# YannisLamp/crypto-recommendation

Measured on AMD Instinct MI355X. Metric: point hash+assign ops/sec at d=128, N=10M, K=256; 1/2/4/8 MI355X, higher is better.
Workload: dtype fp32 points; split-f16 MFMA scores (f32 accumulate); tuples, bucket IDs and cluster IDs bit-exact (x87-exact hashing, certified argmin); distances: certified f32, <= 2^-20 relative to the reference's fp64 (north star: 1e-5; the context's default LSHKM_DIST_CERTIFIED mode), LSHKM_DIST_EXACT for the r; 1 GPU; C3 Lloyd K=256 + C2 LSH L=5 k=4 hashing, N=10000000 per GPU, d=128; N_per_gpu=10000000, N_total=10000000, d=128, K=256, L=5, k=4, nb=100000, parallelism=dp1 (row shards)

## Files before the change

crypto-recommendation_amd/csrc/api.cpp:

```cpp
#include <hip/hip_runtime.h>

#include <algorithm>
#include <cmath>
#include <cstring>
#include <map>
#include <mutex>
#include <random>
#include <sstream>
#include <string>
#include <vector>

#include "../../include/lshkm.h"
#include "common.h"
#include "kernels.h"
#include "index.h"
#include "kpp_layout.h"

namespace lshkm {
static thread_local std::string g_err;
void set_error(const std::string& msg) { g_err = msg; }

int device_cu_count(int* ncu) {
    static std::mutex mu;
    static std::map<int, int> cus;
    int dev = 0;
    if (hipGetDevice(&dev) != hipSuccess) return kstatus("hipGetDevice");
    std::lock_guard<std::mutex> lock(mu);
    if (!cus.count(dev) &&
        hipDeviceGetAttribute(&cus[dev], hipDeviceAttributeMultiprocessorCount, dev) != hipSuccess) {
        cus.erase(dev);
        return kstatus("hipDeviceGetAttribute");
    }
    *ncu = cus[dev];
    return 0;
}
}

using namespace lshkm;

namespace lshkm {

Buf::~Buf() { if (p) (void)hipFree(p); }
int Buf::reserve(size_t bytes) {
    if (bytes <= cap) return 0;
    if (p) { (void)hipFree(p); p = nullptr; cap = 0; }
    if (hipMalloc(&p, bytes) != hipSuccess) { set_error("hipMalloc failed (" + std::to_string(bytes) + " B)"); p = nullptr; return LSHKM_ERR_NOMEM; }
    cap = bytes;
    return 0;
}

}

extern "C" {

const char* lshkm_last_error(void) { return g_err.c_str(); }
const char* lshkm_version(void) { return "lshkm-gfx950 0.1"; }

int lshkm_ctx_create(int device, lshkm_ctx* out) {
    LSHKM_CHECK(out, LSHKM_ERR_ARG, "out is NULL");
    *out = nullptr;
    if (const int rc = pow_contract_check()) return rc;
    int n = 0;
    LSHKM_HIP(hipGetDeviceCount(&n));
    LSHKM_CHECK(device >= 0 && device < n, LSHKM_ERR_ARG, "device out of range");
    LSHKM_HIP(hipSetDevice(device));
    hipDeviceProp_t prop;
    LSHKM_HIP(hipGetDeviceProperties(&prop, device));
    LSHKM_CHECK(std::string(prop.gcnArchName).find("gfx950") != std::string::npos, LSHKM_ERR_UNSUPPORTED,
                std::string("liblshkm is built for gfx950 only; device is ") + prop.gcnArchName);
    lshkm_ctx c = new lshkm_ctx_s();
    c->device = device;
    if (hipStreamCreateWithFlags(&c->own_stream, hipStreamNonBlocking) != hipSuccess) { delete c; set_error("stream create failed"); return LSHKM_ERR_HIP; }
    c->stream = c->own_stream;
    if (c->stats.reserve(sizeof(unsigned long long) * STAT_COUNT)) { delete c; return LSHKM_ERR_NOMEM; }
    (void)hipMemsetAsync(c->stats.p, 0, sizeof(unsigned long long) * STAT_COUNT, c->stream);
    *out = c;
    return 0;
}

int lshkm_ctx_set_stream(lshkm_ctx ctx, void* s) {
    LSHKM_CHECK(ctx, LSHKM_ERR_ARG, "ctx is NULL");
    ctx->stream = (hipStream_t)s;
    return 0;
}

int lshkm_ctx_set_dist_mode(lshkm_ctx ctx, int mode) {
    LSHKM_CHECK(ctx, LSHKM_ERR_ARG, "ctx is NULL");
    LSHKM_CHECK(mode == LSHKM_DIST_CERTIFIED || mode == LSHKM_DIST_EXACT, LSHKM_ERR_ARG,
                "unknown distance mode (LSHKM_DIST_CERTIFIED or LSHKM_DIST_EXACT)");
    ctx->dist_mode = mode;
    return 0;
}

int lshkm_ctx_get_dist_mode(lshkm_ctx ctx, int* mode) {
    LSHKM_CHECK(ctx && mode, LSHKM_ERR_ARG, "bad arguments");
    *mode = ctx->dist_mode;
    return 0;
}

int lshkm_ctx_sync(lshkm_ctx ctx) {
    LSHKM_CHECK(ctx, LSHKM_ERR_ARG, "ctx is NULL");
    LSHKM_HIP(hipStreamSynchronize(ctx->stream));
    return 0;
}

int lshkm_dev_alloc(lshkm_ctx ctx, int64_t bytes, void** out) {
    LSHKM_CHECK(ctx && out && bytes >= 0, LSHKM_ERR_ARG, "bad arguments");
    *out = nullptr;
    if (bytes == 0) return 0;
    LSHKM_HIP(hipSetDevice(ctx->device));
    if (hipMalloc(out, (size_t)bytes) != hipSuccess) {
        *out = nullptr;
        set_error("hipMalloc failed (" + std::to_string(bytes) + " B)");
        return LSHKM_ERR_NOMEM;
    }
    return 0;
}

int lshkm_dev_free(lshkm_ctx ctx, void* p) {
    LSHKM_CHECK(ctx, LSHKM_ERR_ARG, "ctx is NULL");
    if (!p) return 0;
    LSHKM_HIP(hipStreamSynchronize(ctx->stream));
    LSHKM_HIP(hipFree(p));
    return 0;
}

int lshkm_memcpy_h2d(lshkm_ctx ctx, void* dst_dev, const void* src_host, int64_t bytes) {
    LSHKM_CHECK(ctx && bytes >= 0 && (bytes == 0 || (dst_dev && src_host)), LSHKM_ERR_ARG, "bad arguments");
    if (bytes == 0) return 0;
    LSHKM_HIP(hipMemcpyAsync(dst_dev, src_host, (size_t)bytes, hipMemcpyHostToDevice, ctx->stream));
    LSHKM_HIP(hipStreamSynchronize(ctx->stream));
    return 0;
}

int lshkm_memcpy_d2h(lshkm_ctx ctx, void* dst_host, const void* src_dev, int64_t bytes) {
    LSHKM_CHECK(ctx && bytes >= 0 && (bytes == 0 || (dst_host && src_dev)), LSHKM_ERR_ARG, "bad arguments");
    if (bytes == 0) return 0;
    LSHKM_HIP(hipMemcpyAsync(dst_host, src_dev, (size_t)bytes, hipMemcpyDeviceToHost, ctx->stream));
    LSHKM_HIP(hipStreamSynchronize(ctx->stream));
    return 0;
}

int lshkm_ctx_destroy(lshkm_ctx ctx) {
    if (!ctx) return 0;
    (void)hipStreamSynchronize(ctx->stream);
    if (ctx->own_stream) (void)hipStreamDestroy(ctx->own_stream);
    delete ctx;
    return 0;
}

int lshkm_get_stat(lshkm_ctx ctx, int which, int64_t* v) {
    LSHKM_CHECK(ctx && v && which >= 0 && which < STAT_COUNT, LSHKM_ERR_ARG, "bad stat query");
    unsigned long long x = 0;
    LSHKM_HIP(hipMemcpyAsync(&x, (unsigned long long*)ctx->stats.p + which, sizeof(x), hipMemcpyDeviceToHost, ctx->stream));
    LSHKM_HIP(hipStreamSynchronize(ctx->stream));
    *v = (int64_t)x;
    return 0;
}

int lshkm_ctx_enable_timing(lshkm_ctx ctx, int on) {
    LSHKM_CHECK(ctx, LSHKM_ERR_ARG, "ctx is NULL");
    for (hipEvent_t& e : ctx->tev)
        if (!e) LSHKM_HIP(hipEventCreate(&e));
    ctx->timing = on != 0;
    return 0;
}

int lshkm_last_kernel_ms(lshkm_ctx ctx, float* ms) {
    LSHKM_CHECK(ctx && ms && ctx->tev[1], LSHKM_ERR_STATE, "timing not enabled");
    LSHKM_HIP(hipEventSynchronize(ctx->tev[1]));
    LSHKM_HIP(hipEventElapsedTime(ms, ctx->tev[0], ctx->tev[1]));
    if (ctx->tev_side) {
        float m2 = 0.f;
        LSHKM_HIP(hipEventSynchronize(ctx->tev[2]));
        LSHKM_HIP(hipEventElapsedTime(&m2, ctx->tev[0], ctx->tev[2]));
        *ms = std::max(*ms, m2);
    }
    return 0;
}

int lshkm_reset_stats(lshkm_ctx ctx) {
    LSHKM_CHECK(ctx, LSHKM_ERR_ARG, "ctx is NULL");
    LSHKM_HIP(hipMemsetAsync(ctx->stats.p, 0, sizeof(unsigned long long) * STAT_COUNT, ctx->stream));
    return 0;
}

static uint32_t engine_state(std::default_random_engine& g) {
    std::ostringstream os;
    os << g;
    return (uint32_t)std::stoul(os.str());
}

static void draw_euclid_h(std::default_random_engine& g, int d, float w, float* v, float* t) {
    std::normal_distribution<float> nd(0, 1);
    for (int j = 0; j < d; j++) v[j] = nd(g);
    std::uniform_real_distribution<float> ud(0, w);
    *t = ud(g);
}

static void draw_cosine_h(std::default_random_engine& g, int d, double* r) {
    std::normal_distribution<double> nd(0, 1);
    for (int j = 0; j < d; j++) r[j] = nd(g);
}

int lshkm_params_lsh_euclidean(uint64_t seed, int L, int k, int d, float w, float* V, float* t, int32_t* r,
                               uint32_t* state) {
    LSHKM_CHECK(L > 0 && k > 0 && d > 0 && V && t && r, LSHKM_ERR_ARG, "bad arguments");
    std::default_random_engine g;
    g.seed((unsigned long)seed);
    for (int l = 0; l < L; l++) {
        std::uniform_int_distribution<int> uid(0, 100);
        for (int i = 0; i < k; i++) {
            const size_t li = (size_t)l * k + i;
            draw_euclid_h(g, d, w, V + li * d, t + li);
            r[li] = uid(g);
        }
    }
    if (state) *state = engine_state(g);
    return 0;
}

int lshkm_params_lsh_cosine(uint64_t seed, int L, int k, int d, double* R, uint32_t* state) {
    LSHKM_CHECK(L > 0 && k > 0 && d > 0 && R, LSHKM_ERR_ARG, "bad arguments");
    std::default_random_engine g;
    g.seed((unsigned long)seed);
    for (int l = 0; l < L; l++)
        for (int i = 0; i < k; i++) draw_cosine_h(g, d, R + ((size_t)l * k + i) * d);
    if (state) *state = engine_state(g);
    return 0;
}

int lshkm_params_cube_euclidean(uint64_t seed, int k, int d, float w, float* V, float* t, uint32_t* state) {
    LSHKM_CHECK(k > 0 && d > 0 && V && t, LSHKM_ERR_ARG, "bad arguments");
    std::default_random_engine g;
    g.seed((unsigned long)seed);
    for (int i = 0; i < k; i++) draw_euclid_h(g, d, w, V + (size_t)i * d, t + i);
    if (state) *state = engine_state(g);
    return 0;
}

int lshkm_coins_draw(uint32_t* rng_state, const int32_t* h, int64_t n, int32_t* bit) {
    LSHKM_CHECK(rng_state && n >= 0 && (n == 0 || (h && bit)), LSHKM_ERR_ARG, "bad arguments");
    std::default_random_engine g;
    g.seed((unsigned long)*rng_state);
    LSHKM_CHECK(engine_state(g) == *rng_state, LSHKM_ERR_ARG, "rng_state is not a minstd_rand0 state");
    for (int64_t i = 0; i < n; i++) {
        std::uniform_int_distribution<int> coin(1, 2);
        const int c = coin(g);
        bit[i] = (h[i] % c + c) % c;
    }
    *rng_state = engine_state(g);
    return 0;
}

int lshkm_rand_selection(uint64_t seed, int64_t N, int K, int32_t* rows) {
    LSHKM_CHECK(rows && N >= 1 && N <= INT32_MAX && K >= 1 && K <= N, LSHKM_ERR_ARG,
                "bad arguments (need 1 <= K <= N < 2^31)");
    std::default_random_engine g;
    g.seed((unsigned long)seed);
    std::uniform_int_distribution<int> uni(0, (int)(N - 1));
    rows[0] = uni(g);
    for (int i = 1; i < K; i++) {
        int r = uni(g), c = 0;
        while (c < i) {
            if (rows[c] == r) { r = uni(g); c = 0; }
            else c++;
        }
        rows[i] = r;
    }
    return 0;
}

int lshkm_kpp_draws(uint64_t seed, int64_t N_total, int K, int64_t* first_row, double* canon) {
    LSHKM_CHECK(first_row && canon && N_total >= 1 && N_total <= INT32_MAX && K >= 1, LSHKM_ERR_ARG,
                "bad arguments (need 1 <= N < 2^31, K >= 1)");
    std::default_random_engine g;
    g.seed((unsigned long)seed);
    std::uniform_int_distribution<int> uni(0, (int)(N_total - 1));
    *first_row = uni(g);
    canon[0] = 0.0;
    for (int i = 1; i < K; i++) {
        std::uniform_real_distribution<double> unit(0.0, 1.0);
        canon[i] = unit(g);
    }
    return 0;
}

}

static int kmeans_pp_impl(lshkm_ctx ctx, Pts X, int64_t N, int d, int K, int metric, uint64_t seed, int32_t* rows) {
    LSHKM_CHECK(ctx && X.p && rows && N >= 1 && N <= INT32_MAX && d >= 1 && d <= 4096 && K >= 1, LSHKM_ERR_ARG,
                "bad arguments (need N < 2^31, 1 <= d <= 4096, K >= 1)");
    LSHKM_CHECK(metric == LSHKM_METRIC_EUCLIDEAN || metric == LSHKM_METRIC_COSINE, LSHKM_ERR_ARG, "unknown metric");
    LSHKM_HIP(hipSetDevice(ctx->device));
    std::vector<int32_t> chosen(K, 0);
    std::vector<double> canon(K, 0.0);
    int64_t first = 0;
    if (const int rc = lshkm_kpp_draws(seed, N, K, &first, canon.data())) return rc;
    chosen[0] = (int32_t)first;
    Buf &ws = ctx->ws_call[0], &dch = ctx->ws_call[1], &dcanon = ctx->ws_call[2];
    int rc;
    if ((rc = ws.reserve(kpp_layout(N).bytes)) || (rc = dch.reserve(sizeof(int32_t) * K)) ||
        (rc = dcanon.reserve(sizeof(double) * K)))
        return rc;
    LSHKM_HIP(hipMemcpyAsync(dch.p, chosen.data(), sizeof(int32_t) * K, hipMemcpyHostToDevice, ctx->stream));
    LSHKM_HIP(hipMemcpyAsync(dcanon.p, canon.data(), sizeof(double) * K, hipMemcpyHostToDevice, ctx->stream));
    if ((rc = launch_kmeans_pp(ctx->stream, X, N, d, K, metric, dcanon.as<double>(), dch.as<int32_t>(), ws.p,
                               (unsigned long long*)ctx->stats.p))) {
        (void)hipStreamSynchronize(ctx->stream);
        return rc;
    }
    LSHKM_HIP(hipMemcpyAsync(rows, dch.p, sizeof(int32_t) * K, hipMemcpyDeviceToHost, ctx->stream));
    LSHKM_HIP(hipStreamSynchronize(ctx->stream));
    return 0;
}

extern "C" {

int lshkm_kmeans_pp(lshkm_ctx ctx, const float* X, int64_t N, int d, int K, int metric, uint64_t seed,
                    int32_t* rows) {
    return kmeans_pp_impl(ctx, X, N, d, K, metric, seed, rows);
}

int lshkm_kmeans_pp_f64(lshkm_ctx ctx, const double* X, int64_t N, int d, int K, int metric, uint64_t seed,
                        int32_t* rows) {
    return kmeans_pp_impl(ctx, X, N, d, K, metric, seed, rows);
}

}

static int kpp_shard_ws_check(lshkm_ctx ctx, int64_t n, const void* ws, int64_t ws_bytes) {
    LSHKM_CHECK(ctx && n >= 0 && n <= INT32_MAX, LSHKM_ERR_ARG, "bad arguments (need 0 <= n < 2^31)");
    LSHKM_CHECK(n == 0 || (ws && ws_bytes >= 0 && (size_t)ws_bytes >= kpp_layout(n).bytes), LSHKM_ERR_ARG,
                "workspace smaller than lshkm_kpp_shard_ws_bytes");
    LSHKM_HIP(hipSetDevice(ctx->device));
    return 0;
}

static int kpp_shard_read(lshkm_ctx ctx, int64_t n, const void* ws, int launch_rc, KppShardOut* out) {
    if (launch_rc) {
        (void)hipStreamSynchronize(ctx->stream);
        return launch_rc;
    }
    LSHKM_HIP(hipMemcpyAsync(out, (const char*)ws + kpp_layout(n).out, sizeof(*out), hipMemcpyDeviceToHost,
                             ctx->stream));
    LSHKM_HIP(hipStreamSynchronize(ctx->stream));
    return 0;
}

static int kpp_shard_dist_impl(lshkm_ctx ctx, Pts X, int64_t n, int d, int metric, const void* c, int it, void* ws,
                               int64_t ws_bytes, uint64_t* max_bits, double* sum) {
    if (const int rc = kpp_shard_ws_check(ctx, n, ws, ws_bytes)) return rc;
    LSHKM_CHECK(max_bits && sum && d >= 1 && d <= 4096 && it >= 1, LSHKM_ERR_ARG,
                "bad arguments (need 1 <= d <= 4096, it >= 1)");
    LSHKM_CHECK(metric == LSHKM_METRIC_EUCLIDEAN || metric == LSHKM_METRIC_COSINE, LSHKM_ERR_ARG, "unknown metric");
    *max_bits = 0;
    *sum = 0.0;
    if (n == 0) return 0;
    LSHKM_CHECK(X.p && c, LSHKM_ERR_ARG, "rows or centroid row is NULL");
    KppShardOut o;
    const int lrc = launch_kpp_shard_dist(ctx->stream, X, n, d, metric, c, it, ws);
    if (const int rc = kpp_shard_read(ctx, n, ws, lrc, &o)) return rc;
    *max_bits = o.max_bits;
    *sum = o.sum;
    return 0;
}

extern "C" {

int lshkm_kpp_shard_ws_bytes(int64_t n, int64_t* bytes) {
    LSHKM_CHECK(bytes && n >= 0 && n <= INT32_MAX, LSHKM_ERR_ARG, "bad arguments (need 0 <= n < 2^31)");
    *bytes = (int64_t)kpp_layout(n).bytes;
    return 0;
}

int lshkm_kpp_shard_dist(lshkm_ctx ctx, const float* X, int64_t n, int d, int metric, const float* c, int it, void* ws,
                         int64_t ws_bytes, uint64_t* max_bits, double* sum) {
    return kpp_shard_dist_impl(ctx, X, n, d, metric, c, it, ws, ws_bytes, max_bits, sum);
}

int lshkm_kpp_shard_dist_f64(lshkm_ctx ctx, const double* X, int64_t n, int d, int metric, const double* c, int it,
                             void* ws, int64_t ws_bytes, uint64_t* max_bits, double* sum) {
    return kpp_shard_dist_impl(ctx, X, n, d, metric, c, it, ws, ws_bytes, max_bits, sum);
}

int lshkm_kpp_shard_units(lshkm_ctx ctx, int64_t n, uint64_t gmax_bits, double start, void* ws, int64_t ws_bytes) {
    if (const int rc = kpp_shard_ws_check(ctx, n, ws, ws_bytes)) return rc;
    if (n == 0) return 0;
    return launch_kpp_shard_units(ctx->stream, n, gmax_bits, start, ws);
}

int lshkm_kpp_shard_chain(lshkm_ctx ctx, int64_t n, double s_in, void* ws, int64_t ws_bytes, double* s_out) {
    if (const int rc = kpp_shard_ws_check(ctx, n, ws, ws_bytes)) return rc;
    LSHKM_CHECK(s_out, LSHKM_ERR_ARG, "s_out is NULL");
    *s_out = s_in;
    if (n == 0) return 0;
    KppShardOut o;
    const int lrc = launch_kpp_shard_chain(ctx->stream, n, s_in, ws, (unsigned long long*)ctx->stats.p);
    if (const int rc = kpp_shard_read(ctx, n, ws, lrc, &o)) return rc;
    *s_out = o.s_out;
    return 0;
}

int lshkm_kpp_shard_pick(lshkm_ctx ctx, int64_t n, double rd, int owns_row0, void* ws, int64_t ws_bytes,
                         int64_t* row) {
    if (const int rc = kpp_shard_ws_check(ctx, n, ws, ws_bytes)) return rc;
    LSHKM_CHECK(row, LSHKM_ERR_ARG, "row is NULL");
    *row = -1;
    if (n == 0) return 0;
    KppShardOut o;
    const int lrc = launch_kpp_shard_pick(ctx->stream, n, rd, owns_row0, ws);
    if (const int rc = kpp_shard_read(ctx, n, ws, lrc, &o)) return rc;
    LSHKM_CHECK(o.pick >= -1 && o.pick < n, LSHKM_ERR_STATE, "pick outside the shard (rd above the running sum?)");
    *row = o.pick;
    return 0;
}

int lshkm_params_cube_cosine(uint64_t seed, int k, int d, double* R, uint32_t* state) {
    LSHKM_CHECK(k > 0 && d > 0 && R, LSHKM_ERR_ARG, "bad arguments");
    std::default_random_engine g;
    g.seed((unsigned long)seed);
    for (int i = 0; i < k; i++) draw_cosine_h(g, d, R + (size_t)i * d);
    if (state) *state = engine_state(g);
    return 0;
}

}

namespace lshkm {

int ProjTable::upload(hipStream_t s, int metric_, int d_, int L_, int k_, float w_, const float* V, const float* t,
                      const int32_t* r, const double* R) {
    metric = metric_; d = d_; L = L_; k = k_; w = w_;
    LK = L * k;
    LKpad = hash_lkpad(LK);
    const int drows = (d + 3) / 4 * 4;
    std::vector<double> PT((size_t)drows * LKpad, 0.0), pn(LK, 0.0);
    std::vector<float> tt(LK, 0.f);
    std::vector<int32_t> rr(LK, 0);
    for (int f = 0; f < LK; f++) {
        long double n2 = 0.0L;
        for (int j = 0; j < d; j++) {
            const double v = metric == LSHKM_METRIC_EUCLIDEAN ? (double)V[(size_t)f * d + j] : R[(size_t)f * d + j];
            PT[(size_t)j * LKpad + f] = v;
            n2 += (long double)v * (long double)v;
        }
        pn[f] = (double)sqrtl(n2) * (1.0 + 0x1p-40);
        if (metric == LSHKM_METRIC_EUCLIDEAN) { tt[f] = t ? t[f] : 0.f; rr[f] = r ? r[f] : 0; }
    }
    int rc;
    if ((rc = PT_d.reserve(PT.size() * 8)) || (rc = t_d.reserve(LK * 4)) || (rc = pn_d.reserve(LK * 8)) ||
        (rc = r_d.reserve(LK * 4)))
        return rc;
    LSHKM_HIP(hipMemcpyAsync(PT_d.p, PT.data(), PT.size() * 8, hipMemcpyHostToDevice, s));
    LSHKM_HIP(hipMemcpyAsync(t_d.p, tt.data(), LK * 4, hipMemcpyHostToDevice, s));
    LSHKM_HIP(hipMemcpyAsync(pn_d.p, pn.data(), LK * 8, hipMemcpyHostToDevice, s));
    LSHKM_HIP(hipMemcpyAsync(r_d.p, rr.data(), LK * 4, hipMemcpyHostToDevice, s));
    bool r_small = true;
    for (int f = 0; f < LK; f++) r_small = r_small && rr[f] >= 0 && rr[f] <= 100;
    fused_ok = metric == LSHKM_METRIC_EUCLIDEAN && d == 128 && LK <= 32 && r_small;
    mfma_ok = d == 128 && LK <= 32;
    std::vector<_Float16> vh, vl;
    std::vector<double> v1;
    if (mfma_ok) {
        vh.assign(64 * 128, (_Float16)0.f);
        vl.assign(64 * 128, (_Float16)0.f);
        v1.assign(LK, 0.0);
        for (int f = 0; f < LK; f++) {
            long double s1 = 0.0L;
            for (int j = 0; j < 128; j++) {
                const double v = metric == LSHKM_METRIC_EUCLIDEAN ? (double)V[(size_t)f * d + j] : R[(size_t)f * d + j];
                const _Float16 hv = (_Float16)v;
                vh[f * 128 + j] = hv;
                vl[f * 128 + j] = (_Float16)(float)(v - (double)hv);
                s1 += fabsl((long double)v);
            }
            v1[f] = (double)s1 * (1.0 + 0x1p-40);
        }
        if ((rc = vh_d.reserve(vh.size() * 2)) || (rc = vl_d.reserve(vl.size() * 2)) || (rc = v1_d.reserve(LK * 8)))
            return rc;
        LSHKM_HIP(hipMemcpyAsync(vh_d.p, vh.data(), vh.size() * 2, hipMemcpyHostToDevice, s));
        LSHKM_HIP(hipMemcpyAsync(vl_d.p, vl.data(), vl.size() * 2, hipMemcpyHostToDevice, s));
        LSHKM_HIP(hipMemcpyAsync(v1_d.p, v1.data(), LK * 8, hipMemcpyHostToDevice, s));
    }
    LSHKM_HIP(hipStreamSynchronize(s));
    hV.assign(V ? V : (const float*)nullptr, V ? V + (size_t)LK * d : nullptr);
    return 0;
}

HashParams ProjTable::params(int64_t nb) const {
    HashParams p;
    p.PT = (const double*)PT_d.p;
    p.t = (const float*)t_d.p;
    p.pnorm = (const double*)pn_d.p;
    p.r = (const int32_t*)r_d.p;
    p.w = w;
    p.d = d; p.L = L; p.k = k; p.LK = LK; p.LKpad = LKpad;
    p.nb = nb;
    return p;
}

HashMfmaParams ProjTable::mfma_params(int64_t nb) const {
    HashMfmaParams p;
    p.Vh = vh_d.as<_Float16>(); p.Vl = vl_d.as<_Float16>();
    p.t = (const float*)t_d.p; p.pnorm = (const double*)pn_d.p; p.v1 = (const double*)v1_d.p;
    p.r = (const int32_t*)r_d.p; p.PT = (const double*)PT_d.p;
    p.w = w;
    p.d = d; p.L = L; p.k = k; p.LK = LK; p.LKpad = LKpad;
    p.nb = nb;
    return p;
}

}

extern "C" {

int lshkm_lsh_create(lshkm_ctx ctx, int metric, int d, int k, int L, int64_t nb, float w, const float* V,
                     const float* t, const int32_t* r, const double* R, lshkm_lsh* out) {
    LSHKM_CHECK(ctx && out, LSHKM_ERR_ARG, "ctx/out is NULL");
    LSHKM_CHECK(d > 0 && d <= 1024 && k > 0 && L > 0 && L * k <= 256, LSHKM_ERR_ARG, "unsupported d/k/L");
    LSHKM_CHECK(k <= 30, LSHKM_ERR_ARG, "k > 30");
    if (metric == LSHKM_METRIC_EUCLIDEAN) {
        LSHKM_CHECK(V && t && r, LSHKM_ERR_ARG, "euclidean LSH needs V, t, r");
        LSHKM_CHECK(nb > 0 && nb < (1ll << 31), LSHKM_ERR_ARG, "nb must be in [1, 2^31)");
        LSHKM_CHECK(w > 0.f, LSHKM_ERR_ARG, "w must be > 0");
    } else if (metric == LSHKM_METRIC_COSINE) {
        LSHKM_CHECK(R, LSHKM_ERR_ARG, "cosine LSH needs R");
        nb = (int64_t)1 << k;
    } else {
        set_error("unknown metric");
        return LSHKM_ERR_ARG;
    }
    LSHKM_HIP(hipSetDevice(ctx->device));
    lshkm_lsh h = new lshkm_lsh_s();
    h->ctx = ctx; h->metric = metric; h->nb = nb;
    int rc = h->proj.upload(ctx->stream, metric, d, L, k, w, V, t, r, R);
    if (rc) { delete h; return rc; }
    *out = h;
    return 0;
}

int lshkm_lsh_destroy(lshkm_lsh lsh) {
    if (!lsh) return 0;
    (void)hipDeviceSynchronize();
    delete lsh;
    return 0;
}

}

static int lsh_hash_impl(lshkm_lsh lsh, Pts X, int64_t N, int32_t* tuples, int32_t* phi, int32_t* bucket) {
    LSHKM_CHECK(lsh && (X.p || N == 0) && N >= 0, LSHKM_ERR_ARG, "bad arguments");
    lshkm_ctx ctx = lsh->ctx;
    LSHKM_HIP(hipSetDevice(ctx->device));
    const int mode = lsh->metric == LSHKM_METRIC_EUCLIDEAN ? HM_LSH_EUCLID : HM_LSH_COSINE;
    const int rc = hash_rows(ctx, mode, X, N, lsh->proj, lsh->nb, mode == HM_LSH_EUCLID ? tuples : nullptr, phi, bucket,
                             nullptr);
    if (rc) { LSHKM_LAUNCH_CHECK(); return rc; }
    return 0;
}

extern "C" {

int lshkm_lsh_hash(lshkm_lsh lsh, const float* X, int64_t N, int32_t* tuples, int32_t* phi, int32_t* bucket) {
    return lsh_hash_impl(lsh, X, N, tuples, phi, bucket);
}

int lshkm_lsh_hash_f64(lshkm_lsh lsh, const double* X, int64_t N, int32_t* tuples, int32_t* phi, int32_t* bucket) {
    return lsh_hash_impl(lsh, X, N, tuples, phi, bucket);
}

}

static int assign_path(int metric, int d, int K, bool f64) {
    if (test_switch("LSHKM_ASSIGN_PATH", "exact")) return 2;
    if (!test_switch("LSHKM_ASSIGN_PATH", "f32")) {
        const FusedRoute r = fused_route(metric != LSHKM_METRIC_EUCLIDEAN, f64, d, K, false, 0, 0,
                                         test_switch("LSHKM_FUSED_FORM", "chunked"));
        if (r.form != FusedForm::none) return r.rows == 0 ? 0 : 3;
    }
    return assign_dp(d) > 0 ? 1 : 2;
}

static bool fuse_hash(const lshkm_lsh_s* lsh, int metric, int K, bool f64) {
    const lshkm::ProjTable& pj = lsh->proj;
    if (lsh->metric != metric || !(metric == LSHKM_METRIC_EUCLIDEAN ? pj.fused_ok : pj.mfma_ok)) return false;
    return fused_route(metric != LSHKM_METRIC_EUCLIDEAN, f64, pj.d, K, true, pj.k, pj.LK,
                       test_switch("LSHKM_FUSED_FORM", "chunked")).form != FusedForm::none;
}

ExactForm lshkm::exact_form(const AssignJob& q) {
    return exact_route(q.metric != LSHKM_METRIC_EUCLIDEAN, q.X.f64, q.d, q.K, test_switch("LSHKM_EXACT_PASS", "full"));
}

int lshkm::exact_listed_prep(lshkm_ctx ctx, const AssignJob& q) {
    const ExactForm form = exact_form(q);
    int rc;
    if ((rc = ctx->ws_ct.reserve(exact_ws_bytes(form, q.d, q.K)))) return rc;
    return launch_exact_prep(ctx->stream, q, form, ctx->ws_ct.p);
}

int lshkm::exact_listed(lshkm_ctx ctx, const AssignJob& q, const RowList& l, bool exact_dist, bool prepped,
                        const double* xn2, const double* nbv) {
    int rc;
    if (!prepped && l.bound > 0 && (rc = exact_listed_prep(ctx, q))) return rc;
    return launch_exact_pass(ctx->stream, q, l, exact_form(q), ctx->ws_ct.p, exact_dist, xn2, nbv);
}

static int assign_f32_mfma(lshkm_ctx ctx, const AssignJob& q) {
    hipStream_t s = ctx->stream;
    const int DP = assign_dp(q.d), Kpad = (q.K + 63) / 64 * 64;
    const int64_t N = q.N;
    int rc;
    if ((rc = ctx->ws_c32.reserve((size_t)Kpad * DP * 4)) || (rc = ctx->ws_cconst.reserve((size_t)3 * Kpad * 4)) ||
        (rc = ctx->ws_ambig.reserve((size_t)std::max<int64_t>(N, 1) * 2 * 4)) ||
        (rc = ctx->ws_counter.reserve(64)))
        return rc;
    unsigned long long* cnt = (unsigned long long*)ctx->ws_counter.p;
    LSHKM_HIP(hipMemsetAsync(cnt, 0, 16, s));
    if ((rc = launch_centroid_prep(s, q.C, q.K, Kpad, q.d, DP, q.metric, q.X.f64, (float*)ctx->ws_c32.p, (float*)ctx->ws_cconst.p))) return rc;
    if ((rc = launch_assign_mfma(s, q.X, N, q.d, DP, q.C, q.K, Kpad, q.metric, (const float*)ctx->ws_c32.p, (const float*)ctx->ws_cconst.p,
                                 q.assign, q.dist, (int32_t*)ctx->ws_ambig.p, cnt))) return rc;
    RowList l;
    l.p = (int32_t*)ctx->ws_ambig.p; l.count = cnt; l.bound = N;
    if ((rc = exact_listed(ctx, q, l, true, false, nullptr, nullptr))) return rc;
    if (q.metric != LSHKM_METRIC_EUCLIDEAN &&
        ((rc = launch_cos_fix(s, q.X, N, q.d, q.C, (const int32_t*)ctx->ws_ambig.p + N, cnt + 1, q.assign, q.dist)) ||
         (rc = launch_add_counter(s, (unsigned long long*)ctx->stats.p + STAT_COS_FIX, cnt + 1)))) return rc;
    return launch_add_counter(s, (unsigned long long*)ctx->stats.p + STAT_ASSIGN_AMBIG, cnt);
}

static int assign_impl(lshkm_ctx ctx, Pts X, int64_t N, int d, const double* C, int K, int metric,
                       const int32_t* src_rows_host, int32_t* assign, double* dist, lshkm_lsh lsh, int32_t* tuples,
                       int32_t* phi, int32_t* bucket, bool force_exact = false) {
    hipStream_t s = ctx->stream;
    const int path = assign_path(metric, d, K, X.f64);
    AssignRequest q;
    q.X = X; q.N = N; q.d = d; q.C = C; q.K = K; q.metric = metric; q.assign = assign; q.dist = dist;
    q.tuples = tuples; q.phi = phi; q.bucket = bucket; q.force_exact = force_exact;
    if (lsh && path == 0 && fuse_hash(lsh, metric, K, X.f64)) q.lsh = lsh;
    int rc;
    if (lsh && !q.lsh && (rc = hash_rows(ctx, lsh->metric == LSHKM_METRIC_EUCLIDEAN ? HM_LSH_EUCLID : HM_LSH_COSINE,
                                         X, N, lsh->proj, lsh->nb,
                                         lsh->metric == LSHKM_METRIC_EUCLIDEAN ? tuples : nullptr, phi, bucket,
                                         nullptr))) { LSHKM_LAUNCH_CHECK(); return rc; }
    if (path == 0 || path == 3) rc = fused_assign(ctx, q);
    else if (path == 1) rc = assign_f32_mfma(ctx, q);
    else {
        RowList all;
        all.bound = N;
        rc = launch_exact_pass(s, q, all, ExactForm::every, nullptr, true, nullptr, nullptr);
    }
    if (rc) { LSHKM_LAUNCH_CHECK(); return rc; }
    if (src_rows_host) {
        if ((rc = ctx->ws_src.reserve((size_t)K * 4))) return rc;
        const bool same = ctx->src_cache_dev == ctx->ws_src.p && ctx->src_cache_cap == ctx->ws_src.cap &&
                          ctx->src_cache.size() == (size_t)K &&
                          std::memcmp(ctx->src_cache.data(), src_rows_host, (size_t)K * 4) == 0;
        if (!same) {
            if ((rc = ctx->pin_stage((size_t)K * 4))) return rc;
            std::memcpy(ctx->pinned, src_rows_host, (size_t)K * 4);
            LSHKM_HIP(hipMemcpyAsync(ctx->ws_src.p, ctx->pinned, (size_t)K * 4, hipMemcpyHostToDevice, s));
            LSHKM_HIP(hipEventRecord(ctx->pinned_ev, s));
            ctx->src_cache.assign(src_rows_host, src_rows_host + K);
            ctx->src_cache_dev = ctx->ws_src.p;
            ctx->src_cache_cap = ctx->ws_src.cap;
        }
        if ((rc = launch_assign_override(s, (const int32_t*)ctx->ws_src.p, K, N, assign, dist))) { LSHKM_LAUNCH_CHECK(); return rc; }
    }
    return 0;
}

static int lloyd_impl(lshkm_ctx ctx, Pts X, int64_t N, int d, const double* C, int K, int metric,
                      const int32_t* src_rows_host, int32_t* assign, double* dist) {
    LSHKM_CHECK(ctx && (X.p || N == 0) && C && (assign || N == 0) && (dist || N == 0) && N >= 0 && d > 0 && K > 0,
                LSHKM_ERR_ARG, "bad arguments");
    LSHKM_CHECK(metric == LSHKM_METRIC_EUCLIDEAN || metric == LSHKM_METRIC_COSINE, LSHKM_ERR_ARG, "unknown metric");
    LSHKM_HIP(hipSetDevice(ctx->device));
    return assign_impl(ctx, X, N, d, C, K, metric, src_rows_host, assign, dist, nullptr, nullptr, nullptr, nullptr);
}

static int hash_assign_impl(lshkm_lsh lsh, Pts X, int64_t N, const double* C, int K, const int32_t* src_rows_host,
                            int32_t* tuples, int32_t* phi, int32_t* bucket, int32_t* assign, double* dist,
                            int metric = LSHKM_METRIC_EUCLIDEAN) {
    LSHKM_CHECK(lsh && (X.p || N == 0) && C && (assign || N == 0) && (dist || N == 0) && N >= 0 && K > 0, LSHKM_ERR_ARG,
                "bad arguments");
    lshkm_ctx ctx = lsh->ctx;
    LSHKM_HIP(hipSetDevice(ctx->device));
    LSHKM_CHECK(metric == LSHKM_METRIC_EUCLIDEAN || metric == LSHKM_METRIC_COSINE, LSHKM_ERR_ARG, "unknown metric");
    return assign_impl(ctx, X, N, lsh->proj.d, C, K, metric, src_rows_host, assign, dist, lsh, tuples, phi, bucket);
}

static int range_impl(lshkm_ctx ctx, Pts X, int64_t N, int d, const double* C, int K, int metric,
                      const int64_t* comb_ptr, const int32_t* comb_idx, const int32_t* key_host,
                      const int32_t* src_rows_host, int32_t* assign, double* dist, int* passes_host) {
    LSHKM_CHECK(ctx && (X.p || N == 0) && C && comb_ptr && (assign || N == 0) && (dist || N == 0) && N >= 0 &&
                    N < (1ll << 31) && d > 0 && K > 0,
                LSHKM_ERR_ARG, "bad arguments");
    LSHKM_CHECK(metric == LSHKM_METRIC_EUCLIDEAN || metric == LSHKM_METRIC_COSINE, LSHKM_ERR_ARG, "unknown metric");
    LSHKM_HIP(hipSetDevice(ctx->device));
    hipStream_t s = ctx->stream;
    lshkm::Buf* w = ctx->ws_range;
    int rc;
    int64_t M = 0;
    LSHKM_HIP(hipMemcpyAsync(&M, comb_ptr + K, 8, hipMemcpyDeviceToHost, s));
    LSHKM_HIP(hipStreamSynchronize(s));
    LSHKM_CHECK(M >= 0 && (M == 0 || comb_idx), LSHKM_ERR_ARG, "bad combined-bucket CSR");
    const size_t scratch = sort_scratch_bytes(std::max<int64_t>(M, 1), std::max<int64_t>(N, 1));
    if ((rc = w[0].reserve(64)) || (rc = w[1].reserve((size_t)std::max<int64_t>(M, 1) * 4 * 4)) ||
        (rc = w[2].reserve(scratch)) || (rc = w[3].reserve((size_t)(N + 1) * 8)) ||
        (rc = w[4].reserve((size_t)std::max<int64_t>(M, 1) * 9)) || (rc = w[5].reserve((size_t)K * 4)))
        return rc;
    double* r0 = (double*)w[0].p;
    unsigned long long* cnt = (unsigned long long*)w[0].p + 1;
    int32_t* rows = (int32_t*)w[1].p;
    int32_t* cents = rows + std::max<int64_t>(M, 1);
    int32_t* rows_s = cents + std::max<int64_t>(M, 1);
    int32_t* cents_s = rows_s + std::max<int64_t>(M, 1);
    int64_t* vptr = (int64_t*)w[3].p;
    double* cache = (double*)w[4].p;
    int8_t* cached = (int8_t*)(cache + std::max<int64_t>(M, 1));
    const int32_t* key = nullptr;
    if (key_host) {
        LSHKM_HIP(hipMemcpyAsync(w[5].p, key_host, (size_t)K * 4, hipMemcpyHostToDevice, s));
        key = (const int32_t*)w[5].p;
    }
    if ((rc = launch_range_radius(s, C, K, d, metric, r0, (unsigned long long*)w[0].p + 4))) return rc;
    if ((rc = launch_range_init(s, N, assign, dist))) return rc;
    int passes = 0;
    if (M > 0 && N > 0) {
        if ((rc = launch_range_pairs(s, comb_ptr, comb_idx, K, rows, cents))) return rc;
        if ((rc = stable_sort_by_key(s, rows, 1, cents, M, N, rows_s, cents_s, w[2].p))) return rc;
        if ((rc = launch_csr_bounds(s, rows_s, M, N, vptr))) return rc;
        LSHKM_HIP(hipMemsetAsync(cached, 0, (size_t)M, s));
        for (;;) {
            unsigned long long assigned = 0;
            LSHKM_HIP(hipMemsetAsync(cnt, 0, 8, s));
            if ((rc = launch_range_pass(s, X, d, C, K, metric, key, vptr, cents_s, cache, cached, N, r0, passes,
                                        assign, dist, cnt)))
                return rc;
            passes++;
            LSHKM_HIP(hipMemcpyAsync(&assigned, cnt, 8, hipMemcpyDeviceToHost, s));
            LSHKM_HIP(hipStreamSynchronize(s));
            if (!assigned) break;
        }
    } else {
        passes = 1;
    }
    if (N > 0) {
        if ((rc = w[6].reserve((size_t)N * 4))) return rc;
        int32_t* list = (int32_t*)w[6].p;
        unsigned long long* ucnt = cnt + 1;
        unsigned long long U = 0;
        LSHKM_HIP(hipMemsetAsync(ucnt, 0, 8, s));
        if ((rc = launch_range_unassigned(s, assign, N, list, ucnt))) return rc;
        LSHKM_HIP(hipMemcpyAsync(&U, ucnt, 8, hipMemcpyDeviceToHost, s));
        LSHKM_HIP(hipStreamSynchronize(s));
        if (U > 0) {
            if ((rc = w[7].reserve((size_t)U * d * X.esize())) || (rc = w[8].reserve((size_t)U * 12))) return rc;
            double* dr = (double*)w[8].p;
            int32_t* ar = (int32_t*)(dr + U);
            if ((rc = launch_range_gather(s, X, d, list, (int64_t)U, w[7].p))) return rc;
            const Pts Xr = X.f64 ? Pts(w[7].as<double>()) : Pts(w[7].as<float>());
            rc = assign_impl(ctx, Xr, (int64_t)U, d, C, K, metric, nullptr, ar, dr, nullptr, nullptr, nullptr, nullptr,
                             true);
            if (rc) return rc;
            if ((rc = launch_range_scatter(s, list, (int64_t)U, ar, dr, assign, dist))) return rc;
        }
    }
    if (src_rows_host) {
        if ((rc = ctx->ws_src.reserve((size_t)K * 4))) return rc;
        ctx->src_cache_dev = nullptr;
        LSHKM_HIP(hipMemcpyAsync(ctx->ws_src.p, src_rows_host, (size_t)K * 4, hipMemcpyHostToDevice, s));
        if ((rc = launch_assign_override(s, (const int32_t*)ctx->ws_src.p, K, N, assign, dist))) return rc;
        LSHKM_HIP(hipStreamSynchronize(s));
    }
    if (key_host) LSHKM_HIP(hipStreamSynchronize(s));
    if (passes_host) *passes_host = passes;
    return 0;
}

extern "C" {

int lshkm_lloyd_assign(lshkm_ctx ctx, const float* X, int64_t N, int d, const double* C, int K, int metric,
                       const int32_t* src_rows_host, int32_t* assign, double* dist) {
    return lloyd_impl(ctx, X, N, d, C, K, metric, src_rows_host, assign, dist);
}

int lshkm_lloyd_assign_f64(lshkm_ctx ctx, const double* X, int64_t N, int d, const double* C, int K, int metric,
                           const int32_t* src_rows_host, int32_t* assign, double* dist) {
    return lloyd_impl(ctx, X, N, d, C, K, metric, src_rows_host, assign, dist);
}

int lshkm_hash_assign(lshkm_lsh lsh, const float* X, int64_t N, const double* C, int K, const int32_t* src_rows_host,
                      int32_t* tuples, int32_t* phi, int32_t* bucket, int32_t* assign, double* dist) {
    return hash_assign_impl(lsh, X, N, C, K, src_rows_host, tuples, phi, bucket, assign, dist);
}

int lshkm_hash_assign_f64(lshkm_lsh lsh, const double* X, int64_t N, const double* C, int K,
                          const int32_t* src_rows_host, int32_t* tuples, int32_t* phi, int32_t* bucket,
                          int32_t* assign, double* dist) {
    return hash_assign_impl(lsh, X, N, C, K, src_rows_host, tuples, phi, bucket, assign, dist);
}

int lshkm_hash_assign_metric(lshkm_lsh lsh, const float* X, int64_t N, const double* C, int K, int metric,
                             const int32_t* src_rows_host, int32_t* tuples, int32_t* phi, int32_t* bucket,
                             int32_t* assign, double* dist) {
    return hash_assign_impl(lsh, X, N, C, K, src_rows_host, tuples, phi, bucket, assign, dist, metric);
}

int lshkm_hash_assign_metric_f64(lshkm_lsh lsh, const double* X, int64_t N, const double* C, int K, int metric,
                                 const int32_t* src_rows_host, int32_t* tuples, int32_t* phi, int32_t* bucket,
                                 int32_t* assign, double* dist) {
    return hash_assign_impl(lsh, X, N, C, K, src_rows_host, tuples, phi, bucket, assign, dist, metric);
}

int lshkm_range_assign(lshkm_ctx ctx, const float* X, int64_t N, int d, const double* C, int K, int metric,
                       const int64_t* comb_ptr, const int32_t* comb_idx, const int32_t* key_host,
                       const int32_t* src_rows_host, int32_t* assign, double* dist, int* passes_host) {
    return range_impl(ctx, X, N, d, C, K, metric, comb_ptr, comb_idx, key_host, src_rows_host, assign, dist,
                      passes_host);
}

int lshkm_range_assign_f64(lshkm_ctx ctx, const double* X, int64_t N, int d, const double* C, int K, int metric,
                           const int64_t* comb_ptr, const int32_t* comb_idx, const int32_t* key_host,
                           const int32_t* src_rows_host, int32_t* assign, double* dist, int* passes_host) {
    return range_impl(ctx, X, N, d, C, K, metric, comb_ptr, comb_idx, key_host, src_rows_host, assign, dist,
                      passes_host);
}

int lshkm_synth(lshkm_ctx ctx, uint64_t seed, int64_t row0, int64_t rows, int d, float* X) {
    LSHKM_CHECK(ctx && (X || rows == 0) && rows >= 0 && d > 0, LSHKM_ERR_ARG, "bad arguments");
    LSHKM_HIP(hipSetDevice(ctx->device));
    int rc = launch_synth(ctx->stream, seed, row0, rows, d, X);
    if (rc) { LSHKM_LAUNCH_CHECK(); }
    return rc;
}

int lshkm_synth_normal(lshkm_ctx ctx, uint64_t seed, int64_t row0, int64_t rows, int d, float* X) {
    LSHKM_CHECK(ctx && (X || rows == 0) && rows >= 0 && d > 0, LSHKM_ERR_ARG, "bad arguments");
    LSHKM_HIP(hipSetDevice(ctx->device));
    int rc = launch_synth(ctx->stream, seed, row0, rows, d, X, 1);
    if (rc) { LSHKM_LAUNCH_CHECK(); }
    return rc;
}

}
```

crypto-recommendation_amd/csrc/assign.hip:

```cpp
#include "common.h"
#include "kernels.h"
#include "exact.h"

namespace lshkm {

constexpr int AS_THREADS = 256;
constexpr int AS_PB = 128;
constexpr int AS_CC = 64;

typedef float floatx16 __attribute__((ext_vector_type(16)));

int assign_dp(int d) {
    const int dps[] = {16, 32, 64, 128, 256};
    for (int dp : dps)
        if (d <= dp) return dp;
    return 0;
}

__global__ void centroid_prep_kernel(const double* __restrict__ C, int K, int Kpad, int d, int DP, int metric,
                                     int xf64, float* __restrict__ C32, float* __restrict__ cconst) {
    const int c = blockIdx.x * 64 + threadIdx.x;
    const double xw = xf64 ? 2.0 : 0.0;
    float* cn2 = cconst;
    float* chunk = cconst + Kpad + 2 * blockIdx.x;
    double ec = 0.0, eb = 0.0;
    if (c >= K) {
        for (int j = 0; j < DP; j++) C32[(size_t)c * DP + j] = 0.f;
        cn2[c] = metric ? __builtin_nanf("") : __builtin_inff();
    } else {
        double s = 0.0;
        for (int j = 0; j < d; j++) {
            const double v = C[(size_t)c * d + j];
            s = fma(v, v, s);
            C32[(size_t)c * DP + j] = (float)v;
        }
        for (int j = d; j < DP; j++) C32[(size_t)c * DP + j] = 0.f;
        const double up = 1.0 + 0x1p-18;
        const double nc = sqrt(s) * (1.0 + 0x1p-30);
        if (metric == 0) {
            cn2[c] = s < 0x1p100 ? (float)s : __builtin_inff();
            if (!(s < 0x1p100)) atomicOr(reinterpret_cast<unsigned int*>(cconst + Kpad + Kpad / 32), 1u);
            ec = 0x1p-24 * (2.0 * DP + 12.0 + xw) * nc * up;
            eb = (0x1p-24 * 5.0 * s + 0x1p-40 * s + (xf64 ? 0x1p-140 * nc : 0.0)) * up + 1e-30;
        } else {
            const bool ok = s >= 1e-20 && s < 1e30;
            const double rc = ok ? 1.0 / sqrt(s) : 0.0;
            cn2[c] = ok ? (float)rc : __builtin_nanf("");
            ec = (0x1p-24 * (DP + 20.0 + xw) + 0x1p-40) * up;
            eb = ok ? ((DP + 4.0) * 0x1p-124 * rc + 0x1p-116) * up
                    : (s == 0.0 && c > 0 ? 0.0 : __builtin_inf());
        }
    }
    for (int off = 32; off >= 1; off >>= 1) {
        ec = fmax(ec, __shfl_xor(ec, off));
        eb = fmax(eb, __shfl_xor(eb, off));
    }
    if (threadIdx.x == 0) {
        chunk[0] = (float)(ec * (1.0 + 0x1p-20));
        chunk[1] = (float)(eb * (1.0 + 0x1p-20));
    }
}

int launch_centroid_prep(hipStream_t s, const double* C, int K, int Kpad, int d, int DP, int metric, bool xf64,
                         float* C32, float* cconst) {
    (void)hipMemsetAsync(cconst + Kpad + Kpad / 32, 0, 4, s);
    hipLaunchKernelGGL(centroid_prep_kernel, dim3((Kpad + 63) / 64), dim3(64), 0, s, C, K, Kpad, d, DP, metric,
                       xf64 ? 1 : 0, C32, cconst);
    return kstatus("assign.hip");
}

template <int DP, int MET, typename TX>
__global__ __launch_bounds__(AS_THREADS, 2) void assign_mfma_kernel(
    const TX* __restrict__ X, int64_t N, int d, const double* __restrict__ C, int Kpad,
    const float* __restrict__ C32, const float* __restrict__ cconst, int32_t* __restrict__ assign,
    double* __restrict__ dist, int32_t* __restrict__ ambig, unsigned long long* __restrict__ ambig_count) {
    constexpr int H = DP / 2;
    constexpr int DS = DP + 4;
    extern __shared__ __attribute__((aligned(16))) char smem[];
    float* lds = reinterpret_cast<float*>(smem);
    const int lane = threadIdx.x & 63, wave = threadIdx.x >> 6;
    const int col = lane & 31, h = lane >> 5;
    const int64_t pbase = (int64_t)blockIdx.x * AS_PB + wave * 32;

    float* xs = lds + wave * 32 * DS;
    if (d == DP) {
        for (int e4 = lane; e4 < 32 * DP / 4; e4 += 64) {
            const int r = e4 / (DP / 4), j = (e4 % (DP / 4)) * 4;
            const int64_t row = pbase + r;
            float4 v = make_float4(0.f, 0.f, 0.f, 0.f);
            if constexpr (sizeof(TX) == 4) {
                if (row < N) v = *reinterpret_cast<const float4*>(X + row * DP + j);
            } else if (row < N) {
                const double2 a = *reinterpret_cast<const double2*>(X + row * DP + j);
                const double2 b = *reinterpret_cast<const double2*>(X + row * DP + j + 2);
                v = make_float4((float)a.x, (float)a.y, (float)b.x, (float)b.y);
            }
            *reinterpret_cast<float4*>(xs + r * DS + j) = v;
        }
    } else if (sizeof(TX) == 8 && (d & 1) == 0) {
        for (int e2 = lane; e2 < 32 * DP / 2; e2 += 64) {
            const int r = e2 / (DP / 2), j = (e2 % (DP / 2)) * 2;
            const int64_t row = pbase + r;
            float2 v = make_float2(0.f, 0.f);
            if (row < N && j < d) {
                const double2 a = *reinterpret_cast<const double2*>(X + row * d + j);
                v = make_float2((float)a.x, (float)a.y);
            }
            *reinterpret_cast<float2*>(xs + r * DS + j) = v;
        }
    } else if (sizeof(TX) == 4 && (d & 3) == 0) {
        for (int e4 = lane; e4 < 32 * DP / 4; e4 += 64) {
            const int r = e4 / (DP / 4), j = (e4 % (DP / 4)) * 4;
            const int64_t row = pbase + r;
            float4 v = make_float4(0.f, 0.f, 0.f, 0.f);
            if (row < N && j < d) v = *reinterpret_cast<const float4*>(reinterpret_cast<const float*>(X) + row * d + j);
            *reinterpret_cast<float4*>(xs + r * DS + j) = v;
        }
    } else {
        for (int e = lane; e < 32 * DP; e += 64) {
            const int r = e / DP, j = e % DP;
            const int64_t row = pbase + r;
            xs[r * DS + j] = (row < N && j < d) ? (float)X[row * d + j] : 0.f;
        }
    }
    __syncthreads();
    float b[H];
#pragma unroll
    for (int s = 0; s < H; s += 4) {
        const float4 v = *reinterpret_cast<const float4*>(xs + col * DS + h * H + s);
        b[s] = v.x; b[s + 1] = v.y; b[s + 2] = v.z; b[s + 3] = v.w;
    }
    double xn2 = 0.0;
#pragma unroll
    for (int s = 0; s < H; s++) xn2 = fma((double)b[s], (double)b[s], xn2);
    xn2 += __shfl_xor(xn2, 32);
    if (sizeof(TX) == 8) xn2 = xn2 * (1.0 + 0x1p-21) + 0x1p-280;
    const float nx = (float)(sqrt(xn2) * (1.0 + 0x1p-30));
    const float ex = MET == 0 ? (xn2 < 0x1p100 ? (float)(0x1p-40 * xn2 * (1.0 + 0x1p-18) + 1e-30) : __builtin_inff())
                              : (xn2 < 1e36 ? 0.f : __builtin_inff());
    __syncthreads();

    float L1 = __builtin_inff(), L2 = __builtin_inff(), U = __builtin_inff();
    int i1 = 0;
    float* cs = lds;
    float* cc = lds + AS_CC * DS;
    const float* chunkc = cconst + Kpad;
    for (int c0 = 0; c0 < Kpad; c0 += AS_CC) {
        for (int e4 = threadIdx.x; e4 < AS_CC * DP / 4; e4 += AS_THREADS) {
            const int r = e4 / (DP / 4), j = (e4 % (DP / 4)) * 4;
            *reinterpret_cast<float4*>(cs + r * DS + j) =
                *reinterpret_cast<const float4*>(C32 + (size_t)(c0 + r) * DP + j);
        }
        if (threadIdx.x < AS_CC) cc[threadIdx.x] = cconst[c0 + threadIdx.x];
        const float E = fmaf(nx, chunkc[2 * (c0 / AS_CC)], chunkc[2 * (c0 / AS_CC) + 1] + ex);
        __syncthreads();
#pragma unroll 1
        for (int t = 0; t < AS_CC / 32; t++) {
            floatx16 acc;
#pragma unroll
            for (int r = 0; r < 16; r++) acc[r] = 0.f;
            const float* arow = cs + (t * 32 + col) * DS + h * H;
#pragma unroll
            for (int s = 0; s < H; s += 4) {
                const float4 a = *reinterpret_cast<const float4*>(arow + s);
                acc = __builtin_amdgcn_mfma_f32_32x32x2f32(a.x, b[s], acc, 0, 0, 0);
                acc = __builtin_amdgcn_mfma_f32_32x32x2f32(a.y, b[s + 1], acc, 0, 0, 0);
                acc = __builtin_amdgcn_mfma_f32_32x32x2f32(a.z, b[s + 2], acc, 0, 0, 0);
                acc = __builtin_amdgcn_mfma_f32_32x32x2f32(a.w, b[s + 3], acc, 0, 0, 0);
            }
#pragma unroll
            for (int g = 0; g < 4; g++) {
                const int cb = t * 32 + 8 * g + 4 * h;
                const float4 cn = *reinterpret_cast<const float4*>(cc + cb);
                const float cnv[4] = {cn.x, cn.y, cn.z, cn.w};
#pragma unroll
                for (int q = 0; q < 4; q++) {
                    const float sc = MET == 0 ? fmaf(-2.f, acc[4 * g + q], cnv[q]) : -acc[4 * g + q] * cnv[q];
                    const float lo = sc - E, hi = sc + E;
                    if (lo < L1) { L2 = L1; L1 = lo; i1 = c0 + cb + q; }
                    else if (lo < L2) L2 = lo;
                    U = fminf(U, hi);
                }
            }
        }
        __syncthreads();
    }

    const float oL1 = __shfl_xor(L1, 32), oL2 = __shfl_xor(L2, 32), oU = __shfl_xor(U, 32);
    const int oi1 = __shfl_xor(i1, 32);
    float nL2; int ni1;
    if (oL1 < L1 || (oL1 == L1 && oi1 < i1)) { ni1 = oi1; nL2 = fminf(L1, oL2); }
    else { ni1 = i1; nL2 = fminf(oL1, L2); }
    U = fminf(U, oU);
    const bool cbad = __float_as_uint(cconst[Kpad + Kpad / 32]) != 0u;
    const bool cert = !cbad && nL2 > U;
    const int64_t row = pbase + col;
    const bool valid = row < N;

    if (MET == 1) {
        bool fix = false;
        if (h == 1 && valid) {
            if (cert) {
                assign[row] = ni1;
                double v;
                if (cosine_fast(X + row * d, C + (size_t)ni1 * d, d, v)) dist[row] = v;
                else fix = true;
            } else {
                const unsigned long long slot = atomicAdd(ambig_count, 1ull);
                ambig[slot] = (int32_t)row;
            }
        }
        seg_append(fix, (int32_t)row, ambig_count + 1, ambig + N, lane);
        return;
    }
    double accd = 0.0;
    const TX* xrow = X + (valid ? row : 0) * d;
    if (h == 0 && cert && valid) {
        const double* crow = C + (size_t)ni1 * d;
#pragma unroll
        for (int s = 0; s < H; s++)
            if (s < d) {
                const double xv = sizeof(TX) == 4 ? (double)b[s] : (double)xrow[s];
                const double df = __dsub_rn(xv, crow[s]);
                accd = __dadd_rn(accd, gp_sq(df));
            }
    }
    const double part = __shfl_xor(accd, 32);
    if (h == 1 && valid) {
        if (cert) {
            double a2 = part;
            const double* crow = C + (size_t)ni1 * d;
#pragma unroll
            for (int s = 0; s < H; s++)
                if (H + s < d) {
                    const double xv = sizeof(TX) == 4 ? (double)b[s] : (double)xrow[H + s];
                    const double df = __dsub_rn(xv, crow[H + s]);
                    a2 = __dadd_rn(a2, gp_sq(df));
                }
            assign[row] = ni1;
            dist[row] = sqrt(a2);
        } else {
            const unsigned long long slot = atomicAdd(ambig_count, 1ull);
            ambig[slot] = (int32_t)row;
        }
    }
}

template <typename TX>
static int assign_mfma_tx(hipStream_t s, const TX* X, int64_t N, int d, int DP, const double* C, int Kpad, int metric,
                          const float* C32, const float* cconst, int32_t* assign, double* dist, int32_t* ambig,
                          unsigned long long* ambig_count) {
    const dim3 grid((unsigned)((N + AS_PB - 1) / AS_PB)), block(AS_THREADS);
    const size_t lds = (size_t)4 * 32 * (DP + 4) * 4;
    switch (DP * 2 + (metric ? 1 : 0)) {
#define AS_CASE(V) \
        case 2 * V: hipLaunchKernelGGL((assign_mfma_kernel<V, 0, TX>), grid, block, lds, s, X, N, d, C, Kpad, C32, cconst, assign, dist, ambig, ambig_count); break; \
        case 2 * V + 1: hipLaunchKernelGGL((assign_mfma_kernel<V, 1, TX>), grid, block, lds, s, X, N, d, C, Kpad, C32, cconst, assign, dist, ambig, ambig_count); break;
        AS_CASE(16) AS_CASE(32) AS_CASE(64) AS_CASE(128) AS_CASE(256)
#undef AS_CASE
        default: return -4;
    }
    return kstatus("assign.hip");
}

int launch_assign_mfma(hipStream_t s, Pts X, int64_t N, int d, int DP, const double* C, int K, int Kpad, int metric,
                       const float* C32, const float* cconst, int32_t* assign, double* dist, int32_t* ambig,
                       unsigned long long* ambig_count) {
    (void)K;
    if (N <= 0) return 0;
    return X.f64 ? assign_mfma_tx(s, X.d(), N, d, DP, C, Kpad, metric, C32, cconst, assign, dist, ambig, ambig_count)
                 : assign_mfma_tx(s, X.f(), N, d, DP, C, Kpad, metric, C32, cconst, assign, dist, ambig, ambig_count);
}

template <typename TX>
__global__ __launch_bounds__(256) void cos_fix_kernel(const TX* __restrict__ X, int d, const double* __restrict__ C,
                                                      const int32_t* __restrict__ rows,
                                                      const unsigned long long* __restrict__ count,
                                                      const int32_t* __restrict__ assign, double* __restrict__ dist) {
    const int64_t n = (int64_t)*count;
    for (int64_t i = (int64_t)blockIdx.x * 256 + threadIdx.x; i < n; i += (int64_t)gridDim.x * 256) {
        const int64_t row = rows[i];
        dist[row] = exact_cosine_x87(X + row * d, C + (size_t)assign[row] * d, d);
    }
}

int launch_cos_fix(hipStream_t s, Pts X, int64_t N, int d, const double* C, const int32_t* rows,
                   const unsigned long long* count, const int32_t* assign, double* dist) {
    if (N <= 0) return 0;
    const dim3 grid((unsigned)std::min<int64_t>((N + 255) / 256, 2048));
    if (X.f64) hipLaunchKernelGGL(cos_fix_kernel<double>, grid, dim3(256), 0, s, X.d(), d, C, rows, count, assign, dist);
    else hipLaunchKernelGGL(cos_fix_kernel<float>, grid, dim3(256), 0, s, X.f(), d, C, rows, count, assign, dist);
    return kstatus("assign.hip");
}

__global__ void assign_override_kernel(const int32_t* __restrict__ src, int K, int64_t N,
                                       int32_t* __restrict__ assign, double* __restrict__ dist) {
    const int c = blockIdx.x * blockDim.x + threadIdx.x;
    if (c >= K) return;
    const int32_t r = src[c];
    if (r < 0 || r >= N) return;
    for (int c2 = c + 1; c2 < K; c2++)
        if (src[c2] == r) return;
    assign[r] = c;
    dist[r] = 0.0;
}

constexpr int OV_LDS_MAX = 8192;
__global__ __launch_bounds__(1024) void assign_override_lds_kernel(const int32_t* __restrict__ src, int K, int64_t N,
                                                                  int32_t* __restrict__ assign,
                                                                  double* __restrict__ dist) {
    __shared__ __attribute__((aligned(16))) int32_t ls[OV_LDS_MAX + 16];
    const int Kp = (K + 15) & ~15;
    for (int c = threadIdx.x; c < Kp + 16; c += blockDim.x) ls[c] = c < K ? src[c] : -1;
    __syncthreads();
    for (int c = threadIdx.x; c < K; c += blockDim.x) {
        const int32_t r = ls[c];
        if (r < 0 || r >= N) continue;
        bool later = false;
        for (int b = (c + 1) & ~15; b < Kp && !later; b += 16) {
            const int4 v0 = *reinterpret_cast<const int4*>(ls + b);
            const int4 v1 = *reinterpret_cast<const int4*>(ls + b + 4);
            const int4 v2 = *reinterpret_cast<const int4*>(ls + b + 8);
            const int4 v3 = *reinterpret_cast<const int4*>(ls + b + 12);
            const int w[16] = {v0.x, v0.y, v0.z, v0.w, v1.x, v1.y, v1.z, v1.w,
                               v2.x, v2.y, v2.z, v2.w, v3.x, v3.y, v3.z, v3.w};
#pragma unroll
            for (int t = 0; t < 16; t++) later |= b + t > c && w[t] == r;
        }
        if (!later) {
            assign[r] = c;
            dist[r] = 0.0;
        }
    }
}

int launch_assign_override(hipStream_t s, const int32_t* src_rows, int K, int64_t N, int32_t* assign,
                           double* dist) {
    if (K <= OV_LDS_MAX)
        hipLaunchKernelGGL(assign_override_lds_kernel, dim3(1), dim3(1024), 0, s, src_rows, K, N, assign, dist);
    else
        hipLaunchKernelGGL(assign_override_kernel, dim3((K + 255) / 256), dim3(256), 0, s, src_rows, K, N, assign,
                           dist);
    return kstatus("assign.hip");
}

__global__ void add_counter_kernel(unsigned long long* dst, const unsigned long long* src) {
    if (threadIdx.x == 0) *dst += *src;
}

int launch_add_counter(hipStream_t s, unsigned long long* dst, const unsigned long long* src) {
    hipLaunchKernelGGL(add_counter_kernel, dim3(1), dim3(1), 0, s, dst, src);
    return kstatus("assign.hip");
}

struct CounterAdds {
    int n;
    int dst[8];
    const unsigned long long* src[8];
};
__global__ void add_counters_kernel(unsigned long long* stats, CounterAdds c) {
    if ((int)threadIdx.x < c.n) atomicAdd(stats + c.dst[threadIdx.x], *c.src[threadIdx.x]);
}

int launch_add_counters(hipStream_t s, unsigned long long* stats, int n, const int* dst_idx,
                        const unsigned long long* const* src) {
    if (n <= 0) return 0;
    if (n > 8) {
        set_error("launch_add_counters: at most 8 counters");
        return -1;
    }
    CounterAdds c;
    c.n = n;
    for (int i = 0; i < n; i++) { c.dst[i] = dst_idx[i]; c.src[i] = src[i]; }
    hipLaunchKernelGGL(add_counters_kernel, dim3(1), dim3(64), 0, s, stats, c);
    return kstatus("assign.hip");
}

}
```

crypto-recommendation_amd/csrc/exact_pass.hip:

```cpp
#include <type_traits>

#include "common.h"
#include "kernels.h"
#include "exact.h"
#include "pick.h"

namespace lshkm {

struct ListWalk {
    const int32_t* rows;
    int64_t total, g0, gstride;
};
template <int SPLIT, int WAVES>
__device__ inline ListWalk list_walk(const int32_t* rows, const unsigned long long* row_count, int64_t max_rows,
                                     const int32_t* seg_counts, int64_t seg_rows) {
    const int wave = threadIdx.x >> 6;
    ListWalk w;
    if (seg_counts) {
        const int nseg = gridDim.x / SPLIT;
        const int seg = blockIdx.x % nseg, part = blockIdx.x / nseg;
        w.rows = rows + (int64_t)seg * seg_rows;
        w.total = seg_counts[SEG_SLOTS * seg + SEG_ROWS];
        w.g0 = (int64_t)part * WAVES + wave;
        w.gstride = (int64_t)SPLIT * WAVES;
    } else {
        w.rows = rows;
        w.total = rows ? (int64_t)*row_count : max_rows;
        w.g0 = (int64_t)blockIdx.x * WAVES + wave;
        w.gstride = (int64_t)gridDim.x * WAVES;
    }
    if (w.total > max_rows) w.total = max_rows;
    return w;
}

template <int R>
__device__ inline int group_rows(const int32_t* __restrict__ rows, int64_t base, int64_t cnt, int32_t (&myrow)[R]) {
    const int nr = (int)min((int64_t)R, cnt - base);
#pragma unroll
    for (int r = 0; r < R; r++) myrow[r] = rows[base + min(r, nr - 1)];
    return nr;
}

template <int R, typename TX>
__device__ inline void stage_rows(const TX* __restrict__ X, int d, const int32_t (&myrow)[R], TX (*xs)[XB_DMAX],
                                  float (&xn2p)[R]) {
    const int lane = threadIdx.x & 63;
    TX xv[R][XB_DMAX / 64];
#pragma unroll
    for (int r = 0; r < R; r++)
#pragma unroll
        for (int u = 0; u < XB_DMAX / 64; u++) {
            const int j = lane + 64 * u;
            xv[r][u] = j < d ? X[(int64_t)myrow[r] * d + j] : TX(0);
        }
#pragma unroll
    for (int r = 0; r < R; r++) {
        float q = 0.f;
#pragma unroll
        for (int u = 0; u < XB_DMAX / 64; u++) {
            const int j = lane + 64 * u;
            if (j < d) {
                xs[r][j] = xv[r][u];
                q = fmaf((float)xv[r][u], (float)xv[r][u], q);
            }
        }
        xn2p[r] = q;
    }
    wave_sync();
}

template <typename F>
__device__ inline void every_centroid(int K, F&& dd, double& best, int& bi) {
    for (int c = threadIdx.x & 63; c < K; c += 64) {
        const double v = dd(c);
        if (bi < 0 ? (v == v || c == 0) : v < best) { best = v; bi = c; }
    }
}

template <typename TX>
__device__ inline bool cosine_nonfinite_row(const TX* x, int d, double& best, int& bi) {
    bool bad = false;
    for (int j = threadIdx.x & 63; j < d; j += 64) bad |= !(fabs((double)x[j]) <= 1.7976931348623157e308);
    if (!__any(bad)) return false;
    best = __longlong_as_double((long long)0xFFF8000000000000ull);
    bi = 0;
    return true;
}

__device__ inline void wave_store(double best, int bi, int64_t row, int32_t* __restrict__ assign,
                                  double* __restrict__ dist) {
    group_argmin<64>(best, bi);
    if ((threadIdx.x & 63) == 0) {
        assign[row] = bi < 0 ? 0 : bi;
        dist[row] = bi < 0 ? -1.0 : best;
    }
}

constexpr int XC_MAXV = 4;
template <typename TX>
__global__ __launch_bounds__(64 * XE_WAVES) void assign_exact_kernel(
    const TX* __restrict__ X, int d, const double* __restrict__ C, int K, int metric,
    const int32_t* __restrict__ rows, const unsigned long long* __restrict__ row_count, int64_t max_rows,
    int32_t* __restrict__ assign, double* __restrict__ dist, const int32_t* __restrict__ seg_counts,
    int64_t seg_rows, const double* __restrict__ xn2, const double* __restrict__ nbv) {
    const int lane = threadIdx.x & 63;
    const ListWalk w = list_walk<XE_SPLIT, XE_WAVES>(rows, row_count, max_rows, seg_counts, seg_rows);
    for (int64_t it = w.g0; it < w.total; it += w.gstride) {
        const int64_t row = w.rows ? w.rows[it] : it;
        const TX* x = X + row * d;
        double best = 0.0; int bi = -1;
        const double xa = metric == 1 && xn2 ? xn2[row] : -1.0;
        if (metric == 1 && cosine_nonfinite_row(x, d, best, bi)) {
            wave_store(best, bi, row, assign, dist);
            continue;
        }
        if (metric == 1 && K <= 64 * XC_MAXV) {
            double v[XC_MAXV], rad[XC_MAXV];
            int st[XC_MAXV];
            double U = __builtin_inf();
            bool unknown = false;
#pragma unroll
            for (int k = 0; k < XC_MAXV; k++) {
                const int c = lane + 64 * k;
                st[k] = 0; v[k] = 0.0; rad[k] = 0.0;
                if (c < K) {
                    st[k] = cosine_interval(x, C + (size_t)c * d, d, v[k], rad[k], xa, nbv ? nbv[c] : -1.0);
                    unknown |= st[k] == 2;
                    if (st[k] != 2) U = fmin(U, v[k] + rad[k]);
                }
            }
            if (!__ballot(unknown)) {
                U = group_min<64>(U);
#pragma unroll
                for (int k = 0; k < XC_MAXV; k++) {
                    const int c = lane + 64 * k;
                    if (c < K && v[k] - rad[k] <= U) {
                        const double dd = st[k] == 0 ? v[k] : exact_cosine_x87(x, C + (size_t)c * d, d, xa, nbv ? nbv[c] : -1.0);
                        if (bi < 0 || dd < best) { best = dd; bi = c; }
                    }
                }
                group_argmin<64>(best, bi);
                if (lane == 0) {
                    assign[row] = bi;
                    dist[row] = best;
                }
                continue;
            }
        }
        every_centroid(K, [&](int c) {
            return metric == 0 ? exact_euclid(x, C + (size_t)c * d, d)
                               : exact_cosine_x87(x, C + (size_t)c * d, d, xa, nbv ? nbv[c] : -1.0);
        }, best, bi);
        wave_store(best, bi, row, assign, dist);
    }
}

__global__ void transpose_centroids_kernel(const double* __restrict__ C, int K, int Kpad, int d,
                                           double* __restrict__ CT) {
    const int64_t e = (int64_t)blockIdx.x * blockDim.x + threadIdx.x;
    if (e >= (int64_t)d * Kpad) return;
    const int j = (int)(e / Kpad), c = (int)(e % Kpad);
    CT[e] = c < K ? C[(size_t)c * d + j] : 0.0;
}

template <typename TX>
__global__ __launch_bounds__(64 * XB_WAVES) void assign_exact_batch_kernel(
    const TX* __restrict__ X, int d, const double* __restrict__ CT, int K, int Kpad,
    const int32_t* __restrict__ rows, const unsigned long long* __restrict__ row_count, int64_t max_rows,
    int32_t* __restrict__ assign, double* __restrict__ dist, const int32_t* __restrict__ seg_counts,
    int64_t seg_rows) {
    __shared__ TX xs[XB_WAVES][XB_R][XB_DMAX];
    const int lane = threadIdx.x & 63, wave = threadIdx.x >> 6;
    const ListWalk w = list_walk<XB_SPLIT, XB_WAVES>(rows, row_count, max_rows, seg_counts, seg_rows);
    const int64_t ngroups = (w.total + XB_R - 1) / XB_R;
    for (int64_t g = w.g0; g < ngroups; g += w.gstride) {
        int32_t myrow[XB_R];
        const int nr = group_rows(w.rows, g * XB_R, w.total, myrow);
        float xn2p[XB_R];
        stage_rows(X, d, myrow, xs[wave], xn2p);
        double best[XB_R];
        int bi[XB_R];
#pragma unroll
        for (int r = 0; r < XB_R; r++) { best[r] = 0.0; bi[r] = -1; }
        for (int c0 = 0; c0 < K; c0 += 256) {
            double acc[XB_R][4];
#pragma unroll
            for (int r = 0; r < XB_R; r++)
#pragma unroll
                for (int i = 0; i < 4; i++) acc[r][i] = 0.0;
            const double* ct = CT + c0 + lane;
#pragma unroll 4
            for (int j = 0; j < d; j++) {
                double cv[4];
#pragma unroll
                for (int i = 0; i < 4; i++) cv[i] = ct[(size_t)j * Kpad + 64 * i];
#pragma unroll
                for (int r = 0; r < XB_R; r++) {
                    const double xj = (double)xs[wave][r][j];
#pragma unroll
                    for (int i = 0; i < 4; i++) {
                        const double df = __dsub_rn(xj, cv[i]);
                        acc[r][i] = __dadd_rn(acc[r][i], gp_sq(df));
                    }
                }
            }
#pragma unroll
            for (int i = 0; i < 4; i++) {
                const int c = c0 + lane + 64 * i;
                if (c >= K) continue;
#pragma unroll
                for (int r = 0; r < XB_R; r++) {
                    const double dd = sqrt(acc[r][i]);
                    if (bi[r] < 0 || dd < best[r]) { best[r] = dd; bi[r] = c; }
                }
            }
        }
#pragma unroll
        for (int r = 0; r < XB_R; r++) {
            double b = best[r];
            int i1 = bi[r];
            group_argmin<64>(b, i1);
            if (lane == 0 && r < nr) {
                assign[myrow[r]] = i1;
                dist[myrow[r]] = b;
            }
        }
        wave_sync();
    }
}


template <int MET, typename TX>
__device__ inline double pruned_dist(const TX* __restrict__ x, const double* __restrict__ c, int d) {
    if constexpr (MET == 0) {
        return exact_euclid_rolled(x, c, d);
    } else {
        if constexpr (sizeof(TX) == 4) {
            if ((d & 15) == 0) return exact_cosine_x87_b16(x, c, d);
        }
        return exact_cosine_x87(x, c, d);
    }
}

__global__ void exact_prep_kernel(const double* __restrict__ C, int K, int Kpad, int d, int xf64,
                                  float* __restrict__ CT32, float* __restrict__ cconst,
                                  float* __restrict__ chunkc, int metric) {
    const int c = blockIdx.x, lane = threadIdx.x;
    double scale = 1.0;
    if (metric == 1) {
        double q = 0.0;
        for (int j = lane; j < d; j += 64) {
            const double v = c < K ? C[(size_t)c * d + j] : 0.0;
            q = fma(v, v, q);
        }
        for (int off = 32; off >= 1; off >>= 1) q += __shfl_xor(q, off);
        scale = (q >= 1e-200 && q <= 1e200) ? 1.0 / sqrt(q) : 0.0;
        if (c < K && scale == 0.0) {
            for (int j = lane; j < d; j += 64) CT32[(size_t)j * Kpad + c] = 0.f;
            if (lane == 0) cconst[c] = __builtin_inff();
            return;
        }
    }
    double sq = 0.0;
    for (int j = lane; j < d; j += 64) {
        const double v = c < K ? C[(size_t)c * d + j] * scale : 0.0;
        sq = fma(v, v, sq);
        CT32[(size_t)j * Kpad + c] = (float)v;
    }
    for (int off = 32; off >= 1; off >>= 1) sq += __shfl_xor(sq, off);
    if (lane != 0) return;
    if (c >= K) { cconst[c] = __builtin_inff(); return; }
    unsigned int* chunk = reinterpret_cast<unsigned int*>(chunkc + 2 * (c / 64));
    if (metric == 1) {
        cconst[c] = 0.f;
        const double ec = ((d + 2.0) * 0x1p-24 * (1.0 + 0x1p-10) + 0x1p-40 + (xf64 ? 0x1p-23 : 0.0)) * (1.0 + 0x1p-18);
        atomicMax(chunk, __float_as_uint((float)(ec * (1.0 + 0x1p-20))));
        atomicMax(chunk + 1, __float_as_uint(1e-30f));
        return;
    }
    const double up = 1.0 + 0x1p-18;
    const double nc = sqrt(sq) * (1.0 + 0x1p-30);
    cconst[c] = (float)sq;
    const double ec = 0x1p-24 * (2.0 * d + 12.0 + (xf64 ? 2.0 : 0.0)) * nc * up;
    const double eb = (0x1p-24 * 5.0 * sq + 0x1p-40 * sq + (xf64 ? 0x1p-140 * nc : 0.0)) * up + 1e-30;
    atomicMax(chunk, __float_as_uint((float)(ec * (1.0 + 0x1p-20))));
    atomicMax(chunk + 1, __float_as_uint((float)(eb * (1.0 + 0x1p-20))));
}

template <int UNROLL, int R, int NCH, typename TX>
__device__ inline void score_chunks(const float* __restrict__ CT32, int Kpad, int d, const TX (*xs)[XB_DMAX],
                                    float (&acc)[R][NCH]) {
    const int lane = threadIdx.x & 63;
#pragma unroll
    for (int r = 0; r < R; r++)
#pragma unroll
        for (int i = 0; i < NCH; i++) acc[r][i] = 0.f;
    int coff[NCH];
#pragma unroll
    for (int i = 0; i < NCH; i++) coff[i] = (64 * i < Kpad ? 64 * i : 0) + lane;
#pragma unroll UNROLL
    for (int j = 0; j < d; j++) {
        float cv[NCH];
#pragma unroll
        for (int i = 0; i < NCH; i++) cv[i] = CT32[(size_t)j * Kpad + coff[i]];
#pragma unroll
        for (int r = 0; r < R; r++) {
            const float xj = (float)xs[r][j];
#pragma unroll
            for (int i = 0; i < NCH; i++) acc[r][i] = fmaf(xj, cv[i], acc[r][i]);
        }
    }
}

template <int MET, typename TX, int NCH>
__device__ inline bool row_candidates(float xn2p, const float (&acc)[NCH], const float* __restrict__ cconst,
                                      const float* __restrict__ chunkc, int K, unsigned long long (&cm)[NCH],
                                      int& ncand) {
    const int lane = threadIdx.x & 63;
    double xn2 = (double)xn2p;
    for (int off = 32; off >= 1; off >>= 1) xn2 += __shfl_xor(xn2, off);
    xn2 = xn2 * (sizeof(TX) == 4 ? 1.0 + 0x1p-20 : 1.0 + 0x1p-19) + (sizeof(TX) == 4 ? 0.0 : 0x1p-280);
    const float nx = (float)(sqrt(xn2) * (1.0 + 0x1p-30));
    const float ex = (float)(0x1p-40 * xn2 * (1.0 + 0x1p-18) + 1e-30);
    float lo[NCH];
    float U = __builtin_inff();
    bool finite = nx <= 3.0e38f;
#pragma unroll
    for (int i = 0; i < NCH; i++) {
        const int c = lane + 64 * i;
        lo[i] = __builtin_inff();
        if (c < K) {
            const float E = fmaf(nx, chunkc[2 * i], chunkc[2 * i + 1] + ex);
            const float sc = MET == 1 ? cconst[c] - acc[i] : fmaf(-2.f, acc[i], cconst[c]);
            lo[i] = sc - E;
            const float hi = sc + E;
            finite = finite && (hi - lo[i]) <= 3.0e38f;
            U = fminf(U, hi);
        }
    }
    for (int off = 32; off >= 1; off >>= 1) U = fminf(U, __shfl_xor(U, off));
    ncand = 0;
#pragma unroll
    for (int i = 0; i < NCH; i++) {
        cm[i] = __ballot(lo[i] <= U);
        ncand += __popcll(cm[i]);
    }
    return __all(finite) && ncand >= 1;
}

template <int NCH>
__device__ inline int kth_candidate(const unsigned long long (&cm)[NCH], int k) {
    int c = -1, seen = 0;
#pragma unroll
    for (int i = 0; i < NCH; i++) {
        const int n = __popcll(cm[i]);
        if (c < 0 && k >= seen && k < seen + n) {
            unsigned long long m = cm[i];
            for (int t = k - seen; t > 0; t--) m &= m - 1;
            c = 64 * i + __builtin_ctzll(m);
        }
        seen += n;
    }
    return c;
}

template <int MET, typename TX, int NCH>
__device__ inline void wave_decide(const TX* xr, const double* __restrict__ C, int d, int K, bool prune,
                                   const unsigned long long (&cm)[NCH], bool exact_dist, int64_t row,
                                   int32_t* __restrict__ assign, double* __restrict__ dist) {
    double best = 0.0;
    int bi = -1;
    if (prune) {
        const int c = kth_candidate(cm, threadIdx.x & 63);
        if constexpr (MET == 0) {
            pruned_pick_euclid<64>(xr, C, d, c, exact_dist, best, bi);
        } else if (c >= 0) {
            best = pruned_dist<MET>(xr, C + (size_t)c * d, d);
            bi = c;
        }
    } else if (!(MET == 1 && cosine_nonfinite_row(xr, d, best, bi))) {
        every_centroid(K, [&](int c) { return pruned_dist<MET>(xr, C + (size_t)c * d, d); }, best, bi);
    }
    wave_store(best, bi, row, assign, dist);
}

template <int R>
__device__ inline const int* seg_group_prefix(const int32_t* __restrict__ seg_counts, int nseg) {
    __shared__ int gpre[FUSED_MAX_SEGS + 1];
    for (int sg = threadIdx.x; sg < nseg; sg += blockDim.x) gpre[sg + 1] = (seg_counts[SEG_SLOTS * sg + SEG_ROWS] + R - 1) / R;
    __syncthreads();
    if (threadIdx.x == 0) {
        gpre[0] = 0;
        for (int sg = 0; sg < nseg; sg++) gpre[sg + 1] += gpre[sg];
    }
    __syncthreads();
    return gpre;
}

template <typename TX, int MET, bool WIDE>
__global__ __launch_bounds__(64 * XP_WAVES) void assign_pruned_kernel(
    const TX* __restrict__ X, int d, const double* __restrict__ C, const float* __restrict__ CT32,
    const float* __restrict__ cconst, const float* __restrict__ chunkc, int K, int Kpad,
    const int32_t* __restrict__ rows, const unsigned long long* __restrict__ row_count, int64_t max_rows,
    int32_t* __restrict__ assign, double* __restrict__ dist, const int32_t* __restrict__ seg_counts,
    int64_t seg_rows, int nseg, int exact_dist) {
    constexpr int NCH = WIDE ? 16 : 4, R = WIDE ? XPW_R : XP_R, UNROLL = WIDE ? 2 : 8;
    __shared__ TX xs[XP_WAVES][R][XB_DMAX];
    const int lane = threadIdx.x & 63, wave = threadIdx.x >> 6;
    const bool flat_segs = WIDE && seg_counts;
    const ListWalk w = list_walk<XP_SPLIT, XP_WAVES>(rows, row_count, max_rows, flat_segs ? nullptr : seg_counts, seg_rows);
    int64_t ngroups = (w.total + R - 1) / R;
    const int* gpre = nullptr;
    if constexpr (WIDE) {
        if (flat_segs) {
            gpre = seg_group_prefix<R>(seg_counts, nseg);
            ngroups = gpre[nseg];
        }
    }
    for (int64_t g = w.g0; g < ngroups; g += w.gstride) {
        const int32_t* grows = w.rows;
        int64_t gbase = g * R, cnt = w.total;
        if constexpr (WIDE) {
            if (flat_segs) {
                int lo = 0, hi = nseg;
                while (hi - lo > 1) {
                    const int mid = (lo + hi) >> 1;
                    if (gpre[mid] <= g) lo = mid; else hi = mid;
                }
                grows = rows + (int64_t)lo * seg_rows;
                gbase = (g - gpre[lo]) * R;
                cnt = seg_counts[SEG_SLOTS * lo + SEG_ROWS];
            }
        }
        int32_t myrow[R];
        const int nr = group_rows(grows, gbase, cnt, myrow);
        float xn2p[R];
        stage_rows(X, d, myrow, xs[wave], xn2p);
        float acc[R][NCH];
        score_chunks<UNROLL>(CT32, Kpad, d, xs[wave], acc);
        if constexpr (WIDE) {
#pragma unroll
            for (int r = 0; r < R; r++) {
                if (r >= nr) break;
                unsigned long long cm[NCH];
                int ncand;
                const bool ok = row_candidates<MET, TX>(xn2p[r], acc[r], cconst, chunkc, K, cm, ncand);
                wave_decide<MET>(xs[wave][r], C, d, K, ok && ncand <= 64, cm, exact_dist != 0, myrow[r], assign, dist);
            }
        } else {
            constexpr int RL = 64 / R;
            unsigned long long cm[R][NCH];
            int ncand[R];
            bool pr[R];
#pragma unroll
            for (int r = 0; r < R; r++)
                pr[r] = row_candidates<MET, TX>(xn2p[r], acc[r], cconst, chunkc, K, cm[r], ncand[r]) && r < nr;
            {
                const int r = lane / RL, k = lane % RL;
                int c = -1;
#pragma unroll
                for (int rr = 0; rr < R; rr++)
                    if (rr == r && pr[rr] && ncand[rr] <= RL) c = kth_candidate(cm[rr], k);
                double best = 0.0;
                int bi = -1;
                if constexpr (MET == 0) {
                    pruned_pick_euclid<RL>(xs[wave][r], C, d, c, exact_dist != 0, best, bi);
                } else {
                    if (c >= 0) {
                        best = pruned_dist<MET>(xs[wave][r], C + (size_t)c * d, d);
                        bi = c;
                    }
                    group_argmin<RL>(best, bi);
                }
                if (k == 0 && bi >= 0) {
                    assign[myrow[r]] = bi;
                    dist[myrow[r]] = best;
                }
            }
            for (int r = 0; r < nr; r++) {
                if (pr[r] && ncand[r] <= RL) continue;
                wave_decide<MET>(xs[wave][r], C, d, K, pr[r] && ncand[r] <= 64, cm[r], exact_dist != 0, myrow[r], assign, dist);
            }
        }
        wave_sync();
    }
}

int launch_exact_prep(hipStream_t s, const AssignJob& q, ExactForm form, void* ws) {
    const ExactWs w = exact_ws(form, q.d, q.K);
    char* base = static_cast<char*>(ws);
    if (form == ExactForm::batch) {
        const int64_t ne = (int64_t)q.d * w.Kpad;
        hipLaunchKernelGGL(transpose_centroids_kernel, dim3((unsigned)((ne + 255) / 256)), dim3(256), 0, s, q.C, q.K,
                           w.Kpad, q.d, reinterpret_cast<double*>(base + w.ct));
        return kstatus("transpose_centroids_kernel");
    }
    if (!exact_is_pruned(form)) return 0;
    if (q.d > XB_DMAX || q.K > XP_KMAX) {
        set_error("launch_exact_prep: unsupported shape");
        return -1;
    }
    if (hipMemsetAsync(base + w.chunk, 0, w.bytes - w.chunk, s) != hipSuccess) return kstatus("exact prep");
    hipLaunchKernelGGL(exact_prep_kernel, dim3((unsigned)w.Kpad), dim3(64), 0, s, q.C, q.K, w.Kpad, q.d, q.X.f64 ? 1 : 0,
                       reinterpret_cast<float*>(base + w.ct), reinterpret_cast<float*>(base + w.cconst),
                       reinterpret_cast<float*>(base + w.chunk), q.metric == 0 ? 0 : 1);
    return kstatus("exact_prep_kernel");
}

int launch_exact_pass(hipStream_t s, const AssignJob& q, const RowList& l, ExactForm form, const void* ws,
                      bool exact_dist, const double* xn2, const double* nbv) {
    if (l.bound <= 0) return 0;
    const int32_t* seg_counts = l.seg_counts();
    if ((form != ExactForm::every && (q.d > XB_DMAX || !l.p)) || (exact_is_pruned(form) && q.K > XP_KMAX) ||
        l.nseg > FUSED_MAX_SEGS) {
        set_error("launch_exact_pass: unsupported shape");
        return -1;
    }
    const ExactWs w = exact_ws(form, q.d, q.K);
    const char* base = static_cast<const char*>(ws);
    const dim3 grid((unsigned)exact_blocks(form, l.nseg, l.bound, l.p != nullptr));
    const int metric = q.metric == 0 ? 0 : 1;
    with_rows(q.X, [&](auto* X) {
        using TX = std::remove_cv_t<std::remove_pointer_t<decltype(X)>>;
        const auto pruned = [&](auto met, auto wide) {
            hipLaunchKernelGGL((assign_pruned_kernel<TX, decltype(met)::value, decltype(wide)::value>), grid, dim3(64 * XP_WAVES), 0, s, X, q.d,
                               q.C, reinterpret_cast<const float*>(base + w.ct),
                               reinterpret_cast<const float*>(base + w.cconst),
                               reinterpret_cast<const float*>(base + w.chunk), q.K, w.Kpad, l.p, l.count, l.bound,
                               q.assign, q.dist, seg_counts, l.seg_rows, l.nseg, exact_dist ? 1 : 0);
        };
        using Euclid = std::integral_constant<int, 0>;
        using Cosine = std::integral_constant<int, 1>;
        switch (form) {
            case ExactForm::every:
                hipLaunchKernelGGL(assign_exact_kernel<TX>, grid, dim3(64 * XE_WAVES), 0, s, X, q.d, q.C, q.K, metric,
                                   l.p, l.count, l.bound, q.assign, q.dist, seg_counts, l.seg_rows, xn2, nbv);
                break;
            case ExactForm::batch:
                hipLaunchKernelGGL(assign_exact_batch_kernel<TX>, grid, dim3(64 * XB_WAVES), 0, s, X, q.d,
                                   reinterpret_cast<const double*>(base + w.ct), q.K, w.Kpad, l.p, l.count, l.bound,
                                   q.assign, q.dist, seg_counts, l.seg_rows);
                break;
            case ExactForm::pruned:
                if (metric) pruned(Cosine{}, std::false_type{}); else pruned(Euclid{}, std::false_type{});
                break;
            case ExactForm::pruned_wide:
                if (metric) pruned(Cosine{}, std::true_type{}); else pruned(Euclid{}, std::true_type{});
                break;
        }
    });
    return kstatus("exact_pass.hip");
}

}
```

crypto-recommendation_amd/csrc/fused.hip:

```cpp
#include "../../include/lshkm.h"
#include "fused_impl.h"
#include "index.h"

namespace lshkm {

namespace {

struct FusedPlan {
    bool hash = false, cos = false;
    int rows = 0;
    int nblk = 0;
    int64_t seg_rows = 0;
    int np_hi = 0;
    int np_refine = 0;
};

int fused_workspace(lshkm_ctx ctx, const FusedShape& sh, FusedWorkspace& w) {
    const FusedLayout l = fused_layout(sh);
    int rc;
    struct { Buf& b; size_t bytes; } const bufs[] = {
        {ctx->ws_c32, l.c16},      {ctx->ws_cconst, l.cconst}, {ctx->ws_ambig, l.list1}, {ctx->ws_counter, l.counter},
        {ctx->ws_seg, l.seg1},     {ctx->ws_hfix, l.fix},      {ctx->ws_seg3, l.seg3},   {ctx->ws_part, l.part},
        {ctx->ws_ambig2, l.list2}, {ctx->ws_seg2, l.seg2},     {ctx->ws_tuples, l.tuples}, {ctx->ws_cf32, l.cf32},
        {ctx->ws_c64p, l.c64p},    {ctx->ws_xn2, l.xn2}};
    for (const auto& e : bufs)
        if (e.bytes && (rc = e.b.reserve(e.bytes))) return rc;
    const auto at = [](const Buf& b, size_t off) { return off == FusedLayout::NONE ? nullptr : (char*)b.p + off; };
    w.list_cap = l.list_cap;
    w.Ch = (_Float16*)at(ctx->ws_c32, 0); w.Cl = (_Float16*)at(ctx->ws_c32, l.cl_off);
    w.cbound = (float*)at(ctx->ws_cconst, 0); w.cnh = (float*)at(ctx->ws_cconst, l.cnh_off);
    w.nbv = (double*)at(ctx->ws_cconst, l.nbv_off);
    if (l.cf32) { w.C32 = (float*)at(ctx->ws_cf32, 0); w.rn32 = (float*)at(ctx->ws_cf32, l.rn32_off); }
    if (l.c64p) w.C64p = ctx->ws_c64p.as<double>();
    w.list1 = ctx->ws_ambig.as<int32_t>(); w.seg1 = ctx->ws_seg.as<int32_t>();
    w.list2 = ctx->ws_ambig2.as<int32_t>(); w.seg2 = ctx->ws_seg2.as<int32_t>();
    if (l.seg3) w.seg3 = ctx->ws_seg3.as<int32_t>();
    w.hfix = (unsigned long long*)at(ctx->ws_hfix, l.hfix_off);
    w.cfix = (unsigned long long*)at(ctx->ws_hfix, l.cfix_off);
    w.hfix2 = (unsigned long long*)at(ctx->ws_hfix, l.hfix2_off);
    w.pairs = (unsigned long long*)at(ctx->ws_hfix, l.pair_off);
    if (l.part) w.part = ctx->ws_part.as<float4>();
    w.cnt = ctx->ws_counter.as<unsigned long long>();
    if (l.xn2) w.xn2 = ctx->ws_xn2.as<double>();
    if (l.tuples) w.tuples = ctx->ws_tuples.as<int32_t>();
    return 0;
}

FusedArgs fused_common_args(lshkm_ctx ctx, const AssignRequest& q, const FusedShape& sh, const FusedWorkspace& w) {
    FusedArgs a{};
    a.X = q.X.f64 ? nullptr : q.X.f(); a.X64 = q.X.f64 ? q.X.d() : nullptr;
    a.N = q.N; a.d = q.d; a.K = q.K;
    a.xvec = sh.rows == 1 ? (a.d % 4 == 0 && ((uintptr_t)a.X & 15) == 0) : (a.d % 2 == 0 && ((uintptr_t)a.X64 & 15) == 0);
    a.Ch = w.Ch; a.Cl = w.Cl; a.cnh = w.cnh; a.cbound = w.cbound; a.Kpad = sh.Kpad();
    a.C64 = w.C64p ? w.C64p : q.C; a.Cd = q.C;
    a.C32 = w.C32; a.rn32 = w.rn32; a.fast_dist = sh.fast ? 1 : 0;
    a.assign = q.assign; a.dist = q.dist;
    a.stats = ctx->stats.as<unsigned long long>();
    a.nb = 1;
    if (q.lsh) {
        const ProjTable& pj = q.lsh->proj;
        a.Vh = pj.vh_d.as<_Float16>(); a.Vl = pj.vl_d.as<_Float16>(); a.PT = pj.PT_d.as<double>();
        a.tv = pj.t_d.as<float>(); a.pnorm = pj.pn_d.as<double>(); a.v1 = pj.v1_d.as<double>();
        a.rv = pj.r_d.as<int32_t>(); a.w = pj.w; a.L = pj.L; a.k = pj.k; a.LK = pj.LK; a.LKpad = pj.LKpad;
        a.nb = q.lsh->nb;
    }
    a.bdiv = make_bucket_div(a.nb);
    if (sh.cosine) { a.nbv = w.nbv; a.xn2 = w.xn2; }
    a.cfix = w.cfix; a.cfix_counts = w.seg3; a.cfix_count = w.cfix ? w.cnt + CNT_CFIX : nullptr;
    a.pass_first = 1; a.pass_last = 1;
    return a;
}

void hash_outputs(FusedArgs& a, const AssignRequest& q, const FusedShape& sh, const FusedWorkspace& w) {
    a.hfix = w.hfix; a.hfix_count = w.hfix ? w.cnt + CNT_HFIX : nullptr;
    if (!q.lsh) return;
    a.phi = q.phi; a.bucket = q.bucket;
    a.tuples = sh.cosine ? nullptr : q.tuples ? q.tuples : w.tuples;
}

template <typename T>
DevList<T> segmented(T* p, unsigned long long* count, int32_t* counts, const AssignRequest& q, const FusedPlan& plan) {
    DevList<T> l;
    l.p = p; l.count = count; l.bound = q.N; l.counts = counts;
    l.seg_rows = plan.seg_rows; l.nseg = plan.nblk;
    return l;
}

int fused_hi_passes(hipStream_t s, const FusedArgs& hi, const FusedPlan& p) {
    const bool gather_on = !test_switch("LSHKM_GATHER", "0");
    int rc;
    if (p.rows != 0) {
        HiForm h;
        h.metric = p.cos; h.rows = p.rows;
        h.fast = !p.cos && hi.fast_dist;
        h.gath = !p.cos && !h.fast && p.rows == 1 && hi.Kpad <= FH_GATH_KMAX && gather_on;
        return launch_fused_hi_pass(s, p.nblk, h, hi);
    }
    if (!p.cos && p.np_hi == 2 && test_switch("LSHKM_HI_TWO_IMAGE", "1")) {
        HiForm h;
        h.hash = p.hash; h.two_image = true;
        return launch_fused_hi_pass(s, p.nblk, h, hi);
    }
    for (int i = 0; i < p.np_hi; i++) {
        const int c0 = i * FH_KMAX;
        FusedArgs a = hi;
        a.Ch = hi.Ch + (size_t)c0 * FU_D; a.cnh = hi.cnh + c0;
        a.Kpad = std::min(FH_KMAX, hi.Kpad - c0);
        a.t0 = c0 / 32; a.pass_first = i == 0; a.pass_last = i == p.np_hi - 1;
        HiForm h;
        h.hash = p.hash && i == 0; h.mp = p.np_hi > 1; h.metric = p.cos;
        if (!p.cos && !h.mp) {
            const bool small = a.Kpad <= FH_GATH_KMAX && gather_on;
            h.fast = small && a.fast_dist;
            h.gath = small && !a.fast_dist;
            h.rowpf = h.fast && !test_switch("LSHKM_ROW_PREFETCH", "0");
        } else if (!p.cos) {
            h.fast = !h.hash && a.fast_dist && a.pass_last;
        }
        if ((rc = launch_fused_hi_pass(s, p.nblk, h, a))) return rc;
    }
    return 0;
}

int fused_refine_passes(hipStream_t s, const FusedArgs& rf, const FusedPlan& p) {
    for (int i = 0; i < p.np_refine; i++) {
        const int c0 = i * FP_KMAX;
        FusedArgs r = rf;
        r.Ch = rf.Ch + (size_t)c0 * FU_D; r.Cl = rf.Cl + (size_t)c0 * FU_D; r.cnh = rf.cnh + c0;
        r.Kpad = std::min(FP_KMAX, rf.Kpad - c0);
        r.t0 = c0 / 32; r.pass_first = i == 0; r.pass_last = i == p.np_refine - 1;
        const int rc = launch_fused_refine_pass(s, (unsigned)p.nblk, p.cos, p.np_refine > 1, p.rows, r);
        if (rc) return rc;
    }
    return 0;
}

struct SideFork {
    lshkm_ctx c;
    bool open = false;
    int fork() {
        if (hipEventRecord(c->fork_ev, c->stream) != hipSuccess ||
            hipStreamWaitEvent(c->side_stream, c->fork_ev, 0) != hipSuccess)
            return kstatus("fused_assign (fork)");
        open = true;
        return 0;
    }
    int end_side() {
        if (c->timing) {
            if (hipEventRecord(c->tev[2], c->side_stream) != hipSuccess) return kstatus("fused_assign (timing)");
            c->tev_side = true;
        }
        if (hipEventRecord(c->join_ev, c->side_stream) != hipSuccess) return kstatus("fused_assign (join)");
        return 0;
    }
    int join() {
        if (!open) return 0;
        if (hipStreamWaitEvent(c->stream, c->join_ev, 0) != hipSuccess) return kstatus("fused_assign (join)");
        open = false;
        return 0;
    }
    ~SideFork() { if (open) (void)hipStreamSynchronize(c->side_stream); }
};

#ifdef LSHKM_PHASE_TIMING
struct PhaseReport {
    hipStream_t s;
    unsigned long long* d = nullptr;
    explicit PhaseReport(hipStream_t s_) : s(s_) {
        static unsigned long long* prof_d = nullptr;
        if (!prof_d) (void)hipMalloc(&prof_d, 64);
        (void)hipMemsetAsync(prof_d, 0, 64, s);
        d = prof_d;
    }
    ~PhaseReport() {
        unsigned long long v[6];
        (void)hipMemcpyAsync(v, d, 48, hipMemcpyDeviceToHost, s);
        (void)hipStreamSynchronize(s);
        fprintf(stderr, "PHASES %llu %llu %llu %llu %llu\n", v[0], v[1], v[2], v[3], v[4]);
    }
};
#endif

}

int fused_assign(lshkm_ctx ctx, const AssignRequest& q) {
    hipStream_t s = ctx->stream;
    const bool cosine = q.metric != LSHKM_METRIC_EUCLIDEAN;
    const ProjTable* pj = q.lsh ? &q.lsh->proj : nullptr;
    const FusedRoute route = fused_route(cosine, q.X.f64, q.d, q.K, pj != nullptr, pj ? pj->k : 0, pj ? pj->LK : 0,
                                         test_switch("LSHKM_FUSED_FORM", "chunked"));
    if (route.form == FusedForm::none || (pj && (q.lsh->metric != q.metric || !pj->mfma_ok))) {
        set_error("fused_assign: no fused form runs this shape (fused_route, fused_layout.h)");
        return LSHKM_ERR_ARG;
    }
    FusedShape sh;
    sh.N = q.N; sh.d = q.d; sh.K = q.K; sh.cosine = cosine; sh.rows = route.rows;
    sh.hash = pj != nullptr; sh.LK = pj ? pj->LK : 0;
    sh.fast = !cosine && sh.rows != 2 && !q.force_exact && ctx->dist_mode == LSHKM_DIST_CERTIFIED;
    sh.image32 = sh.fast || (!cosine && sh.rows != 2 && sh.Kpad() <= 256 && !test_switch("LSHKM_GATHER32", "0"));
    sh.own_tuples = sh.hash && !cosine && !q.tuples;
    const bool pwfix = sh.pwfix();
    int rc;
    FusedWorkspace w;
    if ((rc = fused_workspace(ctx, sh, w))) return rc;
    LSHKM_HIP(hipMemsetAsync(w.cnt, 0, FUSED_COUNTER_CLEAR, s));
    if (ctx->timing) LSHKM_HIP(hipEventRecord(ctx->tev[0], s));
    ctx->tev_side = false;
    if ((rc = launch_fused_prep(s, q.C, q.K, q.d, cosine ? 1 : 0, w))) return rc;
    const bool xprep = exact_is_pruned(exact_form(q));
    if (xprep && (rc = exact_listed_prep(ctx, q))) return rc;
    if (w.xn2 && (rc = launch_row_sumsq(s, q.X.d(), q.N, q.d, w.xn2))) return rc;

    const FusedArgs common = fused_common_args(ctx, q, sh, w);
    RowList exact_rows;
    exact_rows.p = w.list1; exact_rows.count = w.cnt + CNT_AMBIG; exact_rows.bound = q.N;
    RecList dist_fix[2];
    int ndist_fix = 0;
    RecList pair_rows;
    SideFork side{ctx};
    if (q.N > 0 && route.form == FusedForm::chunked) {
        FusedArgs a = common;
        hash_outputs(a, q, sh, w);
        a.ambig = w.list1; a.ambig_count = w.cnt + CNT_AMBIG;
        if ((rc = launch_fused_chunked(s, sh.hash, a))) return rc;
    } else if (q.N > 0) {
        FusedPlan p;
        p.hash = sh.hash; p.cos = cosine; p.rows = sh.rows;
        int ncu = 0;
        if (device_cu_count(&ncu)) return LSHKM_ERR_HIP;
        p.nblk = fused_grid(q.N, ncu);
        p.seg_rows = fused_seg_rows(q.N, p.nblk);
        if (p.nblk > FUSED_MAX_SEGS) {
            set_error("fused_assign: more blocks than list segments");
            return LSHKM_ERR_ARG;
        }
        p.np_hi = (sh.Kpad() + FH_KMAX - 1) / FH_KMAX;
        p.np_refine = (sh.Kpad() + FP_KMAX - 1) / FP_KMAX;
        const RowList l1 = segmented(w.list1, w.cnt + CNT_REFINED, w.seg1, q, p);
        const RecList lh = segmented(w.hfix, w.cnt + CNT_HFIX, w.seg1, q, p);
        const RowList l2 = segmented(w.list2, w.cnt + CNT_AMBIG, w.seg2, q, p);
        FusedArgs seg = common;
        seg.seg_rows = p.seg_rows; seg.part = w.part;
#ifdef LSHKM_PHASE_TIMING
        PhaseReport report(s);
        seg.prof = report.d;
#endif
        FusedArgs hi = seg;
        hash_outputs(hi, q, sh, w);
        hi.ambig = l1.p; hi.ambig_count = l1.count; hi.seg_counts = l1.counts;
        if ((rc = fused_hi_passes(s, hi, p))) return rc;
        if (sh.hash) {
            const bool forked = ctx->side_init() == 0;
            if (forked && (rc = side.fork())) return rc;
            launch_hash_fixup(forked ? ctx->side_stream : s, lh, cosine, hi);
            if (forked && (rc = side.end_side())) return rc;
        }
        FusedArgs rf = seg;
        rf.list_in = l1.p; rf.list_counts = l1.counts; rf.list_seg_rows = l1.seg_rows;
        rf.ambig = l2.p; rf.ambig_count = l2.count; rf.seg_counts = l2.counts;
        rf.hfix = cosine ? w.hfix2 : hi.hfix; rf.hfix_count = cosine ? w.cnt + CNT_CFIX : hi.hfix_count;
        if (sh.pairs() && !test_switch("LSHKM_PAIR_PASS", "0")) {
            pair_rows = segmented(w.pairs, w.cnt + CNT_PAIR, w.seg2, q, p);
            rf.pairs = pair_rows.p; rf.pair_count = pair_rows.count;
        }
        if ((rc = fused_refine_passes(s, rf, p))) return rc;
        if (cosine && (rc = side.join())) return rc;
        if ((rc = kstatus("fused_hi_kernel"))) return rc;
        exact_rows = l2;        if (cosine || pwfix) dist_fix[ndist_fix++] = segmented(w.cfix, w.cnt + CNT_CFIX, w.seg3, q, p);
        if (cosine) dist_fix[ndist_fix++] = segmented(w.hfix2, w.cnt + CNT_CFIX, w.seg2, q, p);
    }
    if (ctx->timing) LSHKM_HIP(hipEventRecord(ctx->tev[1], s));
    if ((rc = exact_listed(ctx, q, exact_rows, !sh.fast, xprep, cosine ? w.xn2 : nullptr, cosine ? w.nbv : nullptr)))
        return rc;
    if ((rc = side.join())) return rc;
    {
        int di[5], n = 0;
        const unsigned long long* sp[5];
        di[n] = STAT_REFINED; sp[n++] = w.cnt + CNT_REFINED;
        if (sh.hash) { di[n] = STAT_HASH_FIX; sp[n++] = w.cnt + CNT_HFIX; }
        di[n] = STAT_ASSIGN_AMBIG; sp[n++] = w.cnt + CNT_AMBIG;
        if (pair_rows.bound > 0) {
            di[n] = STAT_ASSIGN_AMBIG; sp[n++] = w.cnt + CNT_PAIR;
            di[n] = STAT_PAIR_ROWS; sp[n++] = w.cnt + CNT_PAIR;
        }
        if ((rc = launch_add_counters(s, ctx->stats.as<unsigned long long>(), n, di, sp))) return rc;
    }
    if (cosine || pwfix) {
        if ((rc = launch_cos_fix_seg(s, q, ndist_fix, dist_fix, cosine ? w.xn2 : nullptr, cosine ? w.nbv : nullptr)))
            return rc;
        if ((rc = launch_add_counter(s, ctx->stats.as<unsigned long long>() + (cosine ? STAT_COS_FIX : STAT_POW_FIX),
                                     w.cnt + CNT_CFIX)))
            return rc;
    }
    return 0;
}

}
```

crypto-recommendation_amd/csrc/fused_args.h:

```cpp
#pragma once
#include <hip/hip_runtime.h>
#include <stdint.h>

#include "fused_layout.h"
#include "tile.h"

namespace lshkm {

struct FusedArgs {
    const float* X;
    int64_t N;
    const _Float16* Ch;
    const _Float16* Cl;
    const float* cnh;
    const float* cbound;
    const double* C64;
    int Kpad;
    const _Float16* Vh;
    const _Float16* Vl;
    const double* PT;
    const float* tv;
    const double* pnorm;
    const double* v1;
    const int32_t* rv;
    float w;
    int L, k, LK, LKpad;
    int64_t nb;
    int32_t* tuples;
    int32_t* phi;
    int32_t* bucket;
    int32_t* assign;
    double* dist;
    int32_t* ambig;
    unsigned long long* ambig_count;
    unsigned long long* hfix;
    unsigned long long* hfix_count;
    unsigned long long* cfix;
    int32_t* cfix_counts;
    unsigned long long* cfix_count;
    unsigned long long* stats;
    int64_t seg_rows;
    int32_t* seg_counts;
    BucketDiv bdiv;
    const double* nbv;
    const double* xn2;
    float4* part;
    int t0, pass_first, pass_last;
    const int32_t* list_in;
    const int32_t* list_counts;
    int64_t list_seg_rows;
    unsigned long long* prof;
    const float* C32;
    const float* rn32;
    int fast_dist;
    const double* X64;
    int d, xvec;
    const double* Cd;
    int pw_lds;
    unsigned long long* pairs;
    unsigned long long* pair_count;
    int K;
};

}
```

crypto-recommendation_amd/csrc/fused_layout.h:

```cpp
#pragma once
#include <algorithm>
#include <cstddef>
#include <cstdint>

namespace lshkm {

constexpr int FP_WAVES = 8;
constexpr int FH_WAVES_MIN = 8, FH_WAVES_MAX = 12;
constexpr int HMF_W = 4;
constexpr int HMF_BPC = 2;
constexpr int FP_KMAX = 256;
constexpr int FH_KMAX = 512;
constexpr int FUSED_DIMS = 128;

enum class FusedForm { none, hi, chunked };
struct FusedRoute {
    FusedForm form;
    int rows;
};
inline FusedRoute fused_route(bool cosine, bool f64, int d, int K, bool hash, int k, int LK, bool chunked_switch) {
    const bool hash_ok = !hash || (LK >= 1 && LK <= 32 && (!cosine || k == 4));
    if (!f64 && d == FUSED_DIMS && hash_ok) {
        if (!cosine) return {chunked_switch || (hash && k != 4) ? FusedForm::chunked : FusedForm::hi, 0};
        if (!chunked_switch) return {FusedForm::hi, 0};
    }
    if (!hash && d >= 1 && d <= FUSED_DIMS && K <= FH_KMAX) return {FusedForm::hi, f64 ? 2 : 1};
    return {FusedForm::none, 0};
}

constexpr int FUSED_MAX_SEGS = 1024;
constexpr int SEG_ROWS = 0, SEG_FIX = 1, SEG_SLOTS = 2;
constexpr size_t SEG_COUNTER_BYTES = (size_t)FUSED_MAX_SEGS * SEG_SLOTS * 4;
constexpr int64_t FUSED_LIST_SLACK = 32 + (int64_t)FUSED_MAX_SEGS * FH_WAVES_MAX * 32;
inline int64_t fused_list_cap(int64_t N) { return N + FUSED_LIST_SLACK; }
inline int64_t seg_rows_for(int64_t N, int nblk, int W) {
    const int64_t ntiles = (N + 31) / 32;
    return (int64_t)W * 32 * ((ntiles + (int64_t)nblk * W - 1) / ((int64_t)nblk * W));
}
inline int fused_grid(int64_t N, int ncu) {
    const int64_t want = ((N + 31) / 32 + FP_WAVES - 1) / FP_WAVES;
    return (int)std::max<int64_t>(1, std::min<int64_t>(ncu, want));
}
inline int64_t fused_seg_rows(int64_t N, int nblk) {
    int64_t r = 0;
    for (const int W : {FP_WAVES, FH_WAVES_MIN, FH_WAVES_MAX}) r = std::max(r, seg_rows_for(N, nblk, W));
    return r;
}
inline int hash_mfma_grid(int64_t N, int ncu) {
    const int64_t want = ((N + 31) / 32 + HMF_W - 1) / HMF_W;
    return (int)std::max<int64_t>(1, std::min<int64_t>((int64_t)ncu * HMF_BPC, want));
}
inline int64_t hash_mfma_seg_rows(int64_t N, int nblk) { return seg_rows_for(N, nblk, HMF_W); }

constexpr int64_t FUSED_PART_BYTES_PER_ROW = 32;
inline int64_t fused_part_bytes(int64_t N) {
    const int64_t tiles = std::max<int64_t>((N + 31) / 32, (fused_list_cap(N) + 31) / 32 + FUSED_MAX_SEGS);
    return tiles * 32 * FUSED_PART_BYTES_PER_ROW;
}

constexpr int CNT_AMBIG = 0;
constexpr int CNT_HFIX = 1;
constexpr int CNT_REFINED = 2;
constexpr int CNT_CFIX = 3;
constexpr int CNT_PAIR = 4;
constexpr size_t FUSED_COUNTER_BYTES = 64, FUSED_COUNTER_CLEAR = 40;

struct FusedShape {
    int64_t N = 0;
    int d = FUSED_DIMS, K = 0;
    bool cosine = false;
    int rows = 0;
    bool hash = false;
    int LK = 0;
    bool fast = false;
    bool image32 = false;
    bool own_tuples = false;
    int Kpad() const { return (K + 63) / 64 * 64; }
    bool pwfix() const { return !cosine && !fast; }
    bool pairs() const { return !cosine && Kpad() <= FP_KMAX; }
};
struct FusedLayout {
    static constexpr size_t NONE = ~(size_t)0;
    int64_t list_cap = 0;
    int64_t part_bytes = 0;
    size_t c16 = 0;
    size_t cconst = 0;
    size_t list1 = 0, list2 = 0;
    size_t seg1 = 0, seg2 = 0, seg3 = 0;
    size_t counter = 0;
    size_t fix = 0;
    size_t part = 0;
    size_t tuples = 0;
    size_t cf32 = 0;
    size_t c64p = 0;
    size_t xn2 = 0;
    size_t cl_off = 0, cnh_off = 0, nbv_off = 0, rn32_off = 0;
    size_t hfix_off = NONE, cfix_off = NONE, hfix2_off = NONE, pair_off = NONE;
};
inline FusedLayout fused_layout(const FusedShape& q) {
    FusedLayout l;
    const size_t Kpad = (size_t)q.Kpad(), D = FUSED_DIMS;
    const bool pwfix = q.pwfix();
    l.list_cap = fused_list_cap(q.N);
    const size_t cap = (size_t)l.list_cap, rows1 = (size_t)std::max<int64_t>(q.N, 1);
    l.c16 = Kpad * D * 2 * 2;
    l.cl_off = Kpad * D * 2;
    l.cconst = (Kpad + 8) * 4 + Kpad * 8;
    l.cnh_off = 8 * 4;
    l.nbv_off = (Kpad + 8) * 4;
    l.list1 = l.list2 = cap * 4;
    l.seg1 = l.seg2 = SEG_COUNTER_BYTES;
    l.counter = FUSED_COUNTER_BYTES;
    size_t regions = 0;
    if (q.hash || q.cosine || pwfix) regions++;
    if (q.hash || q.cosine) l.hfix_off = 0;
    if (q.cosine || pwfix) l.cfix_off = regions++ * cap * 8;
    if (q.cosine) l.hfix2_off = regions++ * cap * 8;
    if (q.pairs()) l.pair_off = regions++ * cap * 8;
    l.fix = regions * cap * 8;
    if (q.cosine || pwfix) l.seg3 = SEG_COUNTER_BYTES;
    if (Kpad > (size_t)FP_KMAX) l.part = (size_t)(l.part_bytes = fused_part_bytes(q.N));
    if (q.hash && !q.cosine && q.own_tuples) l.tuples = rows1 * (size_t)q.LK * 4;
    if (q.image32) {
        l.cf32 = Kpad * D * 4 + Kpad * 4;
        l.rn32_off = Kpad * D * 4;
    }
    if (q.rows != 0 && q.d != FUSED_DIMS) l.c64p = Kpad * D * 8;
    if (q.cosine && q.rows == 2) l.xn2 = rows1 * 8;
    return l;
}

struct HashLayout {
    int64_t list_cap = 0;
    size_t fix = 0, seg1 = 0, tuples = 0;
};
inline HashLayout hash_layout(int64_t N, int LK, bool own_tuples) {
    HashLayout l;
    l.list_cap = fused_list_cap(N);
    l.fix = (size_t)l.list_cap * 8;
    l.seg1 = SEG_COUNTER_BYTES;
    if (own_tuples) l.tuples = (size_t)N * (size_t)LK * 4;
    return l;
}

}
```

crypto-recommendation_amd/csrc/fused_refine.hip:

```cpp
#include "fused_impl.h"

namespace lshkm {

__device__ inline void split8p(const float* x, half8& hi, half8& lo) {
#pragma unroll
    for (int j = 0; j < 8; j += 2) {
        const half2v hp = {(_Float16)x[j], (_Float16)x[j + 1]};
        hi[j] = hp.x;
        hi[j + 1] = hp.y;
        const half2v lp = {(_Float16)resid_lo(x[j], hp), (_Float16)resid_hi(x[j + 1], hp)};
        lo[j] = lp.x;
        lo[j + 1] = lp.y;
    }
}

__device__ inline void tile_scores(const floatx16& acc_hi, const floatx16& acc_lo, const float* cn_tile_h,
                                   float (&sv)[16]) {
#pragma unroll
    for (int g = 0; g < 4; g++) {
        const float4 cn = *reinterpret_cast<const float4*>(cn_tile_h + 8 * g);
        const float2v h01 = {acc_hi[4 * g], acc_hi[4 * g + 1]}, l01 = {acc_lo[4 * g], acc_lo[4 * g + 1]};
        const float2v h23 = {acc_hi[4 * g + 2], acc_hi[4 * g + 3]}, l23 = {acc_lo[4 * g + 2], acc_lo[4 * g + 3]};
        const float2v c01 = {cn.x, cn.y}, c23 = {cn.z, cn.w};
        const float2v s01 = (h01 + l01) + c01, s23 = (h23 + l23) + c23;
        sv[4 * g] = s01.x; sv[4 * g + 1] = s01.y; sv[4 * g + 2] = s23.x; sv[4 * g + 3] = s23.y;
    }
}

__host__ __device__ constexpr int fp_lds_bytes(int Kpad) { return 16 + 2 * Kpad * FU_RS * 2 + Kpad * 4; }
static_assert(fp_lds_bytes(FP_KMAX) <= 160 * 1024, "refinement LDS image exceeds 160 KiB");

constexpr int FP_PAIR_REC = 16;
constexpr int FP_PAIR_RS = FU_D | 1;
__host__ __device__ constexpr int fp_pair_lds_bytes(int rows) {
    return 16 + FP_WAVES * FP_PAIR_REC * FP_PAIR_RS * (rows == 2 ? 8 : 4);
}
static_assert(fp_pair_lds_bytes(2) <= 160 * 1024, "pair staging exceeds 160 KiB");
__host__ __device__ inline unsigned long long pair_record(int64_t row, int i1, int i2) {
    return (unsigned long long)(uint32_t)row | ((unsigned long long)(uint32_t)i1 << 32) |
           ((unsigned long long)(uint32_t)i2 << 48);
}
template <int ROWS>
__device__ inline void pair_finish(const FusedArgs& a, const unsigned long long* recs, int total, char* lds,
                                   int wave, int lane) {
    using TX = std::conditional_t<ROWS == 2, double, float>;
    const TX* X;
    if constexpr (ROWS == 2) X = a.X64; else X = a.X;
    const int d = ROWS == 0 ? FU_D : a.d;
    TX* xs = reinterpret_cast<TX*>(lds) + wave * FP_PAIR_REC * FP_PAIR_RS;
    for (int base = wave * FP_PAIR_REC; base < total; base += FP_WAVES * FP_PAIR_REC) {
        const int i = base + (lane >> 1);
        const unsigned long long rec = recs[min(i, total - 1)];
        int64_t row = (int64_t)(uint32_t)rec;
        int c = (lane & 1) ? (int)(rec >> 48) : (int)((rec >> 32) & 0xFFFFu);
        if (lane >= 2 * FP_PAIR_REC || i >= total || row >= a.N) row = -1;
        if (row < 0 || c >= a.K) c = -1;
#pragma unroll 1
        for (int r0 = 0; r0 < FP_PAIR_REC && base + r0 < total; r0 += 8) {
            TX xv[8][FU_D / 64];
#pragma unroll
            for (int r = 0; r < 8; r++) {
                const int64_t rr = __shfl(row, 2 * (r0 + r));
#pragma unroll
                for (int u = 0; u < FU_D / 64; u++) {
                    const int j = lane + 64 * u;
                    xv[r][u] = j < d && rr >= 0 ? X[rr * d + j] : TX(0);
                }
            }
#pragma unroll
            for (int r = 0; r < 8; r++)
#pragma unroll
                for (int u = 0; u < FU_D / 64; u++) xs[(r0 + r) * FP_PAIR_RS + lane + 64 * u] = xv[r][u];
        }
        wave_sync();
        double best = 0.0;
        int bi = -1;
        pruned_pick_euclid<2>(xs + ((lane >> 1) & (FP_PAIR_REC - 1)) * FP_PAIR_RS, a.Cd, d, c, !a.fast_dist, best, bi);
        if (!(lane & 1) && bi >= 0) {
            a.assign[row] = bi;
            a.dist[row] = best;
        }
        wave_sync();
    }
}

template <int MET, bool MP, int ROWS>
__global__ __launch_bounds__(FP_THREADS, 1) void fused_persistent_kernel(FusedArgs a) {
    extern __shared__ __attribute__((aligned(16))) char smem[];
    const int Kpad = a.Kpad;
    constexpr bool PAIR = MET == 0 && !MP;
    int* lcount = reinterpret_cast<int*>(smem);
    _Float16* lch = reinterpret_cast<_Float16*>(smem + 16);
    _Float16* lcl = lch + Kpad * FU_RS;
    float* lcn = reinterpret_cast<float*>(lcl + Kpad * FU_RS);

    constexpr int FP_CU = 4;
    for (int e0 = 0; e0 < Kpad * 16; e0 += FP_THREADS * FP_CU) {
        float4 vh[FP_CU], vl[FP_CU];
#pragma unroll
        for (int u = 0; u < FP_CU; u++) {
            const int e = e0 + u * FP_THREADS + (int)threadIdx.x < Kpad * 16 ? e0 + u * FP_THREADS + (int)threadIdx.x : 0;
            const int r = e >> 4, g = e & 15;
            vh[u] = *reinterpret_cast<const float4*>(a.Ch + (size_t)r * FU_D + g * 8);
            vl[u] = *reinterpret_cast<const float4*>(a.Cl + (size_t)r * FU_D + g * 8);
        }
#pragma unroll
        for (int u = 0; u < FP_CU; u++) {
            const int e = e0 + u * FP_THREADS + (int)threadIdx.x < Kpad * 16 ? e0 + u * FP_THREADS + (int)threadIdx.x : 0;
            const int r = e >> 4, g = e & 15;
            *reinterpret_cast<float4*>(lch + r * FU_RS + g * 8) = vh[u];
            *reinterpret_cast<float4*>(lcl + r * FU_RS + g * 8) = vl[u];
        }
    }
    for (int e = threadIdx.x; e < Kpad; e += FP_THREADS) lcn[e] = a.cnh[e];
    if (threadIdx.x < 2) lcount[threadIdx.x] = 0;
    int32_t* ambig_seg = a.ambig + (int64_t)blockIdx.x * a.seg_rows;
    unsigned long long* hfix_seg = a.hfix + (int64_t)blockIdx.x * a.seg_rows;
    unsigned long long* pair_seg = PAIR && a.pairs ? a.pairs + (int64_t)blockIdx.x * a.seg_rows : nullptr;
    __syncthreads();

    const int lane = threadIdx.x & 63, wave = threadIdx.x >> 6;
    const int col = lane & 31, h = lane >> 5;
    const float ecf = a.cbound[0], ebf = a.cbound[1], cmaxf = a.cbound[3];
    const bool c_ok = __float_as_uint(a.cbound[2]) == 0u;
    const _Float16* my_h = lch + col * FU_RS + 8 * h;
    const _Float16* my_l = lcl + col * FU_RS + 8 * h;
    const int ntile32 = Kpad >> 5;
    const int32_t* lrows = a.list_in + (int64_t)blockIdx.x * a.list_seg_rows;
    const int64_t lcnt = (int64_t)a.list_counts[SEG_SLOTS * blockIdx.x + SEG_ROWS];
    const int64_t ptile0 = (int64_t)blockIdx.x * ((a.list_seg_rows + 31) >> 5);

    PT_DECL
    for (int64_t tile = wave; tile < (lcnt + 31) >> 5; tile += FP_WAVES) {
        const bool valid = tile * 32 + col < lcnt;
        const int64_t row = lrows[valid ? tile * 32 + col : lcnt - 1];
        const int64_t ptile = ptile0 + tile;

        float xf[64];
        if constexpr (ROWS != 0) {
            load_row_gen<ROWS>(a, valid ? row : a.N - 1, h, xf);
        } else {
            load_row_b(a.X + (valid ? row : a.N - 1) * FU_D + 8 * h, xf);
        }
        half8 bh[8], bl[8];
        float2v n2a = {0.f, 0.f}, n2b = {0.f, 0.f};
#pragma unroll
        for (int s = 0; s < 8; s++) {
            split8p(xf + 8 * s, bh[s], bl[s]);
#pragma unroll
            for (int j = 0; j < 8; j += 4) {
                const float2v u = {xf[8 * s + j], xf[8 * s + j + 1]}, v = {xf[8 * s + j + 2], xf[8 * s + j + 3]};
                n2a = __builtin_elementwise_fma(u, u, n2a);
                n2b = __builtin_elementwise_fma(v, v, n2b);
            }
        }
        float xn2f = (n2a.x + n2a.y) + (n2b.x + n2b.y);
        xn2f += __shfl_xor(xn2f, 32);
        const double xn2 = (double)xn2f * (1.0 + 0x1p-16);
        const double nx = sqrt(xn2);
        const double x1 = FU_SQRT_D * nx;
        const bool x_ok = xn2f <= FU_RANGE * FU_RANGE;

        PT_MARK(0)
        PT_MARK(1)
        const float E = MET == 0
            ? (float)(nx * (double)ecf + (double)ebf + FU_A2 * x1 + 0x1p-41 * xn2 +
                      0x1p-18 * (nx * (double)cmaxf + 0.5 * (double)cmaxf * (double)cmaxf) +
                      (ROWS == 2 ? 0x1p-24 * nx * (double)cmaxf : 0.0)) * (1.f + 0x1p-20f) + 1e-30f
            : (float)(nx * (double)ecf + (double)ebf + FU_A2 * x1 + 0x1p-41 * xn2 +
                      0x1p-18 * nx * (double)cmaxf + 0x1p-43 * nx) * (1.f + 0x1p-20f) + 1e-30f;
        float m1 = -__builtin_inff(), m2 = -__builtin_inff();
        int t1 = 0;
        Top3 top = {m1, m1, m1, 0, 0};
        if (MP && !a.pass_first) {
            const float4 st = a.part[ptile * 64 + lane];
            m1 = st.x; m2 = st.y; t1 = __float_as_int(st.z);
        }
        const int tg0 = MP ? a.t0 : 0;
        __builtin_amdgcn_s_setprio(MFMA_PRIO);
#pragma unroll 1
        for (int t = 0; t < ntile32; t++) {
            float sv[16];
            floatx16 acc_hi, acc_lo;
            tile_mfma(my_h + t * 32 * FU_RS, my_l + t * 32 * FU_RS, bh, bl, acc_hi, acc_lo);
            tile_scores(acc_hi, acc_lo, lcn + t * 32 + 4 * h, sv);
            if constexpr (PAIR) {
                tile_epilogue3(sv, t, top);
            } else {
                const float m1_prev = m1;
                tile_epilogue(sv, m1, m2);
                t1 = m1 != m1_prev ? t + tg0 : t1;
            }
        }
        __builtin_amdgcn_s_setprio(0);
        if constexpr (PAIR) { m1 = top.m1; m2 = top.m2; t1 = top.t1; }
        if (MP && !a.pass_last) {
            a.part[ptile * 64 + lane] = make_float4(m1, m2, __int_as_float(t1), 0.f);
            continue;
        }
        const uint32_t l1 = __float_as_uint(m1) & 0xFu;
        const int i1 = t1 * 32 + 8 * (int)(l1 >> 2) + 4 * h + (int)(l1 & 3u);
        const float om1 = __shfl_xor(m1, 32), om2 = __shfl_xor(m2, 32);
        const int oi1 = __shfl_xor(i1, 32);
        const float M2 = fmaxf(fmaxf(m2, om2), fminf(m1, om1));
        const int I1 = (om1 > m1 || (om1 == m1 && oi1 < i1)) ? oi1 : i1;
        const float M1 = fmaxf(m1, om1);
        const bool cert = x_ok && c_ok && ((double)M2 < (double)M1 - 2.0 * (double)E);
        bool pair = false;
        int I2 = 0;
        if constexpr (PAIR) {
            const uint32_t l2 = __float_as_uint(m2) & 0xFu;
            const int i2 = top.t2 * 32 + 8 * (int)(l2 >> 2) + 4 * h + (int)(l2 & 3u);
            const HalfTop me = {m1, m2, top.m3, i1, i2};
            const HalfTop ot = {om1, om2, __shfl_xor(top.m3, 32), oi1, __shfl_xor(i2, 32)};
            const PairMerge pm = I1 == i1 ? merge_halves(me, ot) : merge_halves(ot, me);
            I2 = pm.I2;
            pair = pair_seg && !cert && x_ok && c_ok && I1 != I2 && I1 < a.K && I2 < a.K &&
                   (double)pm.M3 < (double)M1 - 2.0 * (double)E;
        }

        PT_MARK(2)
        if constexpr (MET == 1) {
            bool fix = false;
            if (h == 1 && valid && cert) {
                a.assign[row] = I1;
                double v;
                bool okc;
                if constexpr (ROWS == 1) okc = cosine_fast_nb(a.X + row * a.d, a.Cd + (size_t)I1 * a.d, a.d, a.nbv[I1], v);
                else if constexpr (ROWS == 2) okc = cosine_fast_nb(a.X64 + row * a.d, a.Cd + (size_t)I1 * a.d, a.d, a.nbv[I1], v);
                else okc = cosine_fast_nb(a.X + row * FU_D, a.C64 + (size_t)I1 * FU_D, FU_D, a.nbv[I1], v);
                if (okc) a.dist[row] = v;
                else fix = true;
            }
            const unsigned long long fb = __ballot(fix);
            if (fb) {
                const int leader = __builtin_ctzll(fb);
                int base = 0;
                if (lane == leader) base = atomicAdd(lcount + 1, __popcll(fb));
                base = __shfl(base, leader);
                if (fix) hfix_seg[base + __popcll(fb & ((1ull << lane) - 1ull))] = (unsigned long long)row;
            }
        } else {
            const double* crow = a.C64 + (size_t)I1 * FU_D + 8 * h;
            double acc = 0.0;
            double2 cbuf[4];
            double2 xnext[4];
            const int64_t rowc = valid ? row : a.N - 1;
            if constexpr (ROWS == 2) load_x64_step(a, rowc, 0, h, xnext);
#pragma unroll
            for (int j = 0; j < 4; j++) cbuf[j] = *reinterpret_cast<const double2*>(crow + 2 * j);
#pragma unroll
            for (int s = 0; s < 8; s++) {
                double sq[8];
                double2 cur[4];
#pragma unroll
                for (int j = 0; j < 4; j++) cur[j] = cbuf[j];
                if (s + 1 < 8) {
#pragma unroll
                    for (int j = 0; j < 4; j++) cbuf[j] = *reinterpret_cast<const double2*>(crow + 16 * (s + 1) + 2 * j);
                }
                double2 xcur[4];
                if constexpr (ROWS == 2) {
#pragma unroll
                    for (int j = 0; j < 4; j++) xcur[j] = xnext[j];
                    if (s + 1 < 8) load_x64_step(a, rowc, s + 1, h, xnext);
                } else {
#pragma unroll
                    for (int j = 0; j < 4; j++) xcur[j] = make_double2((double)xf[8 * s + 2 * j], (double)xf[8 * s + 2 * j + 1]);
                }
#pragma unroll
                for (int j = 0; j < 4; j++) {
                    const double2 cc = cur[j];
                    const double d0 = __dsub_rn(xcur[j].x, cc.x);
                    const double d1 = __dsub_rn(xcur[j].y, cc.y);
                    sq[2 * j] = a.fast_dist ? __dmul_rn(d0, d0) : gp_sq(d0);
                    sq[2 * j + 1] = a.fast_dist ? __dmul_rn(d1, d1) : gp_sq(d1);
                }
                if (h == 0) {
#pragma unroll
                    for (int j = 0; j < 8; j++) acc = __dadd_rn(acc, sq[j]);
                }
                acc = take_from_lower(acc);
                if (h == 1) {
#pragma unroll
                    for (int j = 0; j < 8; j++) acc = __dadd_rn(acc, sq[j]);
                }
                acc = take_from_upper(acc);
            }
            if (h == 1 && valid && cert) {
                a.assign[row] = I1;
                a.dist[row] = sqrt(acc);
            }
        }
        PT_MARK(3)
        if constexpr (PAIR)
            seg_append(valid && pair && h == 1, pair_record(row, I1, I2), lcount + 1, pair_seg, lane);
        const bool amb = valid && !cert && !pair;
        const unsigned long long amask = __ballot(amb && h == 1);
        if (h == 1 && valid) {
            if (amb) {
                int base = 0;
                const int leader = __builtin_ctzll(amask);
                if (lane == leader) base = atomicAdd(lcount, __popcll(amask));
                base = __shfl(base, leader);
                const int rank = __popcll(amask & ((1ull << lane) - 1ull));
                ambig_seg[base + rank] = (int32_t)row;
            }
        }
        PT_MARK(4)
    }
    PT_FLUSH
    __syncthreads();
    if constexpr (PAIR) {
        if (pair_seg && lcount[1] > 0) pair_finish<ROWS>(a, pair_seg, lcount[1], smem + 16, wave, lane);
    }
    if (threadIdx.x < 2 && (!MP || (threadIdx.x == 0 ? a.pass_last != 0 : (MET == 1 && a.pass_last)))) {
        const int c = lcount[threadIdx.x];
        a.seg_counts[SEG_SLOTS * blockIdx.x + threadIdx.x] = c;
        if (c) atomicAdd(threadIdx.x == 0 ? a.ambig_count : MET == 1 ? a.hfix_count : a.pair_count, (unsigned long long)c);
    }
}

template <int MET, bool MP, int ROWS>
static void refine_launch(hipStream_t s, unsigned nblk, const FusedArgs& a) {
    const int lds = MET == 0 && !MP && a.pairs ? std::max(fp_lds_bytes(a.Kpad), fp_pair_lds_bytes(ROWS)) : fp_lds_bytes(a.Kpad);
    hipLaunchKernelGGL((fused_persistent_kernel<MET, MP, ROWS>), dim3(nblk), dim3(FP_THREADS), (size_t)lds, s, a);
}
template <int MET, bool MP>
static void refine_rows(hipStream_t s, unsigned nblk, int rows, const FusedArgs& a) {
    if (rows == 0) refine_launch<MET, MP, 0>(s, nblk, a);
    else if (rows == 1) refine_launch<MET, MP, 1>(s, nblk, a);
    else refine_launch<MET, MP, 2>(s, nblk, a);
}

int launch_fused_refine_pass(hipStream_t s, unsigned nblk, int metric, bool mp, int rows, const FusedArgs& a) {
    if (metric < 0 || metric > 1 || rows < 0 || rows > 2 || a.Kpad > FP_KMAX) {
        set_error("launch_fused_refine_pass: no kernel for this metric / row kind / slice");
        return -1;
    }
    if (metric == 1) mp ? refine_rows<1, true>(s, nblk, rows, a) : refine_rows<1, false>(s, nblk, rows, a);
    else mp ? refine_rows<0, true>(s, nblk, rows, a) : refine_rows<0, false>(s, nblk, rows, a);
    return 0;
}

}
```

crypto-recommendation_amd/csrc/fused_small.hip:

```cpp
#include "fused_impl.h"

namespace lshkm {

constexpr int HF_WAVES = 4;
constexpr int HF_SPLIT = 4;
constexpr int HF_G = 8;
constexpr int HF_SLOTS = 64 * HF_WAVES / HF_G;
constexpr int HF_XL = FU_D / HF_G;
constexpr int HF_PS = 33;
constexpr int HF_QS = HF_XL * HF_PS + 4;
constexpr size_t HF_LDS = (size_t)HF_G * HF_QS * 8 + 32 * (8 + 8 + 4);
__device__ inline int hf_pidx(int r) { return ((r >> 2) & 7) * HF_QS + (((r >> 5) << 2) | (r & 3)) * HF_PS; }

template <int CTRL>
__device__ inline uint32_t dpp_move(uint32_t v) {
    return (uint32_t)__builtin_amdgcn_mov_dpp((int)v, CTRL, 0xF, 0xF, false);
}
template <int CTRL>
__device__ inline double dpp_move(double v) {
    const uint64_t b = (uint64_t)__double_as_longlong(v);
    const uint64_t lo = dpp_move<CTRL>((uint32_t)b), hi = dpp_move<CTRL>((uint32_t)(b >> 32));
    return __longlong_as_double((long long)((hi << 32) | lo));
}
template <int CTRL>
__device__ inline float dpp_move(float v) { return __uint_as_float(dpp_move<CTRL>(__float_as_uint(v))); }
constexpr int QP_X1 = 0xB1, QP_X2 = 0x4E, HALF_MIRROR = 0x141;
template <typename T>
__device__ inline T group_sum(T v) {
    v += dpp_move<QP_X1>(v);
    v += dpp_move<QP_X2>(v);
    v += dpp_move<HALF_MIRROR>(v);
    return v;
}

__device__ __noinline__ int32_t fixup_floor_x87(const float* xrow, const double* pts, int f, double tt, float w) {
    return hash_x87_floor([&](int j) { return pts[hf_pidx(j) + f]; }, xrow, FU_D, tt, w);
}
__device__ __noinline__ int fixup_sign_x87(const float* xrow, const double* pts, int f) {
    return hash_x87_sign([&](int j) { return pts[hf_pidx(j) + f]; }, xrow, FU_D);
}

struct FixRow {
    int64_t row;
    uint32_t mask;
    float x[HF_XL];
    int32_t v[4];
};

struct alignas(4) Tup4 { int32_t v[4]; };

template <bool COS>
__device__ inline void fix_load(const FusedArgs& a, unsigned long long ent, int q, FixRow& r) {
    r.row = (int64_t)(ent >> 32);
    r.mask = (uint32_t)ent;
    const float* xq = a.X + r.row * FU_D + 4 * q;
#pragma unroll
    for (int u = 0; u < HF_XL / 4; u++) {
        const float4 v = *reinterpret_cast<const float4*>(xq + 32 * u);
        r.x[4 * u] = v.x; r.x[4 * u + 1] = v.y; r.x[4 * u + 2] = v.z; r.x[4 * u + 3] = v.w;
    }
    const int l = min(q, a.L - 1);
    if (COS) {
        r.v[0] = ((a.bucket ? a.bucket : a.phi) + r.row * a.L)[l];
    } else {
        const Tup4 v = reinterpret_cast<const Tup4*>(a.tuples + r.row * a.LK)[l];
#pragma unroll
        for (int j = 0; j < 4; j++) r.v[j] = v.v[j];
    }
}

template <bool COS>
__device__ inline void fix_row(const FusedArgs& a, const double* pts, const double* cpn, const double* ctt, int q,
                               FixRow& r) {
    float xs[4] = {0.f, 0.f, 0.f, 0.f};
#pragma unroll
    for (int j = 0; j < HF_XL; j++) xs[j & 3] = fmaf(r.x[j], r.x[j], xs[j & 3]);
    const float s = group_sum((xs[0] + xs[1]) + (xs[2] + xs[3]));
    const double nx = (double)__builtin_amdgcn_sqrtf(fmaf(s, 1.f + 0x1p-15f, 0x1p-118f)) * (1.0 + 0x1p-20);
    const float* xrow = a.X + r.row * FU_D;
    const int k = a.k;
    const double iwd = 1.0 / (double)a.w;
    for (uint32_t m = r.mask; m; m &= m - 1) {
        const int f = __builtin_ctz(m);
        const double* pq = pts + q * HF_QS + f;
        double aq[4] = {0.0, 0.0, 0.0, 0.0};
#pragma unroll
        for (int j = 0; j < HF_XL; j++) aq[j & 3] = fma(pq[j * HF_PS], (double)r.x[j], aq[j & 3]);
        const double acc = group_sum((aq[0] + aq[1]) + (aq[2] + aq[3]));
        const double P = cpn[f] * nx * (1.0 + 0x1p-40);
        if (COS) {
            int bit;
            if (!hash_decide_sign(acc, P, FU_D, bit)) {
                bit = fixup_sign_x87(xrow, pts, f);
                if (q == 0) atomicAdd(a.stats + STAT_HASH_EXACT, 1ull);
            }
            const int l = f / k, b = 1 << (k - 1 - (f - l * k));
            if (l == q) r.v[0] = bit ? (r.v[0] | b) : (r.v[0] & ~b);
        } else {
            const double tt = ctt[f], iw = iwd;
            const double y = (acc + tt) * iw;
            const double B = ((double)(FU_D + 2) * 0x1p-52 * (P + fabs(tt))) * (iw * (1.0 + 0x1p-50)) +
                             fabs(y) * 0x1p-50;
            const double lo = floor(y - B), hi = floor(y + B);
            int32_t hv = (int32_t)lo;
            if (!(lo == hi && fabs(lo) < 0x1p31)) {
                hv = fixup_floor_x87(xrow, pts, f, tt, a.w);
                if (q == 0) atomicAdd(a.stats + STAT_HASH_EXACT, 1ull);
            }
#pragma unroll
            for (int i = 0; i < 4; i++) r.v[i] = f == 4 * q + i ? hv : r.v[i];
        }
    }
}

__device__ inline void fix_settle(FixRow& r, unsigned long long& ent) {
    asm volatile("" : "+v"(r.row), "+v"(r.mask), "+v"(ent));
#pragma unroll
    for (int j = 0; j < HF_XL; j++) asm volatile("" : "+v"(r.x[j]));
#pragma unroll
    for (int j = 0; j < 4; j++) asm volatile("" : "+v"(r.v[j]));
}

template <bool COS>
__device__ inline void fix_store(const FusedArgs& a, const int32_t* crv, int q, const FixRow& r) {
    const int k = a.k;
    const uint32_t kmask = k >= 32 ? 0xFFFFFFFFu : ((1u << k) - 1u);
    const bool touched = q < a.L && (r.mask & (kmask << (q * k)));
    if (COS) {
        if (touched) {
            if (a.phi) a.phi[r.row * a.L + q] = r.v[0];
            if (a.bucket) a.bucket[r.row * a.L + q] = r.v[0];
        }
        return;
    }
    uint32_t hn = 0;
#pragma unroll
    for (int j = 0; j < 4; j++) hn += phi_term(r.v[j], crv[4 * q + j]);
    if (touched) {
        Tup4 v;
#pragma unroll
        for (int j = 0; j < 4; j++) v.v[j] = r.v[j];
        *reinterpret_cast<Tup4*>(a.tuples + r.row * a.LK + 4 * q) = v;
        const uint32_t ph = phi_final(hn);
        if (a.phi) a.phi[r.row * a.L + q] = (int32_t)ph;
        if (a.bucket) a.bucket[r.row * a.L + q] = bucket_fast(ph, a.bdiv);
    }
}

template <bool COS>
__global__ __launch_bounds__(64 * HF_WAVES) void hash_fixup_kernel(FusedArgs a) {
    extern __shared__ __attribute__((aligned(16))) char smem[];
    double* pts = reinterpret_cast<double*>(smem);
    double* cpn = pts + HF_G * HF_QS;
    double* ctt = cpn + 32;
    int32_t* crv = reinterpret_cast<int32_t*>(ctt + 32);
    const int nseg = gridDim.x / HF_SPLIT;
    const int seg = blockIdx.x % nseg, part = blockIdx.x / nseg;
    const int n = a.seg_counts[SEG_SLOTS * seg + SEG_FIX];
    if (n == 0) return;
    const unsigned long long* list = a.hfix + (int64_t)seg * a.seg_rows;
    const int LK = a.LK, LKpad = a.LKpad;
    {
        const int f = threadIdx.x & 31, fc = min(f, LKpad - 1);
        double pv[FU_D * 32 / (64 * HF_WAVES)];
#pragma unroll
        for (int i = 0; i < FU_D * 32 / (64 * HF_WAVES); i++)
            pv[i] = a.PT[((threadIdx.x >> 5) + i * (2 * HF_WAVES)) * LKpad + fc];
#pragma unroll
        for (int i = 0; i < FU_D * 32 / (64 * HF_WAVES); i++)
            pts[hf_pidx((threadIdx.x >> 5) + i * (2 * HF_WAVES)) + f] = f < LK ? pv[i] : 0.0;
    }
    if (threadIdx.x < 32) {
        const int f = threadIdx.x;
        cpn[f] = f < LK ? a.pnorm[f] : 0.0;
        ctt[f] = !COS && f < LK ? (double)a.tv[f] : 0.0;
        crv[f] = !COS && f < LK ? a.rv[f] : 0;
    }
    __syncthreads();
    const int q = threadIdx.x & (HF_G - 1), slot = threadIdx.x / HF_G;
    constexpr int STRIDE = HF_SPLIT * HF_SLOTS;
    int e = part * HF_SLOTS + slot;
    if (e >= n) return;
    FixRow cur, nxt;
    fix_load<COS>(a, list[e], q, cur);
    unsigned long long ent2 = list[min(e + STRIDE, n - 1)];
    fix_settle(cur, ent2);
    for (; e < n; e += STRIDE) {
        fix_load<COS>(a, ent2, q, nxt);
        ent2 = list[min(e + 2 * STRIDE, n - 1)];
        fix_row<COS>(a, pts, cpn, ctt, q, cur);
        fix_settle(nxt, ent2);
        fix_store<COS>(a, crv, q, cur);
        cur = nxt;
    }
}

void launch_hash_fixup(hipStream_t s, const RecList& l, bool cosine, FusedArgs a) {
    a.hfix = l.p; a.seg_counts = l.counts; a.seg_rows = l.seg_rows;
    const unsigned nseg = (unsigned)l.nseg;
    const dim3 grid(nseg * HF_SPLIT), block(64 * HF_WAVES);
    if (cosine) hipLaunchKernelGGL(hash_fixup_kernel<true>, grid, block, HF_LDS, s, a);
    else hipLaunchKernelGGL(hash_fixup_kernel<false>, grid, block, HF_LDS, s, a);
}

constexpr int FP_PREP_WAVES = 8;
__global__ void fused_centroid_prep(const double* __restrict__ C, int K, int Kpad, _Float16* __restrict__ Ch,
                                    _Float16* __restrict__ Cl, float* __restrict__ cnh, unsigned int* __restrict__ cb,
                                    int metric, double* __restrict__ nbv, float* __restrict__ C32,
                                    float* __restrict__ rn32, int d, double* __restrict__ C64p) {
    const int c = blockIdx.x * FP_PREP_WAVES + (threadIdx.x >> 6);
    const int lane = threadIdx.x & 63;
    double s2 = 0.0, s1 = 0.0;
    bool bad = false;
    double scale = 1.0;
    if (metric == 1) {
        double q = 0.0;
        for (int j = lane; j < FU_D; j += 64) {
            const double v = c < K && j < d ? C[(size_t)c * d + j] : 0.0;
            q = fma(v, v, q);
        }
        for (int off = 32; off >= 1; off >>= 1) q += __shfl_xor(q, off);
        if (c < K && !(q >= 1e-200 && q <= 1e200)) bad = true;
        scale = (q >= 1e-200 && q <= 1e200) ? 1.0 / sqrt(q) : 0.0;
        if (lane == 0 && c < K) {
            double b = 0.0;
            for (int j = 0; j < d; j++) {
                const double cj = C[(size_t)c * d + j];
                b = __dadd_rn(b, gp_sq(cj));
            }
            nbv[c] = b;
        }
    }
    bool not32 = false;
    bool tiny = false;
    double rr = 0.0, hh = 0.0;
    double r32 = 0.0;
    for (int j = lane; j < FU_D; j += 64) {
        const double raw = c < K && j < d ? C[(size_t)c * d + j] : 0.0;
        const double v = raw * scale;
        if (C64p) C64p[(size_t)c * FU_D + j] = raw;
        const float f = (float)v;
        not32 |= c < K && (double)f != v;
        tiny |= c < K && fabs(raw) < 0x1p-460 && raw != 0.0;
        if (C32) {
            C32[(size_t)c * FU_D + j] = f;
            const double e = v - (double)f;
            r32 = fma(e, e, r32);
        }
        const _Float16 hv = (_Float16)f;
        Ch[(size_t)c * FU_D + j] = hv;
        Cl[(size_t)c * FU_D + j] = (_Float16)(f - (float)hv);
        s2 = fma(v, v, s2);
        s1 += fabs(v);
        const double r = v - (double)hv;
        rr = fma(r, r, rr);
        hh = fma((double)hv, (double)hv, hh);
        bad |= !(fabs(v) <= (double)FU_RANGE);
    }
    for (int off = 32; off >= 1; off >>= 1) {
        s2 += __shfl_xor(s2, off);
        s1 += __shfl_xor(s1, off);
        rr += __shfl_xor(rr, off);
        hh += __shfl_xor(hh, off);
        r32 += __shfl_xor(r32, off);
    }
    if (rn32 && lane == 0) rn32[c] = r32 == 0.0 ? 0.f : (float)(sqrt(r32) * (1.0 + 0x1p-40)) * (1.f + 0x1p-22f);
    const unsigned long long anybad = __ballot(bad);
    const unsigned long long any_not32 = __ballot(not32);
    const unsigned long long any_tiny = __ballot(tiny);
    __shared__ unsigned int wmax[FP_PREP_WAVES][8];
    if (lane == 0) {
        unsigned int m[8] = {0u, 0u, 0u, 0u, 0u, 0u, 0u, 0u};
        m[7] = (any_not32 ? 1u : 0u) | (any_tiny ? 2u : 0u);
        if (c >= K) {
            cnh[c] = -0x1p100f;
        } else {
            cnh[c] = metric == 1 ? 0.f : (float)(-0.5 * s2);
            const double up = 1.0 + 0x1p-18;
            const double nc = sqrt(s2) * (1.0 + 0x1p-30);
            m[0] = __float_as_uint((float)((FU_A1 + 0x1p-22) * nc * up));
            m[1] = __float_as_uint((float)((FU_A2 * s1 * (1.0 + 0x1p-20) + (metric == 1 ? 0.0 : 0x1p-23 * s2) +
                                            0x1p-41 * s2) * up));
            m[2] = anybad ? 1u : 0u;
            m[3] = __float_as_uint((float)(nc * up));
            m[4] = __float_as_uint((float)(sqrt(rr) * (1.0 + 0x1p-30) * up));
            m[5] = __float_as_uint((float)(sqrt(hh) * (1.0 + 0x1p-30) * up));
            m[6] = __float_as_uint((float)(metric == 1 ? 0.0 : 0.5 * s2 * up));
        }
#pragma unroll
        for (int i = 0; i < 8; i++) wmax[threadIdx.x >> 6][i] = m[i];
    }
    __syncthreads();
    if (threadIdx.x < 8) {
        const int i = threadIdx.x;
        unsigned int v = 0u;
        for (int w = 0; w < FP_PREP_WAVES; w++) v = i == 2 || i == 7 ? (v | wmax[w][i]) : max(v, wmax[w][i]);
        if (v) {
            if (i == 2 || i == 7) atomicOr(cb + i, v);
            else atomicMax(cb + i, v);
        }
    }
}

int launch_fused_prep(hipStream_t s, const double* C, int K, int d, int metric, const FusedWorkspace& w) {
    const int Kpad = (K + 63) / 64 * 64;
    static_assert(64 % FP_PREP_WAVES == 0, "Kpad is a multiple of 64");
    (void)hipMemsetAsync(w.cbound, 0, 32, s);
    hipLaunchKernelGGL(fused_centroid_prep, dim3((unsigned)(Kpad / FP_PREP_WAVES)), dim3(64 * FP_PREP_WAVES), 0, s, C, K, Kpad, w.Ch, w.Cl, w.cnh,
                       reinterpret_cast<unsigned int*>(w.cbound), metric, w.nbv, w.C32, w.rn32, d, w.C64p);
    return kstatus("fused_centroid_prep");
}

constexpr int CF_SPLIT = 8;
struct CosLists {
    const unsigned long long* list[2];
    const int32_t* counts[2];
};
template <typename TX, int MET>
__global__ __launch_bounds__(256) void cos_fix_seg_kernel(const TX* __restrict__ X, int d, const double* __restrict__ C,
                                                          CosLists cl, int nseg, int64_t seg_rows,
                                                          const int32_t* __restrict__ assign, double* __restrict__ dist,
                                                          const double* __restrict__ xn2, const double* __restrict__ nbv) {
    const int per_list = nseg * CF_SPLIT;
    const int li = blockIdx.x / per_list, b = blockIdx.x % per_list;
    const int seg = b % nseg, part = b / nseg;
    const int n = cl.counts[li][SEG_SLOTS * seg + SEG_FIX];
    const unsigned long long* l = cl.list[li] + (int64_t)seg * seg_rows;
    const bool vec = sizeof(TX) == 4 && d % 8 == 0 && ((uintptr_t)X & 15) == 0 && ((uintptr_t)C & 15) == 0;
    __shared__ double sqs[4][64 * 16];
    double* sq = sqs[threadIdx.x >> 6];
    const int lane = threadIdx.x & 63;
    for (int i0 = part * 256 + (threadIdx.x & ~63); i0 < n; i0 += CF_SPLIT * 256) {
        const int i = i0 + lane;
        const bool live = i < n;
        const int64_t row = (int64_t)l[live ? i : i0];
        const TX* xr = X + row * d;
        const double* cr = C + (size_t)assign[row] * d;
        double v;
        if constexpr (MET == 1) {
            if (nbv && (sizeof(TX) == 4 || xn2)) {
                const double xa = sizeof(TX) == 4 ? -1.0 : xn2[row], cb = nbv[assign[row]];
                if (vec) v = exact_cosine_x87_pf<sizeof(TX) == 4>(xr, cr, d, xa, cb);
                else v = exact_cosine_x87_pf<false>(xr, cr, d, xa, cb);
            } else if (vec) {
                v = exact_cosine_x87_wave<sizeof(TX) == 4>(xr, cr, d, sq);
            } else {
                v = exact_cosine_x87_wave<false>(xr, cr, d, sq);
            }
        } else {
            if (vec) v = exact_euclid_wave<sizeof(TX) == 4>(xr, cr, d, sq);
            else v = exact_euclid_wave<false>(xr, cr, d, sq);
        }
        if (live) dist[row] = v;
    }
}

constexpr int RSQ_S = 10;
template <bool VEC>
__global__ __launch_bounds__(256) void row_sumsq_kernel(const double* __restrict__ X, int64_t N, int d,
                                                         double* __restrict__ out) {
    __shared__ double sqs[4][64 * 8];
    __shared__ __attribute__((aligned(16))) double tr[4][64 * RSQ_S];
    double* sq = sqs[threadIdx.x >> 6];
    double* t = tr[threadIdx.x >> 6];
    const int lane = threadIdx.x & 63;
    for (int64_t i0 = (int64_t)blockIdx.x * 256 + (threadIdx.x & ~63); i0 < N; i0 += (int64_t)gridDim.x * 256) {
        const int64_t i = i0 + lane;
        double a = 0.0;
        if constexpr (VEC) {
            double2 pc[4], pn[4];
            auto load = [&](int j0, double2 (&dst)[4]) {
#pragma unroll
                for (int k = 0; k < 4; k++) {
                    const int q = 64 * k + lane, r = q >> 2, part = q & 3;
                    const int64_t rr = i0 + r < N ? i0 + r : N - 1;
                    const int j = j0 + 2 * part;
                    dst[k] = j < d ? *reinterpret_cast<const double2*>(X + rr * d + j) : make_double2(0.0, 0.0);
                }
            };
            load(0, pn);
            for (int j0 = 0; j0 < d; j0 += 8) {
#pragma unroll
                for (int k = 0; k < 4; k++) pc[k] = pn[k];
                if (j0 + 8 < d) load(j0 + 8, pn);
#pragma unroll
                for (int k = 0; k < 4; k++) {
                    const int q = 64 * k + lane;
                    *reinterpret_cast<double2*>(t + (q >> 2) * RSQ_S + 2 * (q & 3)) = pc[k];
                }
                __builtin_amdgcn_fence(__ATOMIC_RELEASE, "wavefront");
                __builtin_amdgcn_wave_barrier();
                __builtin_amdgcn_fence(__ATOMIC_ACQUIRE, "wavefront");
                double v[8], p[8];
#pragma unroll
                for (int h = 0; h < 4; h++) {
                    const double2 w = *reinterpret_cast<const double2*>(t + lane * RSQ_S + 2 * h);
                    v[2 * h] = w.x;
                    v[2 * h + 1] = w.y;
                }
                __builtin_amdgcn_fence(__ATOMIC_RELEASE, "wavefront");
                __builtin_amdgcn_wave_barrier();
                __builtin_amdgcn_fence(__ATOMIC_ACQUIRE, "wavefront");
                gp_sq_wave<8>(v, p, sq);
#pragma unroll
                for (int u = 0; u < 8; u++)
                    if (j0 + u < d) a = __dadd_rn(a, p[u]);
            }
        } else {
            const double* x = X + (i < N ? i : N - 1) * d;
            for (int j0 = 0; j0 < d; j0 += 8) {
                double v[8], p[8];
#pragma unroll
                for (int u = 0; u < 8; u++) v[u] = j0 + u < d ? x[j0 + u] : 0.0;
                gp_sq_wave<8>(v, p, sq);
#pragma unroll
                for (int u = 0; u < 8; u++)
                    if (j0 + u < d) a = __dadd_rn(a, p[u]);
            }
        }
        if (i < N) out[i] = a;
    }
}

int launch_row_sumsq(hipStream_t s, const double* X, int64_t N, int d, double* out) {
    if (N <= 0) return 0;
    const unsigned grid = (unsigned)std::min<int64_t>((N + 255) / 256, 4096);
    if (d % 2 == 0 && ((uintptr_t)X & 15) == 0) hipLaunchKernelGGL(row_sumsq_kernel<true>, dim3(grid), dim3(256), 0, s, X, N, d, out);
    else hipLaunchKernelGGL(row_sumsq_kernel<false>, dim3(grid), dim3(256), 0, s, X, N, d, out);
    return kstatus("row_sumsq_kernel");
}

int launch_cos_fix_seg(hipStream_t s, const AssignJob& q, int nlists, const RecList* lists, const double* xn2,
                       const double* nbv) {
    const int nseg = nlists > 0 ? lists[0].nseg : 0;
    if (nseg <= 0) return 0;
    if (nlists > 2) return -1;
    const Pts X = q.X;
    const int d = q.d, metric = q.metric;
    const double* C = q.C;
    const int32_t* assign = q.assign;
    double* dist = q.dist;
    const int64_t seg_rows = lists[0].seg_rows;
    CosLists cl{};
    for (int i = 0; i < nlists; i++) { cl.list[i] = lists[i].p; cl.counts[i] = lists[i].counts; }
    const dim3 grid((unsigned)(nlists * nseg * CF_SPLIT));
#define CF_LAUNCH(TX, M, XP) hipLaunchKernelGGL((cos_fix_seg_kernel<TX, M>), grid, dim3(256), 0, s, XP, d, C, cl, nseg, seg_rows, assign, dist, xn2, nbv)
    if (metric == 1) {
        if (X.f64) CF_LAUNCH(double, 1, X.d()); else CF_LAUNCH(float, 1, X.f());
    } else {
        if (X.f64) CF_LAUNCH(double, 0, X.d()); else CF_LAUNCH(float, 0, X.f());
    }
#undef CF_LAUNCH
    return kstatus("cos_fix_seg_kernel");
}

}
```

crypto-recommendation_amd/csrc/index.h:

```cpp
#pragma once
#include <algorithm>
#include <hip/hip_runtime.h>
#include <stdint.h>

#include <vector>

#include "kernels.h"

namespace lshkm {

struct Buf {
    void* p = nullptr;
    size_t cap = 0;
    Buf() = default;
    Buf(const Buf&) = delete;
    Buf& operator=(const Buf&) = delete;
    ~Buf();
    int reserve(size_t bytes);
    template <typename T> T* as() const { return reinterpret_cast<T*>(p); }
};

struct ProjTable {
    int metric = 0, d = 0, L = 0, k = 0, LK = 0, LKpad = 0;
    float w = 0.f;
    Buf PT_d, t_d, pn_d, r_d;
    bool fused_ok = false;
    bool mfma_ok = false;
    Buf vh_d, vl_d, v1_d;
    std::vector<float> hV;
    int upload(hipStream_t s, int metric, int d, int L, int k, float w, const float* V, const float* t,
               const int32_t* r, const double* R);
    HashParams params(int64_t nb) const;
    HashMfmaParams mfma_params(int64_t nb) const;
};

}

struct lshkm_ctx_s;
struct lshkm_lsh_s;
struct lshkm_cube_s;
namespace lshkm {
int cube_vertices(lshkm_cube_s* cube, Pts X, int64_t N, int32_t* vertex);
int hash_rows(lshkm_ctx_s* ctx, int mode, Pts X, int64_t N, const ProjTable& pj, int64_t nb, int32_t* out_h,
              int32_t* out_phi, int32_t* out_bucket, int32_t* mm, bool* h16 = nullptr);
ExactForm exact_form(const AssignJob& q);
int exact_listed_prep(lshkm_ctx_s* ctx, const AssignJob& q);
int exact_listed(lshkm_ctx_s* ctx, const AssignJob& q, const RowList& l, bool exact_dist, bool prepped,
                 const double* xn2, const double* nbv);
struct AssignRequest : AssignJob {
    const ::lshkm_lsh_s* lsh = nullptr;
    int32_t *tuples = nullptr, *phi = nullptr, *bucket = nullptr;
    bool force_exact = false;
};
int fused_assign(lshkm_ctx_s* ctx, const AssignRequest& q);

}

struct lshkm_ctx_s {
    int device = 0;
    int dist_mode = 0;
    hipStream_t stream = nullptr;
    hipStream_t own_stream = nullptr;
    lshkm::Buf stats;
    lshkm::Buf ws_c32, ws_cconst, ws_ambig, ws_counter, ws_src, ws_hfix, ws_ct, ws_seg, ws_tuples, ws_part;
    lshkm::Buf ws_cf32, ws_c64p;
    lshkm::Buf ws_ambig2, ws_seg2;
    lshkm::Buf ws_seg3;
    lshkm::Buf ws_xn2;
    lshkm::Buf ws[16];
    lshkm::Buf ws_range[9];
    lshkm::Buf ws_sil_near;
    lshkm::Buf ws_sil_s;
    lshkm::Buf ws_long;
    lshkm::Buf ws_km;
    lshkm::Buf ws_km_seg;
    lshkm::Buf ws_scan;
    lshkm::Buf ws_pam[5];
    lshkm::Buf ws_call[10];
    lshkm::Buf ws_lshpc[7];
    lshkm::Buf ws_nearest[3];
    lshkm::Buf ws_knn;
    uint64_t ws_epoch = 0;
    bool timing = false;
    hipEvent_t tev[3] = {nullptr, nullptr, nullptr};
    bool tev_side = false;
    hipStream_t side_stream = nullptr;
    hipEvent_t fork_ev = nullptr, join_ev = nullptr;
    int side_init() {
        if (side_stream) return 0;
        if (hipStreamCreateWithFlags(&side_stream, hipStreamNonBlocking) != hipSuccess) return -2;
        if (hipEventCreateWithFlags(&fork_ev, hipEventDisableTiming) != hipSuccess ||
            hipEventCreateWithFlags(&join_ev, hipEventDisableTiming) != hipSuccess)
            return -2;
        return 0;
    }
    static constexpr int PIN_SLOTS = 4;
    void* pin_buf[PIN_SLOTS] = {};
    size_t pin_cap[PIN_SLOTS] = {};
    hipEvent_t pin_ev[PIN_SLOTS] = {};
    bool pin_used[PIN_SLOTS] = {};
    int pin_cur = -1;
    void* pinned = nullptr;
    hipEvent_t pinned_ev = nullptr;
    std::vector<int32_t> src_cache;
    void* src_cache_dev = nullptr;
    size_t src_cache_cap = 0;
    int pin_stage(size_t bytes) {
        const int i = (pin_cur + 1) % PIN_SLOTS;
        if (!pin_ev[i] && hipEventCreateWithFlags(&pin_ev[i], hipEventDisableTiming) != hipSuccess) return -2;
        if (pin_used[i]) (void)hipEventSynchronize(pin_ev[i]);
        if (bytes > pin_cap[i]) {
            if (pin_buf[i]) (void)hipHostFree(pin_buf[i]);
            pin_buf[i] = nullptr; pin_cap[i] = 0;
            if (hipHostMalloc(&pin_buf[i], bytes, hipHostMallocDefault) != hipSuccess) return -3;
            pin_cap[i] = bytes;
        }
        pin_cur = i;
        pin_used[i] = true;
        pinned = pin_buf[i];
        pinned_ev = pin_ev[i];
        return 0;
    }
    void* rb_buf = nullptr;
    size_t rb_cap = 0;
    void* ub_buf = nullptr;
    size_t ub_cap = 0;
    hipEvent_t ub_ev = nullptr;
    bool ub_pending = false;
    static int pin_grow(void*& b, size_t& cap, size_t bytes) {
        if (bytes <= cap) return 0;
        if (b) (void)hipHostFree(b);
        b = nullptr;
        cap = 0;
        const size_t nb = std::max<size_t>(bytes, 64 << 10);
        if (hipHostMalloc(&b, nb, hipHostMallocDefault) != hipSuccess) return -3;
        cap = nb;
        return 0;
    }
    ~lshkm_ctx_s() {
        if (rb_buf) (void)hipHostFree(rb_buf);
        if (ub_ev) {
            if (ub_pending) (void)hipEventSynchronize(ub_ev);
            (void)hipEventDestroy(ub_ev);
        }
        if (ub_buf) (void)hipHostFree(ub_buf);
        for (hipEvent_t& e : tev)
            if (e) (void)hipEventDestroy(e);
        if (side_stream) (void)hipStreamSynchronize(side_stream), (void)hipStreamDestroy(side_stream);
        if (fork_ev) (void)hipEventDestroy(fork_ev);
        if (join_ev) (void)hipEventDestroy(join_ev);
        for (int i = 0; i < PIN_SLOTS; i++) {
            if (pin_ev[i]) (void)hipEventSynchronize(pin_ev[i]), (void)hipEventDestroy(pin_ev[i]);
            if (pin_buf[i]) (void)hipHostFree(pin_buf[i]);
        }
    }
};

namespace lshkm {
struct D2H { void* dst; const void* src; size_t bytes; };
struct H2D { void* dst; const void* src; size_t bytes; };
int d2h_batch(lshkm_ctx_s* ctx, const D2H* r, int n);
int h2d_batch(lshkm_ctx_s* ctx, const H2D* r, int n);
}

struct lshkm_lsh_s {
    lshkm_ctx_s* ctx = nullptr;
    int metric = 0;
    int64_t nb = 0;
    lshkm::ProjTable proj;
    int built = 0;
    int64_t N = 0;
    lshkm::Buf tuples, bucket, row_ptr, idx;
    lshkm::Buf mt0;
    bool mt0_valid = false;
    bool q_valid = false;
    uint64_t q_epoch = 0;
    const void* q_Q = nullptr;
    bool q_f64 = false;
    const void* q_alias = nullptr;
    const int64_t* q_out_ptr = nullptr;
    int64_t q_nq = 0, q_total = 0;
    int q_filtered = 0;
};

struct lshkm_cube_s {
    lshkm_ctx_s* ctx = nullptr;
    int metric = 0;
    int k = 0;
    lshkm::ProjTable proj;
    int32_t hmin = 0, hspan = 0;
    lshkm::Buf memo, memo2, first_row;
    lshkm::Buf rng_d;
    lshkm::Buf mm, cnt;
    int built = 0;
    int64_t N = 0;
    lshkm::Buf vertex, row_ptr, idx;
};
```

crypto-recommendation_amd/csrc/kernels.h:

```cpp
#pragma once
#include <climits>
#include <hip/hip_runtime.h>
#include <stdint.h>

#include "exact_layout.h"
#include "fused_layout.h"
#include "recom_layout.h"

namespace lshkm {

struct Pts {
    const void* p = nullptr;
    bool f64 = false;
    Pts() = default;
    Pts(const float* x) : p(x), f64(false) {}
    Pts(const double* x) : p(x), f64(true) {}
    const float* f() const { return static_cast<const float*>(p); }
    const double* d() const { return static_cast<const double*>(p); }
    size_t esize() const { return f64 ? 8 : 4; }
    Pts row(int64_t r, int d) const {
        Pts q = *this;
        q.p = static_cast<const char*>(p) + (size_t)r * d * esize();
        return q;
    }
};
template <typename F>
inline void with_rows(Pts X, F&& f) {
    if (X.f64) f(X.d());
    else f(X.f());
}

struct AssignJob {
    Pts X;
    int64_t N = 0;
    int d = 0;
    const double* C = nullptr;
    int K = 0;
    int metric = 0;
    int32_t* assign = nullptr;
    double* dist = nullptr;
};

template <typename T>
struct DevList {
    static constexpr int slot = sizeof(T) == 4 ? SEG_ROWS : SEG_FIX;
    T* p = nullptr;
    unsigned long long* count = nullptr;
    int64_t bound = 0;
    int32_t* counts = nullptr;
    int64_t seg_rows = 0;
    int nseg = 0;
    const int32_t* seg_counts() const { return nseg > 0 ? counts : nullptr; }
};
using RowList = DevList<int32_t>;
using RecList = DevList<unsigned long long>;

enum HashMode {
    HM_LSH_EUCLID = 0,
    HM_LSH_COSINE = 1,
    HM_CUBE_EUCLID_H = 2,
    HM_CUBE_COSINE = 3,
};

struct HashParams {
    const double* PT;
    const float* t;
    const double* pnorm;
    const int32_t* r;
    float w;
    int d, L, k, LK, LKpad;
    int64_t nb;
};
int hash_fb(int LK);
int hash_lkpad(int LK);

int launch_proj_hash(hipStream_t s, int mode, Pts X, int64_t N, const HashParams& p,
                     int32_t* out_h, int32_t* out_phi, int32_t* out_bucket,
                     unsigned long long* stats);

struct HashMfmaParams {
    const _Float16* Vh;
    const _Float16* Vl;
    const float* t;
    const double* pnorm;
    const double* v1;
    const int32_t* r;
    const double* PT;
    float w;
    int d, L, k, LK, LKpad;
    int64_t nb;
};
int launch_hash_mfma(hipStream_t s, int mode, const float* X, int64_t N, const HashMfmaParams& p, int32_t* out_h,
                     int32_t* out_phi, int32_t* out_bucket, int32_t* mm, const RecList& list,
                     unsigned long long* stats, int h16 = 0);

int assign_dp(int d);
int launch_centroid_prep(hipStream_t s, const double* C, int K, int Kpad, int d, int DP, int metric, bool xf64,
                         float* C32, float* cconst);
int launch_assign_mfma(hipStream_t s, Pts X, int64_t N, int d, int DP, const double* C, int K,
                       int Kpad, int metric, const float* C32, const float* cconst, int32_t* assign, double* dist,
                       int32_t* ambig, unsigned long long* ambig_count);
int launch_cos_fix(hipStream_t s, Pts X, int64_t N, int d, const double* C, const int32_t* rows,
                   const unsigned long long* count, const int32_t* assign, double* dist);
int launch_exact_prep(hipStream_t s, const AssignJob& q, ExactForm form, void* ws);
int launch_exact_pass(hipStream_t s, const AssignJob& q, const RowList& l, ExactForm form, const void* ws,
                      bool exact_dist, const double* xn2, const double* nbv);
int launch_assign_override(hipStream_t s, const int32_t* src_rows, int K, int64_t N, int32_t* assign,
                           double* dist);

int launch_add_counter(hipStream_t s, unsigned long long* dst, const unsigned long long* src);
int launch_add_counters(hipStream_t s, unsigned long long* stats, int n, const int* dst_idx,
                        const unsigned long long* const* src);

size_t sort_scratch_bytes(int64_t N, int64_t range, int T = 1);
int pow_contract_check();

int sort_pairs_small(hipStream_t s, const int32_t* keys, const int32_t* vals, int64_t n, int32_t* keys_out,
                     int32_t* vals_out, const unsigned int* n_dev = nullptr);
int stable_sort_by_key(hipStream_t s, const int32_t* keys, int64_t kstride, const int32_t* vals, int64_t N,
                       int64_t range, int32_t* keys_out, int32_t* vals_out, void* scratch);
int launch_csr_bounds(hipStream_t s, const int32_t* sorted_keys, int64_t N, int64_t nb, int64_t* row_ptr, int T = 1);
int stable_sort_by_key_batched(hipStream_t s, const int32_t* keys, int64_t kstride, int64_t key_ts, const int32_t* vals,
                               int64_t val_ts, int T, int64_t N, int64_t range, int32_t* keys_out, int32_t* vals_out,
                               void* scratch);

size_t scan_ws_bytes(int64_t M);
int launch_scan_i64(hipStream_t s, const int64_t* a, int64_t M, int64_t* out, int64_t* scratch = nullptr);
int launch_lsh_query(hipStream_t s, const int32_t* qbucket, const int32_t* qtuple, const int32_t* alias, int64_t nq,
                     int L, int k, int64_t nb, int filtered, int64_t N, const int32_t* tuples, const int32_t* bucket,
                     const int64_t* row_ptr, const int32_t* idx, int64_t* sizes, int64_t* cand_off,
                     int32_t* klist, int64_t* kcount, int64_t* qsz, int64_t* out_ptr, int32_t* out, int phase,
                     int64_t* scan_ws = nullptr, const int32_t* mt0 = nullptr);
int launch_lsh_gather_t0(hipStream_t s, const int32_t* tuples, const int32_t* idx, int64_t N, int L, int k, int32_t* mt0);
int launch_cube_query(hipStream_t s, const int32_t* qvert, int64_t nq, const int32_t* masks, int S,
                      const int64_t* row_ptr, const int32_t* idx, int64_t* sizes, int64_t* slot_off,
                      int64_t* out_ptr, int32_t* out, int64_t* scan_ws = nullptr);

int launch_h_minmax(hipStream_t s, const int32_t* h, int64_t n, int32_t* mm_dev);
int launch_coin_first(hipStream_t s, const void* h, bool h16, int64_t N, int k, int32_t hmin, int32_t hspan,
                      const int32_t* memo, int32_t* first_row);
int launch_coin_collect(hipStream_t s, int32_t* first_row, int64_t total, int k, int32_t hspan, int32_t* keys,
                        int32_t* vals, unsigned int* count);
int launch_coin_draw(hipStream_t s, const int32_t* sorted_vals, const unsigned int* count, int32_t hmin, int32_t hspan,
                     int32_t* memo, uint32_t* state);
int launch_coin_vertex(hipStream_t s, const void* h, bool h16, int64_t N, int k, int32_t hmin, int32_t hspan,
                       const int32_t* memo, int32_t* vertex);
int launch_memo_rehome(hipStream_t s, const int32_t* old_memo, int32_t old_min, int32_t old_span, int32_t* new_memo,
                       int32_t new_min, int32_t new_span, int k);
int launch_memo_scatter(hipStream_t s, const int32_t* off, const int32_t* bit, int64_t n, int32_t* memo);

int launch_km_chain(hipStream_t s, Pts X, int d, const int32_t* rows, const int64_t* crow, int K,
                    double* sums, int64_t* counts, const double* carry = nullptr,
                    const int64_t* carry_counts = nullptr, const int* flag = nullptr);
size_t km_seg_ws_bytes(int64_t M, int K, int d);
constexpr size_t KM_SEG_WS_CAP = (size_t)8 << 30;
int launch_km_sums_seg(hipStream_t s, Pts X, int d, const int32_t* rows, const int64_t* crow, int K, int64_t M,
                       double* sums, int64_t* counts, const double* carry, const int64_t* carry_counts, void* ws,
                       const int* flag = nullptr);
size_t km_fx_ws_bytes(int K, int d);
int launch_km_sums_fx(hipStream_t s, Pts X, int d, const int32_t* rows, const int64_t* crow, int K, int64_t M,
                      double* sums, int64_t* counts, const double* carry, const int64_t* carry_counts, void* ws,
                      unsigned long long* stat = nullptr, void* seg_ws = nullptr);
size_t km_shard_ws_bytes(int64_t M, int K, int d);
int launch_km_shard_begin(hipStream_t s, Pts X, int d, const int32_t* rows, const int64_t* crow, int K, int64_t M,
                          double* sums, double* asum, int32_t* qt, int64_t* counts, void* ws);
int launch_km_shard_certify(hipStream_t s, const double* gathered, int world, int rank, const double* asum,
                            const int32_t* qt, const int64_t* counts, int K, int d, double* sums_out, double* start,
                            int* flag, uint8_t* mask, unsigned long long* nflag);
int launch_km_shard_prepare(hipStream_t s, Pts X, int d, const int32_t* rows, const int64_t* crow, int K, int64_t M,
                            const double* start, const int* flag, const uint8_t* mask, void* ws);
int launch_km_shard_chain(hipStream_t s, Pts X, int d, const int32_t* rows, const int64_t* crow, int K, int64_t M,
                          const int* flag, const uint8_t* mask, const double* carry, void* ws, double* sums);
size_t seg_columns_ws_bytes(int64_t n, int K, int m);
int launch_seg_iota(hipStream_t s, int32_t* iota, int64_t n);
int launch_seg_columns(hipStream_t s, const double* V, int64_t n, int K, int m, const int32_t* iota,
                       const int64_t* crow, const double* carry, double* out, void* ws);
int launch_grid_bits(hipStream_t s, Pts X, int64_t n, int* qt);
bool grid_exact_squares(const int* qt_host);
int launch_km_finalize(hipStream_t s, const double* sums, const int64_t* counts, int K, int d, const double* C_old,
                       int metric, double min_dist, double* C_new, int* moved);

int launch_kmeans_pp(hipStream_t s, Pts X, int64_t N, int d, int K, int metric, const double* canon,
                     int32_t* chosen, void* ws, unsigned long long* stats);
int launch_kpp_shard_dist(hipStream_t s, Pts X, int64_t n, int d, int metric, const void* crow, int it, void* ws);
int launch_kpp_shard_units(hipStream_t s, int64_t n, unsigned long long gmax_bits, double start, void* ws);
int launch_kpp_shard_chain(hipStream_t s, int64_t n, double s_in, void* ws, unsigned long long* stats);
int launch_kpp_shard_pick(hipStream_t s, int64_t n, double rd, int owns_row0, void* ws);

int launch_rc_norms(hipStream_t s, const double* X, int64_t N, int d, double* xa);
struct RecomJob {
    Pts X;
    const double* x_mean;
    int64_t N;
    int d;
    const int64_t* crow;
    const int32_t* crows;
    int K;
    Pts U;
    const double* u_mean;
    int64_t nq;
    const int32_t* ucl;
    const int64_t* unk_ptr;
    const int32_t* unk_idx;
};
struct RecomCarry {
    double *main, *abs;
    int64_t* cnt;
};
struct RecomOut {
    double* pred;
    int32_t* pidx;
    int n_top;
    int32_t* out;
};
int launch_rc_cluster_top_n(hipStream_t s, const RecomJob& j, double* scratch, const RcWaveScratch& ws,
                            const RecomOut& o, unsigned long long* soft_count);
struct RcGroups {
    const int32_t* ioff;
    int ngroups;
    int64_t nitems;
    const int32_t* gcl;
    const int32_t* gptr;
    const int32_t* gusr;
    void* items;
    int64_t nusers;
    void* users;
};
struct RcTermsOut {
    const int64_t *soff, *toff;
    int64_t total;
    double *sims, *terms;
};
int launch_rc_terms(hipStream_t s, const RecomJob& j, const RcTermsOut& t, char* map, const RcGroups& groups,
                    unsigned long long* soft_count);
struct RcLong {
    const RcLongUser* tab;
    int64_t nlong, rows;
    int D;
    const int64_t* crow;
    double *V, *carry, *sums;
    int32_t* iota;
    void* ws;
};
int launch_rc_chain_terms(hipStream_t s, const RecomJob& j, const RcTermsOut& t, const RecomCarry& in,
                          const RecomCarry& out, double* pred, int64_t long_min);
int launch_rc_long(hipStream_t s, const RcTermsOut& t, const RecomCarry& in, const double* u_mean,
                   const RecomCarry& out, double* pred, const RcLong& lng);
int launch_rc_top(hipStream_t s, const RecomJob& j, const int64_t* soff, const int64_t* carry_cnt, const RecomOut& o);
int launch_rc_shard_sims(hipStream_t s, const RecomJob& j, const int64_t* soff, double* sims,
                         unsigned long long* soft_count);
int launch_rc_shard_chain(hipStream_t s, const RecomJob& j, const int64_t* soff, const double* sims,
                          const RecomCarry& in, const RecomCarry& out, const RecomOut& o);
int launch_rc_p_closest(hipStream_t s, const double* X, const double* xa, int d, const double* U, int64_t nq,
                        const int64_t* cand_ptr, const int32_t* cand_idx, int P, double* sim, double* key,
                        int32_t* pos, int32_t* out_idx, double* out_sim, int32_t* out_cnt, int32_t* replay,
                        unsigned int* replay_count, bool replay_pass = true);
int launch_rc_top_n(hipStream_t s, const double* X, const double* x_mean, int d, const double* u_mean, int64_t nq,
                    const int64_t* unk_ptr, const int32_t* unk_idx, const int32_t* nb_idx, const double* nb_sim,
                    const int32_t* nb_cnt, int P, int n_top, double* pred, int32_t* pidx, int32_t* out);

int launch_cv_gather(hipStream_t s, const double* X, const double* x_mean, const int32_t* rows, int64_t M, int d,
                     double* W, double* w_mean);
int launch_cv_hide(hipStream_t s, const double* X, const double* x_mean, const int32_t* rows, int64_t M, int d,
                   const int64_t* unk_ptr, const int32_t* unk_idx, const int32_t* draw, double* H, double* h_mean,
                   int32_t* hide_idx, double* old);
int launch_cv_exclude(hipStream_t s, const int64_t* in_ptr, const int32_t* in_idx, int64_t nq, int32_t lo, int32_t hi,
                      int64_t* cnt, int32_t* run_a, int32_t* run_b, int64_t* out_ptr, int32_t* out_idx);
int launch_cv_predict(hipStream_t s, const double* X, const double* x_mean, int d, const double* u_mean, int64_t nq,
                      int64_t entries, const int64_t* unk_ptr, const int32_t* unk_idx, const int32_t* nb_idx,
                      const double* nb_sim, const int32_t* nb_cnt, int P, double* pred);
int launch_cv_fold_sum(hipStream_t s, int64_t F, const int32_t* hide_idx, const double* old, const double* pred,
                       const int64_t* nb_ptr, double* err, double* k_sum_out, int64_t* cnt_out, bool carry);

int launch_range_radius(hipStream_t s, const double* C, int K, int d, int metric, double* r0,
                        unsigned long long* tmp);
int launch_range_pairs(hipStream_t s, const int64_t* comb_ptr, const int32_t* comb_idx, int K, int32_t* rows,
                       int32_t* cents);
int launch_range_init(hipStream_t s, int64_t N, int32_t* assign, double* dist);
int launch_range_pass(hipStream_t s, Pts X, int d, const double* C, int K, int metric, const int32_t* key,
                      const int64_t* vptr, const int32_t* cents, double* cache, int8_t* cached, int64_t N,
                      const double* r0, int64_t pass, int32_t* assign, double* dist, unsigned long long* count);
int launch_range_unassigned(hipStream_t s, const int32_t* assign, int64_t N, int32_t* list,
                            unsigned long long* count);
int launch_range_gather(hipStream_t s, Pts X, int d, const int32_t* list, int64_t M, void* Xr);
int launch_range_scatter(hipStream_t s, const int32_t* list, int64_t M, const int32_t* ar, const double* dr,
                         int32_t* assign, double* dist);

int launch_sil_near(hipStream_t s, const double* C, int K, int d, int metric, int32_t* near);
int launch_sil_points(hipStream_t s, Pts X, int d, int metric, const int32_t* rows, const int64_t* crow,
                      const int32_t* assign, const int32_t* near, int64_t N, double* s_out, bool exsq = false);
int launch_sil_sum(hipStream_t s, const double* sv, const int32_t* rows, const int64_t* crow, int K, int64_t N,
                   double* raw, double* out);

int launch_pam_check_assign(hipStream_t s, const int32_t* assign, int64_t N, int K, int* bad);
constexpr int PAM_SCREEN_DMAX = 128;
constexpr int PAM_SCREEN_COLS = 128;
int launch_pam_prep(hipStream_t s, Pts X, int d, const int32_t* rows, const int32_t* assign, int64_t N, double* n2,
                    float* rho, int* cbad, unsigned long long* cmax);
int launch_pam_screen(hipStream_t s, Pts X, int d, const int32_t* rows, const int64_t* crow, const int2* items,
                      int64_t nitems, const double* n2, const float* rho, double* St, double* Et,
                      const unsigned long long* cmax, unsigned long long* Sfix, unsigned long long* Efix);
int launch_pam_mark(hipStream_t s, const int64_t* crow, int K, const int32_t* screen, const int* cbad,
                    const double* St, const double* Et, const unsigned long long* cmax,
                    const unsigned long long* Sfix, const unsigned long long* Efix, uint8_t* flag, int64_t* cnt,
                    unsigned long long* stats);
int launch_pam_compact(hipStream_t s, const int64_t* crow, int K, const uint8_t* flag, const int64_t* coff,
                       int32_t* cand);
int launch_pam_exact(hipStream_t s, Pts X, int d, int metric, const int32_t* rows, const int64_t* crow,
                     const int32_t* assign, const int32_t* cand, const int64_t* m_dev, int64_t N, double* sums,
                     bool exsq);
int launch_pam_select(hipStream_t s, const int32_t* rows, const int32_t* cand, const int64_t* coff, int K,
                      const double* sums, int32_t* med, double* csum);
int launch_pam_gather(hipStream_t s, Pts X, int d, const int32_t* med, int K, const double* C_old, double* C_new);

struct LshpcSide {
    const float* xh;
    const uint32_t* code;
    const float* inv;
    const float* rel;
    int64_t n;
};
struct LshpcKept {
    float *klo, *khi;
    int32_t *krow, *state;
    int64_t np, seg_rows;
    int cap, segs;
};
int launch_lshpc_prep(hipStream_t s, const double* X, int64_t n, int d, int dp, const double* xa, const int32_t* bucket,
                      int L, int k, const LshpcSide& out);
int launch_lshpc_screen(hipStream_t s, int dp, const LshpcSide& rows, const LshpcSide& users, int32_t excl_lo,
                        int32_t excl_hi, int P, int L, int k, const LshpcKept& kept);
struct CubeProbe;
int launch_cubepc_screen(hipStream_t s, int dp, const LshpcSide& rows, const LshpcSide& users, int P,
                         const CubeProbe& probe, const LshpcKept& kept);
int launch_cubepc_handed(hipStream_t s, const int32_t* vertex, const int32_t* list, int64_t m, const int32_t* masks,
                         int S, const int64_t* row_ptr, int32_t* vg, int64_t* ncand);
int launch_lshpc_join(hipStream_t s, const LshpcKept& kept, int64_t n, int P, int64_t* nkept, int64_t* ncand,
                      int64_t* cptr, int32_t* cidx, unsigned long long* stats);
int launch_lshpc_collect(hipStream_t s, const LshpcKept& kept, int64_t n, int64_t u0, const int32_t* replay,
                         const unsigned int* replay_count, int32_t* handed, unsigned int* handed_count);
int launch_lshpc_stats(hipStream_t s, unsigned long long* stats, int64_t settled, int64_t lists);
int launch_lshpc_gather(hipStream_t s, const double* U, int d, const int32_t* list, int64_t m, double* Ug);
int launch_lshpc_scatter(hipStream_t s, const int32_t* list, int64_t m, int P, const int32_t* gidx, const double* gsim,
                         const int32_t* gcnt, const int64_t* eptr, int32_t* out_idx, double* out_sim, int32_t* out_cnt,
                         int64_t* ncand);

struct NearestSide {
    const float* xh;
    const float* a;
    const float* rel;
    int64_t n;
};
struct NearestKept {
    uint32_t* minkey;
    int32_t *cnt, *krow;
    int64_t seg_rows;
    int cap;
};
int launch_nearest_prep(hipStream_t s, Pts X, int64_t n, int d, int dp, int metric, const NearestSide& out, int32_t* pois,
                        unsigned int* npois);
int launch_nearest_screen(hipStream_t s, int dp, int metric, const NearestSide& rows, const NearestSide& qs,
                          const NearestKept& kept, int64_t tiles, int segs);
int launch_nearest_settle(hipStream_t s, Pts X, Pts Q, int64_t nq, int d, int metric, const int64_t* ptr,
                          const int32_t* idx, const NearestKept& kept, const float* qa, const int32_t* pois,
                          const unsigned int* npois, const double* xn2, const double* qn2, double* dist, int32_t* row,
                          unsigned long long* stats);
int launch_nearest_collect(hipStream_t s, const NearestKept& kept, const float* qa, int64_t nq, int32_t* list,
                           unsigned int* count, unsigned long long* stats);
int launch_nearest_scan(hipStream_t s, Pts X, int64_t N, Pts Q, int64_t nq, int d, int metric, const int32_t* list,
                        const unsigned int* count, const double* xn2, const double* qn2, double* dist, int32_t* row,
                        unsigned long long* stats);
bool nearest_needs_norms(Pts X, int metric);
int launch_nearest_norms(hipStream_t s, Pts X, int64_t n, int d, int metric, double* xa);
int launch_nearest_empty(hipStream_t s, int64_t nq, double* dist, int32_t* row);
int launch_nearest_check(hipStream_t s, const int64_t* ptr, int64_t nq, const int32_t* idx, int64_t total, int64_t N,
                         unsigned int* bad);

struct KnnKept {
    uint32_t *gkey, *tau;
    int32_t *cnt, *krow;
    int64_t seg_rows;
    int groups, grp_shift, cap, k;
};
int launch_knn_screen(hipStream_t s, int dp, int metric, const NearestSide& rows, const NearestSide& qs,
                      const KnnKept& kept, int64_t tiles, int segs);
int launch_knn_settle(hipStream_t s, Pts X, Pts Q, int64_t nq, int d, int metric, int k, const int64_t* ptr,
                      const int32_t* idx, const KnnKept& kept, const float* qa, const int32_t* pois,
                      const unsigned int* npois, const double* xn2, const double* qn2, int32_t* row, double* dist,
                      int32_t* cnt, unsigned long long* stats);
int launch_knn_collect(hipStream_t s, const KnnKept& kept, const float* qa, int64_t nq, int32_t* list,
                       unsigned int* count, unsigned long long* stats);
int launch_knn_scan(hipStream_t s, Pts X, int64_t N, Pts Q, int64_t nq, int d, int metric, int k, const int32_t* list,
                    const unsigned int* count, const double* xn2, const double* qn2, int32_t* row, double* dist,
                    int32_t* cnt, unsigned long long* stats);
int launch_knn_empty(hipStream_t s, int64_t nq, int k, int32_t* row, double* dist, int32_t* cnt);

struct UvVisits {
    const int32_t *tw, *grp;
    int64_t V;
    const double* score;
    const int64_t* ci_ptr;
    const int32_t* ci_idx;
    int64_t T, G;
    int C;
};
int launch_uv_check(hipStream_t s, const UvVisits& q, bool coins, uint32_t* flag);
int launch_uv_count(hipStream_t s, const UvVisits& q, int64_t* cnt);
size_t uv_sort_bytes(int64_t E, int64_t nkeys);
int launch_uv_sums(hipStream_t s, const UvVisits& q, const int64_t* off, int64_t E, const double* carry_sum,
                   const uint8_t* carry_known, int32_t* keys, int32_t* vals, int32_t* keys_s, int32_t* vals_s,
                   void* sort_ws, int64_t* row_ptr, int32_t* long_list, uint32_t* long_count, double* sum,
                   uint8_t* known);
int launch_uv_finish(hipStream_t s, const double* sum, const uint8_t* known, int64_t G, int C, int64_t* kept,
                     int64_t* nunk, int64_t* row_off, int64_t* unk_off, double* mean, int64_t* scan_ws, double* U,
                     double* mean_out, int64_t* unk_ptr, int32_t* unk_idx, int32_t* src);

int launch_synth(hipStream_t s, uint64_t seed, int64_t row0, int64_t rows, int d, float* X, int kind = 0);

}
```

crypto-recommendation_amd/csrc/pick.h:

```cpp
#pragma once
#include "exact.h"

namespace lshkm {

template <typename TX>
__device__ __attribute__((always_inline)) inline double exact_euclid_rolled(const TX* __restrict__ x,
                                                                            const double* __restrict__ c, int d) {
    double acc = 0.0;
#pragma unroll 1
    for (int j = 0; j < d; j++) acc = __dadd_rn(acc, gp_sq(__dsub_rn((double)x[j], c[j])));
    return sqrt(acc);
}

template <typename TX>
__device__ inline double euclid_sumsq_mul(const TX* __restrict__ x, const double* __restrict__ c, int d, PwAcc& pw) {
    double acc = 0.0;
    for (int j0 = 0; j0 < d; j0 += 16) {
        double cv[16];
#pragma unroll
        for (int t = 0; t < 16; t++) cv[t] = j0 + t < d ? c[j0 + t] : 0.0;
#pragma unroll
        for (int t = 0; t < 16; t++)
            if (j0 + t < d) {
                const double df = __dsub_rn((double)x[j0 + t], cv[t]);
                const double p = __dmul_rn(df, df);
                pw.add<true>(df);
                acc = __dadd_rn(acc, p);
            }
    }
    return acc;
}

template <int G>
__device__ inline void group_argmin(double& best, int& bi) {
#pragma unroll
    for (int off = G / 2; off >= 1; off >>= 1) {
        const double ob = __shfl_xor(best, off);
        const int oi = __shfl_xor(bi, off);
        const bool take = oi >= 0 && (bi < 0 || ob < best || (ob == best && oi < bi));
        if (take) { best = ob; bi = oi; }
    }
}
template <int G>
__device__ inline double group_min(double v) {
#pragma unroll
    for (int off = G / 2; off >= 1; off >>= 1) v = fmin(v, __shfl_xor(v, off));
    return v;
}

template <int G, typename TX>
__device__ inline void pruned_pick_euclid(const TX* __restrict__ xr, const double* __restrict__ C, int d, int c,
                                          bool exact_dist, double& best, int& bi) {
    PwAcc pw;
    const double S = c >= 0 ? euclid_sumsq_mul(xr, C + (size_t)c * d, d, pw) : 0.0;
    const bool hard = c >= 0 && pw.hard();
    best = c >= 0 ? sqrt(S) : 0.0;
    bi = c;
    group_argmin<G>(best, bi);
    int anyh = hard ? 1 : 0;
#pragma unroll
    for (int off = G / 2; off >= 1; off >>= 1) anyh |= __shfl_xor(anyh, off);
    if (!anyh) return;
    const double S1 = group_min<G>(c >= 0 && c == bi ? S : __builtin_inf());
    const double S2 = group_min<G>(c >= 0 && c != bi ? S : __builtin_inf());
    if (S2 != __builtin_inf() && !(S2 - S1 > 0x1p-41 * S2)) {
        best = c >= 0 ? exact_euclid_rolled(xr, C + (size_t)c * d, d) : 0.0;
        bi = c;
        group_argmin<G>(best, bi);
        return;
    }
    if (!exact_dist) return;
    const int w = bi;
    double v = __builtin_inf();
    if (c == w) v = hard ? exact_euclid_rolled(xr, C + (size_t)c * d, d) : best;
    best = group_min<G>(v);
}

}
```

Measured before the change: 5.494 billion point hash+assign ops/s.

## Settle ambiguous rows inside refinement pass and fuse epilogue counters/override

Ambiguous rows are resolved in place inside the pair-refinement kernel: the kernel recomputes MFMA tiles to build a candidate mask and picks the exact argmin right away. This removes the separate ambiguous-row list and the exact pass over it. The counter adds, the counter and bound clears and the source-row override are merged into one epilogue kernel, and memsets are skipped when the workspace is known clean from the previous call. In exchange the refine kernel does extra MFMA and exact fp64 work per wave that has ambiguous rows, which can add divergence and register pressure.

```diff
diff --git a/crypto-recommendation_amd/csrc/api.cpp b/crypto-recommendation_amd/csrc/api.cpp
--- a/crypto-recommendation_amd/csrc/api.cpp
+++ b/crypto-recommendation_amd/csrc/api.cpp
@@ -617,6 +617,7 @@
         (rc = ctx->ws_counter.reserve(64)))
         return rc;
     unsigned long long* cnt = (unsigned long long*)ctx->ws_counter.p;
+    ctx->ws_dirty();
     LSHKM_HIP(hipMemsetAsync(cnt, 0, 16, s));
     if ((rc = launch_centroid_prep(s, q.C, q.K, Kpad, q.d, DP, q.metric, q.X.f64, (float*)ctx->ws_c32.p, (float*)ctx->ws_cconst.p))) return rc;
     if ((rc = launch_assign_mfma(s, q.X, N, q.d, DP, q.C, q.K, Kpad, q.metric, (const float*)ctx->ws_c32.p, (const float*)ctx->ws_cconst.p,
@@ -628,6 +629,24 @@
         ((rc = launch_cos_fix(s, q.X, N, q.d, q.C, (const int32_t*)ctx->ws_ambig.p + N, cnt + 1, q.assign, q.dist)) ||
          (rc = launch_add_counter(s, (unsigned long long*)ctx->stats.p + STAT_COS_FIX, cnt + 1)))) return rc;
     return launch_add_counter(s, (unsigned long long*)ctx->stats.p + STAT_ASSIGN_AMBIG, cnt);
+}
+
+static int stage_override(lshkm_ctx ctx, const int32_t* src_rows_host, int K) {
+    hipStream_t s = ctx->stream;
+    int rc;
+    if ((rc = ctx->ws_src.reserve((size_t)K * 4))) return rc;
+    const bool same = ctx->src_cache_dev == ctx->ws_src.p && ctx->src_cache_cap == ctx->ws_src.cap &&
+                      ctx->src_cache.size() == (size_t)K &&
+                      std::memcmp(ctx->src_cache.data(), src_rows_host, (size_t)K * 4) == 0;
+    if (same) return 0;
+    if ((rc = ctx->pin_stage((size_t)K * 4))) return rc;
+    std::memcpy(ctx->pinned, src_rows_host, (size_t)K * 4);
+    LSHKM_HIP(hipMemcpyAsync(ctx->ws_src.p, ctx->pinned, (size_t)K * 4, hipMemcpyHostToDevice, s));
+    LSHKM_HIP(hipEventRecord(ctx->pinned_ev, s));
+    ctx->src_cache.assign(src_rows_host, src_rows_host + K);
+    ctx->src_cache_dev = ctx->ws_src.p;
+    ctx->src_cache_cap = ctx->ws_src.cap;
+    return 0;
 }
 
 static int assign_impl(lshkm_ctx ctx, Pts X, int64_t N, int d, const double* C, int K, int metric,
@@ -644,30 +663,20 @@
                                          X, N, lsh->proj, lsh->nb,
                                          lsh->metric == LSHKM_METRIC_EUCLIDEAN ? tuples : nullptr, phi, bucket,
                                          nullptr))) { LSHKM_LAUNCH_CHECK(); return rc; }
-    if (path == 0 || path == 3) rc = fused_assign(ctx, q);
-    else if (path == 1) rc = assign_f32_mfma(ctx, q);
+    const bool fused = path == 0 || path == 3;
+    if (src_rows_host && (rc = stage_override(ctx, src_rows_host, K))) return rc;
+    if (fused) {
+        if (src_rows_host) q.src_dev = (const int32_t*)ctx->ws_src.p;
+        rc = fused_assign(ctx, q);
+    } else if (path == 1) rc = assign_f32_mfma(ctx, q);
     else {
         RowList all;
         all.bound = N;
         rc = launch_exact_pass(s, q, all, ExactForm::every, nullptr, true, nullptr, nullptr);
     }
     if (rc) { LSHKM_LAUNCH_CHECK(); return rc; }
-    if (src_rows_host) {
-        if ((rc = ctx->ws_src.reserve((size_t)K * 4))) return rc;
-        const bool same = ctx->src_cache_dev == ctx->ws_src.p && ctx->src_cache_cap == ctx->ws_src.cap &&
-                          ctx->src_cache.size() == (size_t)K &&
-                          std::memcmp(ctx->src_cache.data(), src_rows_host, (size_t)K * 4) == 0;
-        if (!same) {
-            if ((rc = ctx->pin_stage((size_t)K * 4))) return rc;
-            std::memcpy(ctx->pinned, src_rows_host, (size_t)K * 4);
-            LSHKM_HIP(hipMemcpyAsync(ctx->ws_src.p, ctx->pinned, (size_t)K * 4, hipMemcpyHostToDevice, s));
-            LSHKM_HIP(hipEventRecord(ctx->pinned_ev, s));
-            ctx->src_cache.assign(src_rows_host, src_rows_host + K);
-            ctx->src_cache_dev = ctx->ws_src.p;
-            ctx->src_cache_cap = ctx->ws_src.cap;
-        }
-        if ((rc = launch_assign_override(s, (const int32_t*)ctx->ws_src.p, K, N, assign, dist))) { LSHKM_LAUNCH_CHECK(); return rc; }
-    }
+    if (src_rows_host && !fused &&
+        (rc = launch_assign_override(s, (const int32_t*)ctx->ws_src.p, K, N, assign, dist))) { LSHKM_LAUNCH_CHECK(); return rc; }
     return 0;
 }
 
diff --git a/crypto-recommendation_amd/csrc/assign.hip b/crypto-recommendation_amd/csrc/assign.hip
--- a/crypto-recommendation_amd/csrc/assign.hip
+++ b/crypto-recommendation_amd/csrc/assign.hip
@@ -306,10 +306,8 @@
 }
 
 constexpr int OV_LDS_MAX = 8192;
-__global__ __launch_bounds__(1024) void assign_override_lds_kernel(const int32_t* __restrict__ src, int K, int64_t N,
-                                                                  int32_t* __restrict__ assign,
-                                                                  double* __restrict__ dist) {
-    __shared__ __attribute__((aligned(16))) int32_t ls[OV_LDS_MAX + 16];
+__device__ inline void override_lds(const int32_t* __restrict__ src, int K, int64_t N, int32_t* __restrict__ assign,
+                                    double* __restrict__ dist, int32_t* ls) {
     const int Kp = (K + 15) & ~15;
     for (int c = threadIdx.x; c < Kp + 16; c += blockDim.x) ls[c] = c < K ? src[c] : -1;
     __syncthreads();
@@ -333,6 +331,12 @@
         }
     }
 }
+__global__ __launch_bounds__(1024) void assign_override_lds_kernel(const int32_t* __restrict__ src, int K, int64_t N,
+                                                                  int32_t* __restrict__ assign,
+                                                                  double* __restrict__ dist) {
+    __shared__ __attribute__((aligned(16))) int32_t ls[OV_LDS_MAX + 16];
+    override_lds(src, K, N, assign, dist, ls);
+}
 
 int launch_assign_override(hipStream_t s, const int32_t* src_rows, int K, int64_t N, int32_t* assign,
                            double* dist) {
@@ -376,4 +380,42 @@
     return kstatus("assign.hip");
 }
 
-}
+constexpr int EPI_THREADS = 256, EPI_THREADS_MAX = 1024;
+__global__ __launch_bounds__(EPI_THREADS_MAX) void fused_epilogue_kernel(unsigned long long* stats, CounterAdds c,
+                                                                     unsigned long long* cnt, int ncnt,
+                                                                     unsigned int* cb, int ncb,
+                                                                     const int32_t* __restrict__ src, int K, int64_t N,
+                                                                     int32_t* __restrict__ assign,
+                                                                     double* __restrict__ dist) {
+    extern __shared__ __attribute__((aligned(16))) int32_t epi_ls[];
+    if ((int)threadIdx.x < c.n) atomicAdd(stats + c.dst[threadIdx.x], *c.src[threadIdx.x]);
+    __syncthreads();
+    if ((int)threadIdx.x < ncnt) cnt[threadIdx.x] = 0ull;
+    if ((int)threadIdx.x < ncb) cb[threadIdx.x] = 0u;
+    if (src) override_lds(src, K, N, assign, dist, epi_ls);
+}
+
+int launch_fused_epilogue(hipStream_t s, unsigned long long* stats, int n, const int* dst_idx,
+                          const unsigned long long* const* srcs, unsigned long long* cnt, int ncnt, unsigned int* cb,
+                          int ncb, const int32_t* src_rows, int K, int64_t N, int32_t* assign, double* dist) {
+    if (n > 8 || ncnt > EPI_THREADS || ncb > EPI_THREADS) {
+        set_error("launch_fused_epilogue: at most 8 counters and 256 words to zero");
+        return -1;
+    }
+    CounterAdds c;
+    c.n = n;
+    for (int i = 0; i < n; i++) { c.dst[i] = dst_idx[i]; c.src[i] = srcs[i]; }
+    const bool own_launch = src_rows && K > OV_LDS_MAX;
+    const int32_t* src = own_launch ? nullptr : src_rows;
+    const size_t lds = src ? ((size_t)((K + 15) & ~15) + 16) * 4 : 0;
+    const int threads = src ? std::min(EPI_THREADS_MAX, std::max(EPI_THREADS, (K + 63) / 64 * 64)) : EPI_THREADS;
+    hipLaunchKernelGGL(fused_epilogue_kernel, dim3(1), dim3(threads), lds, s, stats, c, cnt, ncnt, cb, ncb, src, K, N,
+                       assign, dist);
+    if (own_launch) {
+        const int rc = kstatus("fused_epilogue_kernel");
+        return rc ? rc : launch_assign_override(s, src_rows, K, N, assign, dist);
+    }
+    return kstatus("fused_epilogue_kernel");
+}
+
+}
diff --git a/crypto-recommendation_amd/csrc/exact_pass.hip b/crypto-recommendation_amd/csrc/exact_pass.hip
--- a/crypto-recommendation_amd/csrc/exact_pass.hip
+++ b/crypto-recommendation_amd/csrc/exact_pass.hip
@@ -4,6 +4,7 @@
 #include "kernels.h"
 #include "exact.h"
 #include "pick.h"
+#include "settle.h"
 
 namespace lshkm {
 
@@ -69,14 +70,6 @@
     wave_sync();
 }
 
-template <typename F>
-__device__ inline void every_centroid(int K, F&& dd, double& best, int& bi) {
-    for (int c = threadIdx.x & 63; c < K; c += 64) {
-        const double v = dd(c);
-        if (bi < 0 ? (v == v || c == 0) : v < best) { best = v; bi = c; }
-    }
-}
-
 template <typename TX>
 __device__ inline bool cosine_nonfinite_row(const TX* x, int d, double& best, int& bi) {
     bool bad = false;
@@ -85,15 +78,6 @@
     best = __longlong_as_double((long long)0xFFF8000000000000ull);
     bi = 0;
     return true;
-}
-
-__device__ inline void wave_store(double best, int bi, int64_t row, int32_t* __restrict__ assign,
-                                  double* __restrict__ dist) {
-    group_argmin<64>(best, bi);
-    if ((threadIdx.x & 63) == 0) {
-        assign[row] = bi < 0 ? 0 : bi;
-        dist[row] = bi < 0 ? -1.0 : best;
-    }
 }
 
 constexpr int XC_MAXV = 4;
@@ -346,22 +330,6 @@
         ncand += __popcll(cm[i]);
     }
     return __all(finite) && ncand >= 1;
-}
-
-template <int NCH>
-__device__ inline int kth_candidate(const unsigned long long (&cm)[NCH], int k) {
-    int c = -1, seen = 0;
-#pragma unroll
-    for (int i = 0; i < NCH; i++) {
-        const int n = __popcll(cm[i]);
-        if (c < 0 && k >= seen && k < seen + n) {
-            unsigned long long m = cm[i];
-            for (int t = k - seen; t > 0; t--) m &= m - 1;
-            c = 64 * i + __builtin_ctzll(m);
-        }
-        seen += n;
-    }
-    return c;
 }
 
 template <int MET, typename TX, int NCH>
diff --git a/crypto-recommendation_amd/csrc/fused.hip b/crypto-recommendation_amd/csrc/fused.hip
--- a/crypto-recommendation_amd/csrc/fused.hip
+++ b/crypto-recommendation_amd/csrc/fused.hip
@@ -185,6 +185,8 @@
 
 int fused_assign(lshkm_ctx ctx, const AssignRequest& q) {
     hipStream_t s = ctx->stream;
+    const lshkm_ctx_s::WsClean was_clean = ctx->ws_clean;
+    ctx->ws_dirty();
     const bool cosine = q.metric != LSHKM_METRIC_EUCLIDEAN;
     const ProjTable* pj = q.lsh ? &q.lsh->proj : nullptr;
     const FusedRoute route = fused_route(cosine, q.X.f64, q.d, q.K, pj != nullptr, pj ? pj->k : 0, pj ? pj->LK : 0,
@@ -203,11 +205,18 @@
     int rc;
     FusedWorkspace w;
     if ((rc = fused_workspace(ctx, sh, w))) return rc;
-    LSHKM_HIP(hipMemsetAsync(w.cnt, 0, FUSED_COUNTER_CLEAR, s));
+    const bool clean = was_clean.cnt == w.cnt && was_clean.cnt_cap == ctx->ws_counter.cap && was_clean.cb == w.cbound &&
+                       was_clean.cb_cap == ctx->ws_cconst.cap;
+    if (!clean) {
+        LSHKM_HIP(hipMemsetAsync(w.cnt, 0, FUSED_COUNTER_CLEAR, s));
+        LSHKM_HIP(hipMemsetAsync(w.cbound, 0, FUSED_CBOUND_BYTES, s));
+    }
     if (ctx->timing) LSHKM_HIP(hipEventRecord(ctx->tev[0], s));
     ctx->tev_side = false;
     if ((rc = launch_fused_prep(s, q.C, q.K, q.d, cosine ? 1 : 0, w))) return rc;
-    const bool xprep = exact_is_pruned(exact_form(q));
+    const bool pair_pass = q.N > 0 && route.form != FusedForm::chunked && sh.pairs() && !test_switch("LSHKM_PAIR_PASS", "0");
+    const bool settle = pair_pass && !test_switch("LSHKM_SETTLE", "0");
+    const bool xprep = !settle && exact_is_pruned(exact_form(q));
     if (xprep && (rc = exact_listed_prep(ctx, q))) return rc;
     if (w.xn2 && (rc = launch_row_sumsq(s, q.X.d(), q.N, q.d, w.xn2))) return rc;
 
@@ -259,9 +268,10 @@
         rf.list_in = l1.p; rf.list_counts = l1.counts; rf.list_seg_rows = l1.seg_rows;
         rf.ambig = l2.p; rf.ambig_count = l2.count; rf.seg_counts = l2.counts;
         rf.hfix = cosine ? w.hfix2 : hi.hfix; rf.hfix_count = cosine ? w.cnt + CNT_CFIX : hi.hfix_count;
-        if (sh.pairs() && !test_switch("LSHKM_PAIR_PASS", "0")) {
+        if (pair_pass) {
             pair_rows = segmented(w.pairs, w.cnt + CNT_PAIR, w.seg2, q, p);
             rf.pairs = pair_rows.p; rf.pair_count = pair_rows.count;
+            rf.settle = settle ? 1 : 0;
         }
         if ((rc = fused_refine_passes(s, rf, p))) return rc;
         if (cosine && (rc = side.join())) return rc;
@@ -270,12 +280,18 @@
         if (cosine) dist_fix[ndist_fix++] = segmented(w.hfix2, w.cnt + CNT_CFIX, w.seg2, q, p);
     }
     if (ctx->timing) LSHKM_HIP(hipEventRecord(ctx->tev[1], s));
-    if ((rc = exact_listed(ctx, q, exact_rows, !sh.fast, xprep, cosine ? w.xn2 : nullptr, cosine ? w.nbv : nullptr)))
+    if (!settle &&
+        (rc = exact_listed(ctx, q, exact_rows, !sh.fast, xprep, cosine ? w.xn2 : nullptr, cosine ? w.nbv : nullptr)))
         return rc;
-    if ((rc = side.join())) return rc;
+    const bool dist_lists = cosine || pwfix;
+    if (dist_lists) {
+        if ((rc = side.join())) return rc;
+        if ((rc = launch_cos_fix_seg(s, q, ndist_fix, dist_fix, cosine ? w.xn2 : nullptr, cosine ? w.nbv : nullptr)))
+            return rc;
+    }
     {
-        int di[5], n = 0;
-        const unsigned long long* sp[5];
+        int di[6], n = 0;
+        const unsigned long long* sp[6];
         di[n] = STAT_REFINED; sp[n++] = w.cnt + CNT_REFINED;
         if (sh.hash) { di[n] = STAT_HASH_FIX; sp[n++] = w.cnt + CNT_HFIX; }
         di[n] = STAT_ASSIGN_AMBIG; sp[n++] = w.cnt + CNT_AMBIG;
@@ -283,15 +299,15 @@
             di[n] = STAT_ASSIGN_AMBIG; sp[n++] = w.cnt + CNT_PAIR;
             di[n] = STAT_PAIR_ROWS; sp[n++] = w.cnt + CNT_PAIR;
         }
-        if ((rc = launch_add_counters(s, ctx->stats.as<unsigned long long>(), n, di, sp))) return rc;
-    }
-    if (cosine || pwfix) {
-        if ((rc = launch_cos_fix_seg(s, q, ndist_fix, dist_fix, cosine ? w.xn2 : nullptr, cosine ? w.nbv : nullptr)))
+        if (dist_lists) { di[n] = cosine ? STAT_COS_FIX : STAT_POW_FIX; sp[n++] = w.cnt + CNT_CFIX; }
+        if ((rc = launch_fused_epilogue(s, ctx->stats.as<unsigned long long>(), n, di, sp, w.cnt,
+                                        (int)(FUSED_COUNTER_CLEAR / 8), reinterpret_cast<unsigned int*>(w.cbound),
+                                        (int)(FUSED_CBOUND_BYTES / 4), q.src_dev, q.K, q.N, q.assign, q.dist)))
             return rc;
-        if ((rc = launch_add_counter(s, ctx->stats.as<unsigned long long>() + (cosine ? STAT_COS_FIX : STAT_POW_FIX),
-                                     w.cnt + CNT_CFIX)))
-            return rc;
-    }
+    }
+    ctx->ws_clean.cnt = w.cnt; ctx->ws_clean.cnt_cap = ctx->ws_counter.cap;
+    ctx->ws_clean.cb = w.cbound; ctx->ws_clean.cb_cap = ctx->ws_cconst.cap;
+    if ((rc = side.join())) { ctx->ws_dirty(); return rc; }
     return 0;
 }
 
diff --git a/crypto-recommendation_amd/csrc/fused_args.h b/crypto-recommendation_amd/csrc/fused_args.h
--- a/crypto-recommendation_amd/csrc/fused_args.h
+++ b/crypto-recommendation_amd/csrc/fused_args.h
@@ -60,6 +60,7 @@
     unsigned long long* pairs;
     unsigned long long* pair_count;
     int K;
+    int settle;
 };
 
 }
diff --git a/crypto-recommendation_amd/csrc/fused_layout.h b/crypto-recommendation_amd/csrc/fused_layout.h
--- a/crypto-recommendation_amd/csrc/fused_layout.h
+++ b/crypto-recommendation_amd/csrc/fused_layout.h
@@ -64,6 +64,7 @@
 constexpr int CNT_CFIX = 3;
 constexpr int CNT_PAIR = 4;
 constexpr size_t FUSED_COUNTER_BYTES = 64, FUSED_COUNTER_CLEAR = 40;
+constexpr size_t FUSED_CBOUND_BYTES = 32;
 
 struct FusedShape {
     int64_t N = 0;
diff --git a/crypto-recommendation_amd/csrc/fused_refine.hip b/crypto-recommendation_amd/csrc/fused_refine.hip
--- a/crypto-recommendation_amd/csrc/fused_refine.hip
+++ b/crypto-recommendation_amd/csrc/fused_refine.hip
@@ -1,4 +1,5 @@
 #include "fused_impl.h"
+#include "settle.h"
 
 namespace lshkm {
 
@@ -29,6 +30,7 @@
 
 __host__ __device__ constexpr int fp_lds_bytes(int Kpad) { return 16 + 2 * Kpad * FU_RS * 2 + Kpad * 4; }
 static_assert(fp_lds_bytes(FP_KMAX) <= 160 * 1024, "refinement LDS image exceeds 160 KiB");
+static_assert(FP_KMAX <= 32 * ST_TILES, "a settled row's candidate mask covers one refinement pass");
 
 constexpr int FP_PAIR_REC = 16;
 constexpr int FP_PAIR_RS = FU_D | 1;
@@ -81,6 +83,31 @@
             a.dist[row] = best;
         }
         wave_sync();
+    }
+}
+
+template <int ROWS>
+__device__ inline void settle_rows(const FusedArgs& a, unsigned long long amask, const LaneMask& cand, int64_t row,
+                                   bool ok, int lane) {
+    using TX = std::conditional_t<ROWS == 2, double, float>;
+    const TX* X;
+    if constexpr (ROWS == 2) X = a.X64; else X = a.X;
+    const int d = ROWS == 0 ? FU_D : a.d;
+    for (unsigned long long m = amask; m; m &= m - 1) {
+        const int up = __builtin_ctzll(m), lw = up - 32;
+        const int64_t r = __shfl(row, up);
+        const LaneMask m0 = {__shfl(cand.lo, lw), __shfl(cand.hi, lw)}, m1 = {__shfl(cand.lo, up), __shfl(cand.hi, up)};
+        const bool rok = __shfl(ok ? 1 : 0, up) != 0;
+        unsigned long long cm[ST_CHUNKS];
+        const int n = settle_set(m0, m1, a.K, cm);
+        const TX* xr = X + r * d;
+        double best = 0.0;
+        int bi = -1;
+        if (rok && n >= 1 && n <= 64)
+            pruned_pick_euclid<64>(xr, a.Cd, d, kth_candidate(cm, lane), !a.fast_dist, best, bi);
+        else
+            every_centroid(a.K, [&](int c) { return exact_euclid_rolled(xr, a.Cd + (size_t)c * d, d); }, best, bi);
+        wave_store(best, bi, r, a.assign, a.dist);
     }
 }
 
@@ -219,6 +246,29 @@
                    (double)pm.M3 < (double)M1 - 2.0 * (double)E;
         }
 
+        const bool amb = valid && !cert && !pair;
+        LaneMask cand = {0ull, 0ull};
+        bool settle = false;
+        if constexpr (PAIR) {
+            settle = a.settle && __ballot(amb) != 0ull;
+            if (settle) {
+                const double thr = (double)M1 - 2.0 * (double)E;
+                __builtin_amdgcn_s_setprio(MFMA_PRIO);
+#pragma unroll 1
+                for (int t = 0; t < ntile32; t++) {
+                    float sv[16];
+                    floatx16 acc_hi, acc_lo;
+                    tile_mfma(my_h + t * 32 * FU_RS, my_l + t * 32 * FU_RS, bh, bl, acc_hi, acc_lo);
+                    tile_scores(acc_hi, acc_lo, lcn + t * 32 + 4 * h, sv);
+                    uint32_t bits = 0u;
+#pragma unroll
+                    for (int i = 0; i < 16; i++) bits |= (double)sv[i] >= thr ? 1u << i : 0u;
+                    settle_mark(cand, t, bits);
+                }
+                __builtin_amdgcn_s_setprio(0);
+            }
+        }
+
         PT_MARK(2)
         if constexpr (MET == 1) {
             bool fix = false;
@@ -295,7 +345,6 @@
         PT_MARK(3)
         if constexpr (PAIR)
             seg_append(valid && pair && h == 1, pair_record(row, I1, I2), lcount + 1, pair_seg, lane);
-        const bool amb = valid && !cert && !pair;
         const unsigned long long amask = __ballot(amb && h == 1);
         if (h == 1 && valid) {
             if (amb) {
@@ -304,8 +353,11 @@
                 if (lane == leader) base = atomicAdd(lcount, __popcll(amask));
                 base = __shfl(base, leader);
                 const int rank = __popcll(amask & ((1ull << lane) - 1ull));
-                ambig_seg[base + rank] = (int32_t)row;
-            }
+                if (!(PAIR && a.settle)) ambig_seg[base + rank] = (int32_t)row;
+            }
+        }
+        if constexpr (PAIR) {
+            if (settle) settle_rows<ROWS>(a, amask, cand, row, x_ok && c_ok, lane);
         }
         PT_MARK(4)
     }
diff --git a/crypto-recommendation_amd/csrc/fused_small.hip b/crypto-recommendation_amd/csrc/fused_small.hip
--- a/crypto-recommendation_amd/csrc/fused_small.hip
+++ b/crypto-recommendation_amd/csrc/fused_small.hip
@@ -305,7 +305,6 @@
 int launch_fused_prep(hipStream_t s, const double* C, int K, int d, int metric, const FusedWorkspace& w) {
     const int Kpad = (K + 63) / 64 * 64;
     static_assert(64 % FP_PREP_WAVES == 0, "Kpad is a multiple of 64");
-    (void)hipMemsetAsync(w.cbound, 0, 32, s);
     hipLaunchKernelGGL(fused_centroid_prep, dim3((unsigned)(Kpad / FP_PREP_WAVES)), dim3(64 * FP_PREP_WAVES), 0, s, C, K, Kpad, w.Ch, w.Cl, w.cnh,
                        reinterpret_cast<unsigned int*>(w.cbound), metric, w.nbv, w.C32, w.rn32, d, w.C64p);
     return kstatus("fused_centroid_prep");
diff --git a/crypto-recommendation_amd/csrc/index.h b/crypto-recommendation_amd/csrc/index.h
--- a/crypto-recommendation_amd/csrc/index.h
+++ b/crypto-recommendation_amd/csrc/index.h
@@ -51,6 +51,7 @@
     const ::lshkm_lsh_s* lsh = nullptr;
     int32_t *tuples = nullptr, *phi = nullptr, *bucket = nullptr;
     bool force_exact = false;
+    const int32_t* src_dev = nullptr;
 };
 int fused_assign(lshkm_ctx_s* ctx, const AssignRequest& q);
 
@@ -81,6 +82,11 @@
     lshkm::Buf ws_nearest[3];
     lshkm::Buf ws_knn;
     uint64_t ws_epoch = 0;
+    struct WsClean {
+        const void *cnt = nullptr, *cb = nullptr;
+        size_t cnt_cap = 0, cb_cap = 0;
+    } ws_clean;
+    void ws_dirty() { ws_clean = WsClean{}; }
     bool timing = false;
     hipEvent_t tev[3] = {nullptr, nullptr, nullptr};
     bool tev_side = false;
diff --git a/crypto-recommendation_amd/csrc/kernels.h b/crypto-recommendation_amd/csrc/kernels.h
--- a/crypto-recommendation_amd/csrc/kernels.h
+++ b/crypto-recommendation_amd/csrc/kernels.h
@@ -111,6 +111,9 @@
 int launch_add_counter(hipStream_t s, unsigned long long* dst, const unsigned long long* src);
 int launch_add_counters(hipStream_t s, unsigned long long* stats, int n, const int* dst_idx,
                         const unsigned long long* const* src);
+int launch_fused_epilogue(hipStream_t s, unsigned long long* stats, int n, const int* dst_idx,
+                          const unsigned long long* const* srcs, unsigned long long* cnt, int ncnt, unsigned int* cb,
+                          int ncb, const int32_t* src_rows, int K, int64_t N, int32_t* assign, double* dist);
 
 size_t sort_scratch_bytes(int64_t N, int64_t range, int T = 1);
 int pow_contract_check();
diff --git a/crypto-recommendation_amd/csrc/pick.h b/crypto-recommendation_amd/csrc/pick.h
--- a/crypto-recommendation_amd/csrc/pick.h
+++ b/crypto-recommendation_amd/csrc/pick.h
@@ -76,4 +76,21 @@
     best = group_min<G>(v);
 }
 
+template <typename F>
+__device__ inline void every_centroid(int K, F&& dd, double& best, int& bi) {
+    for (int c = threadIdx.x & 63; c < K; c += 64) {
+        const double v = dd(c);
+        if (bi < 0 ? (v == v || c == 0) : v < best) { best = v; bi = c; }
+    }
 }
+
+__device__ inline void wave_store(double best, int bi, int64_t row, int32_t* __restrict__ assign,
+                                  double* __restrict__ dist) {
+    group_argmin<64>(best, bi);
+    if ((threadIdx.x & 63) == 0) {
+        assign[row] = bi < 0 ? 0 : bi;
+        dist[row] = bi < 0 ? -1.0 : best;
+    }
+}
+
+}
diff --git a/crypto-recommendation_amd/csrc/settle.h b/crypto-recommendation_amd/csrc/settle.h
--- /dev/null
+++ b/crypto-recommendation_amd/csrc/settle.h
@@ -0,0 +1,64 @@
+#pragma once
+#include <stdint.h>
+
+#if defined(__HIPCC__) || defined(__CUDACC__)
+#define ST_HD __host__ __device__ inline
+#else
+#define ST_HD inline
+#endif
+
+namespace lshkm {
+
+constexpr int ST_TILES = 8;
+constexpr int ST_CHUNKS = ST_TILES / 2;
+
+struct LaneMask {
+    unsigned long long lo, hi;
+};
+
+ST_HD int settle_centroid(int h, int t, int i) { return 32 * t + 8 * (i >> 2) + 4 * h + (i & 3); }
+
+ST_HD void settle_mark(LaneMask& m, int t, uint32_t bits16) {
+    const unsigned long long b = (unsigned long long)(bits16 & 0xFFFFu) << (16 * (t & 3));
+    if (t < 4) m.lo |= b; else m.hi |= b;
+}
+
+ST_HD unsigned long long settle_spread(uint32_t two_tiles) {
+    unsigned long long x = two_tiles;
+    x = (x | (x << 16)) & 0x0000FFFF0000FFFFull;
+    x = (x | (x << 8)) & 0x00FF00FF00FF00FFull;
+    x = (x | (x << 4)) & 0x0F0F0F0F0F0F0F0Full;
+    return x;
+}
+
+ST_HD int settle_set(const LaneMask& m0, const LaneMask& m1, int K, unsigned long long (&cm)[ST_CHUNKS]) {
+    cm[0] = settle_spread((uint32_t)m0.lo) | (settle_spread((uint32_t)m1.lo) << 4);
+    cm[1] = settle_spread((uint32_t)(m0.lo >> 32)) | (settle_spread((uint32_t)(m1.lo >> 32)) << 4);
+    cm[2] = settle_spread((uint32_t)m0.hi) | (settle_spread((uint32_t)m1.hi) << 4);
+    cm[3] = settle_spread((uint32_t)(m0.hi >> 32)) | (settle_spread((uint32_t)(m1.hi >> 32)) << 4);
+    int n = 0;
+    for (int i = 0; i < ST_CHUNKS; i++) {
+        const int left = K - 64 * i;
+        if (left < 64) cm[i] &= left <= 0 ? 0ull : (1ull << left) - 1ull;
+        n += __builtin_popcountll(cm[i]);
+    }
+    return n;
+}
+
+template <int NCH>
+ST_HD int kth_candidate(const unsigned long long (&cm)[NCH], int k) {
+    int c = -1, seen = 0;
+#pragma unroll
+    for (int i = 0; i < NCH; i++) {
+        const int n = __builtin_popcountll(cm[i]);
+        if (c < 0 && k >= seen && k < seen + n) {
+            unsigned long long m = cm[i];
+            for (int t = k - seen; t > 0; t--) m &= m - 1;
+            c = 64 * i + __builtin_ctzll(m);
+        }
+        seen += n;
+    }
+    return c;
+}
+
+}
```

New measurement: 5.598 billion point hash+assign ops/s (median of 6 runs). 1.02x the previous value.
